# hhcho/sfgwas

Hardware: AMD Instinct MI355X
Metric: pca_power_iter_ring_macs_per_s (higher is better)
Workload: dtype u64 ring words, exact integers: int8 digits on the matrix core for the MAC of all five moduli, fp64-held integers in the encode and key-switch kernels

## Files before the change

### sfgwas_amd/csrc/ab/config.hip

```cpp
#include "../common.hpp"

void ab_read_config(SfgConfig &c) {
    auto env = [](const char *n) { return getenv(n); };
    if (const char *e = env("SFG_MAC_IMPL")) { c.mac_reg = !strcmp(e, "reg"); c.mac_bc = strcmp(e, "dma") != 0 && !c.mac_reg; c.mac_i8 = !strcmp(e, "i8"); }
    if (const char *e = env("SFG_MAC_I8_BIG")) c.mac_i8_big = atoi(e) != 0;
    if (const char *e = env("SFG_MAC_I8_ROT")) { c.mac_i8_nolds = strcmp(e, "lds") != 0; c.mac_i8_ring = !strcmp(e, "ring"); }
    if (env("SFG_MAC_I8_WG")) c.mac_i8_ring = false;
    if (const char *e = env("SFG_MAC_I8_WAVES")) c.mac_i8_waves = atoi(e) == 6 ? 6 : 12;
    if (const char *e = env("SFG_MAC_I8_WG")) c.mac_i8_wg1 = atoi(e) == 1;
    if (const char *e = env("SFG_MAC_WC")) c.mac_wc = atoi(e) == 2 ? 2 : 1;
    if (const char *e = env("SFG_MM_OVERLAP")) c.no_overlap = atoi(e) == 0;
    if (env("SFG_MM_NO_OVERLAP")) c.no_overlap = true;
    if (const char *e = env("SFG_NTT_HALF_IMPL")) c.ntt_half_full = !strcmp(e, "full");
    if (const char *e = env("SFG_NTT_FWD_IMPL")) c.ntt_fwd_full = !strcmp(e, "full");
    if (const char *e = env("SFG_MAC_PT")) c.mac_plain_pt = !strcmp(e, "plain");
    if (const char *e = env("SFG_PT_RIDE")) { c.pt_ride = atoi(e); if (c.pt_ride < 0) c.pt_ride = 0; c.pt_ride = c.pt_ride / 8 * 8; }
    if (const char *e = env("SFG_PT_COMPACT")) c.pt_compact = atoi(e) != 0;
    if (const char *e = env("SFG_PT_KMAJOR")) c.pt_kmajor = atoi(e) != 0;
    if (const char *e = env("SFG_PT_RIDE_DEPTH")) { c.i8_mover_depth_ride = atoi(e); if (c.i8_mover_depth_ride < 1 || c.i8_mover_depth_ride > 3) c.i8_mover_depth_ride = 1; }
    if (const char *e = env("SFG_PT_RIDE_NT")) c.i8_mover_nt_ride = atoi(e) != 0;
    if (env("SFG_ASSOC_TRACE")) c.assoc_trace = true;
}
int ab_set_attrs(sfg_ctx *ctx) { return ab_mac_dma_set_attrs(ctx) || ab_ntt_set_attrs(ctx); }
```

### sfgwas_amd/csrc/common.hpp

```cpp
#pragma once
#include <hip/hip_runtime.h>
#include <cstdint>
#include <cstdio>
#include <cstring>
#include <string>
#include <vector>
#include <map>
#include <set>
#include <initializer_list>
#include <type_traits>
#include <unistd.h>
#include "../../include/sfgwas_hip.h"
#include "fp64mod.hpp"
#include "consts.hpp"

typedef unsigned long long u64;
typedef unsigned __int128 u128;

constexpr unsigned long long SFG_I8_BIG_QMAX = 0x7F7F7F7F7F80ULL;

struct ModConst {
    double q, qinv;
    double ninv, ninv_q;
    u64 qi;
};

struct RotKey {
    u64 *key_dev = nullptr;
    uint16_t *index_dev = nullptr;
};

struct PhaseStat { double ms = 0; int launches = 0; double bytes = 0; };
struct PendingEvent { hipEvent_t e0, e1; std::string name; int launches; double bytes; };

struct sfg_geno {
    const int8_t *dev = nullptr;
    size_t nrow = 0, ncol = 0, ld = 0;
    bool owned = false;
    bool packed = false;
    struct PtcEntry { double *slot; bool transposed; };
    mutable std::map<uint64_t, PtcEntry> ptc;
    mutable size_t ptc_budget = 0, ptc_used = 0;
    mutable double *ptc_arena = nullptr;
    mutable uint32_t *ptc_perm = nullptr;
    mutable const void *ptc_owner = nullptr;
    mutable size_t ptc_hits = 0, ptc_fills = 0;
};

struct SfgConfig {
    int mm_group = 8;
    bool mm_group_auto = true;
    size_t acc_budget = 24ULL << 30;
    size_t assoc_cache_budget = 160ULL << 30;
    size_t ksw_budget = 4ULL << 30;
    int enc_batch = 2048;
    bool upload_blocking = false;
    bool test_hooks = false;
    std::string test_scratch_oom;
    double tie_band = 0x1p-50;
    bool mac_i8_big = true;
    bool mac_reg = false;
    bool mac_bc = true;
    bool mac_i8 = true;
    bool mac_i8_nolds = true;
    bool mac_i8_ring = true;
    int mac_i8_waves = 12;
    bool mac_i8_wg1 = false;
    int mac_wc = 1;
    bool no_overlap = true;
    bool ntt_fwd_full = false;
    bool ntt_half_full = false;
    bool pt_compact = true;
    bool pt_kmajor = true;
    int pt_ride = 192;
    int i8_mover_depth_ride = 1, i8_mover_nt_ride = 1;
    bool mac_plain_pt = false;
    bool assoc_trace = false;
};

struct SfgShared {
    int device = 0;
    int logN = SFG_LOGN, N = SFG_N, nq = 0, np = 0, nmod = 0, beta = 0;
    double scale = 0;
    u64 q[SFG_MAXMOD] = {0}, psi[SFG_MAXMOD] = {0};
    double *tw_fwd = nullptr;
    double *tw_inv = nullptr;
    double2 *pack_fwd = nullptr;
    double2 *pack_inv = nullptr;
    ModConst *modc = nullptr;
    ModConst modc_host[SFG_MAXMOD];
    void *enc_tables = nullptr;
    void *rvec_tables = nullptr;
    void *zeros_dev = nullptr;
    u64 *sk_dev = nullptr;
    u64 *pk_dev = nullptr;
    u64 *skqp_dev = nullptr;
    uint32_t enc_key[8] = {0, 0, 0, 0, 0, 0, 0, 0}; uint32_t *enc_key_dev = nullptr; bool enc_seeded = false;
    u64 enc_next = 0;
    std::map<u64, RotKey> rotkeys;
    SfgConfig cfg;
    int refs = 1;
};

struct sfg_ctx {
    SfgShared *sh = nullptr;
    bool is_fork = false;
    int device = 0;
    int logN = SFG_LOGN, N = SFG_N, nq = 0, np = 0, nmod = 0, beta = 0;
    double scale = 0;
    u64 q[SFG_MAXMOD] = {0}, psi[SFG_MAXMOD] = {0};
    double *tw_fwd = nullptr, *tw_inv = nullptr;
    double2 *pack_fwd = nullptr, *pack_inv = nullptr;
    ModConst *modc = nullptr;
    ModConst modc_host[SFG_MAXMOD];
    SfgConfig cfg;
    unsigned ntt_plain_seq = 0;
    struct I8Slot { const void *src = nullptr; u64 sig[8] = {0, 0, 0, 0, 0, 0, 0, 0}; u64 last_use = 0; };
    static constexpr int I8_SLOTS = 16;
    u64 i8_gen = 1, i8_clock = 0; I8Slot i8_slot[2][I8_SLOTS];
    hipStream_t own_stream = nullptr, stream = nullptr;
    hipStream_t user_stream = nullptr;
    hipStream_t aux_stream = nullptr;
    unsigned char *pin = nullptr; size_t pin_bytes = 0, pin_head = 0;
    hipStream_t coll_stream = nullptr;
    hipEvent_t ev_pipe[4] = {nullptr, nullptr, nullptr, nullptr};
    std::vector<hipEvent_t> ev_pool; size_t ev_next = 0;
    std::map<int, struct KswLevel *> ksw_cache;
    void *ws = nullptr; size_t ws_bytes = 0;
    std::map<std::string, std::pair<void *, size_t>> pool;
    std::map<std::string, std::pair<void *, size_t>> host_pool;
    std::map<std::string, unsigned long long> pool_epoch;
    unsigned long long api_epoch = 0; int api_depth = 0;
    int scratch_oom_seen = 0;
    std::vector<PendingEvent> pending;
    std::string err;
    std::map<std::string, PhaseStat> phases;
    std::set<const sfg_geno *> ptc_genos;
    bool test_hooks = false;
    void *tie_count_dev = nullptr;
    hipStream_t main_stream() const { return user_stream ? user_stream : own_stream; }
    std::map<u64, RotKey> &rotkeys() { return sh->rotkeys; }
    const std::map<u64, RotKey> &rotkeys() const { return sh->rotkeys; }
    void *enc_tables() const { return sh->enc_tables; }
    void *zeros_dev() const { return sh->zeros_dev; }
};

int sfg_sync_all(sfg_ctx *ctx);
int sfg_encoder_check(sfg_ctx *ctx);
void sfg_ptc_detach_all(sfg_ctx *ctx);
void sfg_ptc_invalidate_all(sfg_ctx *ctx);

int encrypt_set_attrs(sfg_ctx *ctx);
int sfg_rows_from_montgomery(sfg_ctx *ctx, unsigned long long *rows_dev, size_t nrows, int nmod);
void sfg_encrypt_destroy(SfgShared *sh);
int enc_take_indices(sfg_ctx *ctx, const char *what, int nct, unsigned long long *first);
int keygen_set_attrs(sfg_ctx *ctx);
void sfg_keygen_destroy(SfgShared *sh);
int sfg_rvec_init(sfg_ctx *ctx);
void sfg_rvec_destroy(SfgShared *sh);
// ... 119 lines not shown
```

### sfgwas_amd/csrc/kernels.hpp

```cpp
#pragma once
#include "common.hpp"
#include "mm_plan.hpp"
#include "assoc_plan.hpp"
#include "batch_plan.hpp"

constexpr int SFG_MAXPATTERN = 128;
struct ModPattern { int period; int8_t m[SFG_MAXPATTERN]; };
inline ModPattern mod_pattern_run(int first, int count) { ModPattern p; p.period = count; for (int j = 0; j < count; j++) p.m[j] = (int8_t)(first + j); return p; }
struct RowMap { int rpg; size_t gstride_in, gstride_out; };
struct PanelMap { int G, g, shift0; unsigned packed_mask = 0; int K = 0; };

int launch_ntt_fwd(sfg_ctx *ctx, const u64 *in, u64 *out, size_t nrows, const ModPattern &pat);
int launch_ntt_inv(sfg_ctx *ctx, const u64 *in, u64 *out, size_t nrows, const ModPattern &pat);
int launch_ntt_plain(sfg_ctx *ctx, const double *pc, u64 *out, size_t nplain, int L);
struct MoveJob;
struct PtRide;
int launch_ntt_plain_half(sfg_ctx *ctx, const double *pc, u64 *out_half, size_t nplain, int L, PanelMap pm, const uint32_t *perm = nullptr, const MoveJob *mv = nullptr);
int launch_expand_half(sfg_ctx *ctx, const u64 *half, u64 *full, size_t nrows);
int launch_ntt_fwd_map(sfg_ctx *ctx, const u64 *in, u64 *out, size_t nrows, const ModPattern &pat, const RowMap &rm);
int launch_ntt_inv_map(sfg_ctx *ctx, const u64 *in, u64 *out, size_t nrows, const ModPattern &pat, const RowMap &rm);
int launch_ntt_fwd_staged(sfg_ctx *ctx, const u64 *in, u64 *out, size_t nrows, const ModPattern &pat, bool staged);
int launch_ntt_inv_split(sfg_ctx *ctx, const u64 *in, u64 *out, size_t nrows, const ModPattern &pat, const RowMap &rm);
struct MacStrides { size_t rot_k, rot_r, pt_k, pt_n, out_n, out_r; bool pt_half = false; bool pt_packed = false; bool pt_digits = false; bool i8 = false; bool i8_big = false; bool pt_digits_big = false;
                    const int8_t *B_small = nullptr, *B_big = nullptr;
                    int pt_layout = 0, pt_L = 0;
                    int B_mode = 0;
                    const int8_t *A_small = nullptr, *A_big = nullptr; };
int launch_mac_i8_small(sfg_ctx *ctx, const double *rotf, size_t rotf_k_stride, size_t rotf_r_stride, int plane0, const u64 *pt, u64 *out, int K, int R, int r0, int Ncols,
                        int l0, int nl, int accumulate, const MacStrides &st);
int launch_mac_i8_big(sfg_ctx *ctx, const double *rotf, size_t rotf_k_stride, size_t rotf_r_stride, int plane0, const u64 *pt, u64 *out, int K, int R, int r0, int Ncols,
                      int l0, int accumulate, const MacStrides &st);
int launch_skew(sfg_ctx *ctx, const int8_t *blk, size_t ld, int r, int c, int transposed, int square, int8_t *D);
struct PcCache { double *slot = nullptr; int mode = 0; const uint32_t *perm = nullptr; };
int launch_encode_rows(sfg_ctx *ctx, const int8_t *D, int shift0, int nshift, int L, u64 *pt, bool half_rows = false, int G = 0, int g = 0, unsigned packed_mask = 0, const PcCache *pcache = nullptr,
                       PtRide *ride = nullptr);
int encode_rows_launches(const sfg_ctx *ctx, int nshift);
int i8_ride_prepare(sfg_ctx *ctx, const u64 *panel, int K, int Ncols, size_t pt_k, size_t pt_n, int layout, int L, int launches, PtRide &ride);
int i8_ride_finish(sfg_ctx *ctx, PtRide &ride);
int i8_ride_tiles(sfg_ctx *ctx, int K, int L, int8_t **Bs, int8_t **Bb);
struct I8Args;
void launch_i8_pack_pt_digits(hipStream_t q, const I8Args &a, unsigned items, bool big);
void launch_move_alone(hipStream_t q, const MoveJob &j);
int launch_share(sfg_ctx *ctx, const u64 *rows, size_t rows_ct_stride, const u64 *xr, size_t x_ct_stride, u64 *h, int nl, int nct, int neg = 0);
int launch_add_rows(sfg_ctx *ctx, const u64 *a, size_t a_ct_stride, const u64 *b, size_t b_ct_stride, u64 *out, size_t out_ct_stride, int nl, int nct);
struct DecSrc {
    enum Kind { ROWS, FINISH, DECRYPT } kind; const u64 *src; size_t stride; const u64 *h0agg;
    static DecSrc rows(const u64 *pt, size_t stride) { return DecSrc{ROWS, pt, stride, nullptr}; }
    static DecSrc finish(const u64 *ct, const u64 *h0agg) { return DecSrc{FINISH, ct, 0, h0agg}; }
    static DecSrc decrypt(const u64 *ct) { return DecSrc{DECRYPT, ct, 0, nullptr}; }
};
int launch_dec_front(sfg_ctx *ctx, const DecSrc &s, int first, int nb, int nl, u64 *x, int *launches = nullptr);
int check_level_count(sfg_ctx *ctx, const char *what, int nct, int level, int maxl, int min_count = 0);
int encrypt_errors_moddown(sfg_ctx *ctx, const int32_t *e0, const int32_t *e1, int nct, int level, u64 *out);
int launch_geno_unpack(sfg_ctx *ctx, const sfg_geno *g, size_t r0, size_t c0, size_t nr, size_t nc, int8_t *out, size_t ld_out);
int launch_rotate_right(sfg_ctx *ctx, const u64 *in, u64 *out, int nct, int level, const int *nrot_host);
int launch_rotate_right_indexed(sfg_ctx *ctx, const u64 *in, int nin, u64 *out, int nct, int level, const int *nrot_host, const int *in_index);
int launch_rotate_right_indexed_f64(sfg_ctx *ctx, const u64 *in, int nin, double *outf, int nct, int level, const int *nrot_host, const int *in_index, int L,
                                    const size_t *out_slot = nullptr);
int launch_rotate_right_sum(sfg_ctx *ctx, const u64 *in, int nin, int nct, int level, const int *nrot_host, const int *in_index, const int *group, int nout,
                            u64 *out, size_t out_stride, int accumulate);
int launch_relinearize(sfg_ctx *ctx, const u64 *tmp, int nct, int level, const u64 *mid, u64 *out);
int launch_ct_add(sfg_ctx *ctx, const u64 *a, const u64 *b, u64 *out, size_t nct, int level);
int mac_dma_planes(sfg_ctx *ctx, int L, std::vector<int> &plane_of, std::vector<int> &is_big);
double mac_big_maxterm(u64 q);
int launch_rot_to_f64(sfg_ctx *ctx, const u64 *rot, size_t nrows, int nl_rot, int L, double *rotf);
int launch_mac_dma(sfg_ctx *ctx, const double *rotf, size_t rows_per_k, const u64 *pt, u64 *out, int K, int R, int Ncols, int L, int accumulate, const MacStrides &st);
int launch_pack_pt(sfg_ctx *ctx, const u64 *in, u64 *out, size_t nrows, size_t words_per_row, int L, unsigned packed_mask);
unsigned mac_dma_packed_mask(sfg_ctx *ctx, int L);
bool mac_use_dma(const sfg_ctx *ctx);
int launch_mac_bc(sfg_ctx *ctx, const double *rotf, size_t rows_per_k, const u64 *pt, u64 *out, int K, int R, int Ncols, int L, int accumulate, const MacStrides &st);
int rotcache_build_rows_tab(sfg_ctx *ctx, const u64 *A, int s, int in_level, int max_level, int nbr, int b0, int b1, const std::vector<std::vector<uint8_t>> *tabs, double *cache);
int assoc_build_rotcache(sfg_ctx *ctx, const u64 *A_dev, int s, int in_level, int max_level, size_t nr, const std::vector<size_t> &widths, double **out);
struct I8RotPre { int G = 0, nbr = 0, s = 0, L = 0; std::vector<int8_t *> As, Ab; };
int i8_rotpre_build(sfg_ctx *ctx, const u64 *A_dev, int s, int in_level, int max_level, int nbr, const std::vector<std::vector<uint8_t>> *tabs, size_t budget_bytes, const char *prefix, I8RotPre &pre);
void i8_rotpre_free(I8RotPre &pre);
struct I8RotPreScope { I8RotPre pre; ~I8RotPreScope() { i8_rotpre_free(pre); } };
struct RotOperand {
    RotSrc src = RotSrc::own;
    const u64 *A = nullptr;
    int in_level = -1;
    const double *rows = nullptr;
    const I8RotPre *tiles = nullptr;
    static RotOperand own(const u64 *A, int in_level) { RotOperand r; r.A = A; r.in_level = in_level; return r; }
    static RotOperand f64_cache(const double *rows, int in_level = -1) { RotOperand r; r.src = RotSrc::f64_cache; r.rows = rows; r.in_level = in_level; return r; }
    static RotOperand i8_tiles(const I8RotPre *pre) { RotOperand r; r.src = RotSrc::i8_tiles; r.tiles = pre; return r; }
    int level_in(int max_level) const { return in_level < 0 ? max_level : in_level; }
    int validate(sfg_ctx *ctx, int s, int L, int nbr, int b0, int b1) const;
};
struct MmArgs { const sfg_geno *g; unsigned flags; int s, max_level, b0, b1, j0, j1, accumulate; uint64_t *acc; size_t acc_col_words; };
struct MmRangeArgs { const sfg_geno *g; unsigned flags; int s, max_level, blk0, blk1; uint64_t *out; };
int matmul_accumulate(sfg_ctx *ctx, const RotOperand &rot, const MmArgs &a);
int matmul_resident_range(sfg_ctx *ctx, const RotOperand &rot, const MmRangeArgs &a);
int launch_i8_pack_rot_to(sfg_ctx *ctx, const double *rotf, size_t rotf_k_stride, size_t rotf_r_stride, int plane0, int K, int R, int l0, int nl, bool big, int8_t *A_out);
struct AssocRot { RotOperand op; I8RotPre pre; };
int assoc_build_rot(sfg_ctx *ctx, const u64 *A_dev, int s, int in_level, int max_level, size_t nr, const std::vector<size_t> &widths, AssocRot &out);
void assoc_free_rot(AssocRot &r);
struct AssocRotScope { AssocRot r; ~AssocRotScope() { assoc_free_rot(r); } };
int assoc_product(sfg_ctx *ctx, const AssocRot &r, int s, int max_level, const sfg_geno *g, unsigned flags, int nct, uint64_t *out);
int assoc_batch_tail(sfg_ctx *ctx, const u64 *tmp, const sfg_geno *g, int s, size_t nct, size_t ctw, uint64_t *out_dev, size_t out_ct_capacity, size_t out_shift,
                     double *sum_host, double *sqsum_host);

int launch_bed_decode(sfg_ctx *ctx, hipStream_t st, const uint8_t *dbed, size_t bps, size_t num_sample, size_t num_snp, const int32_t *rmap, const int32_t *cmap,
                      int8_t *out, size_t ld);
int launch_bed_decode_lut(sfg_ctx *ctx, hipStream_t st, const uint8_t *dbed, size_t bps, size_t num_sample, size_t num_snp, const int32_t *rmap, const int32_t *cmap,
                          int8_t *out, size_t ld, unsigned lut);
int upload_filter_map(sfg_ctx *ctx, const uint8_t *filt, size_t n, DevMem &map, size_t *kept);

int assoc_stream_part(sfg_ctx *ctx, int fmt, const char *path, size_t num_sample, size_t num_snp, const uint8_t *row_filter, const uint8_t *col_filter,
                      size_t batch_snps, const uint64_t *A_dev, int s, int in_level, int max_level, unsigned flags,
                      uint64_t *out_dev, size_t out_ct_capacity, size_t *out_ct, double *sum_host, double *sqsum_host,
                      int part, int nparts, std::vector<std::pair<size_t, size_t>> *ranges);
```

### sfgwas_amd/csrc/mac_i8.hip

```cpp
#include "common.hpp"
#include "kernels.hpp"
#include "i8_move.hpp"
#include <algorithm>
#include <cstring>
#include <vector>

constexpr int I8_PC = 16;
template <int ND> constexpr int i8_rot_img_stride() { return ND * 512; }
template <int ND>
__global__ void __launch_bounds__(256) k_i8_pack_rot(I8Args a) {
    extern __shared__ __attribute__((aligned(16))) int8_t img[];
    constexpr int CS = i8_rot_img_stride<ND>();
    const int N = SFG_N, tid = threadIdx.x;
    int b = blockIdx.x;
    const int rt = b & 1; b >>= 1;
    const int khalf = b & 1; b >>= 1;
    const int xb = b % (N / I8_PC), ch = (b / (N / I8_PC)) % a.nch, m = b / (N / I8_PC) / a.nch;
    const int x0 = xb * I8_PC, cc = tid & (I8_PC - 1), kkq = (tid >> 4) & 3, kh2 = (tid >> 6) & 1, rh = tid >> 7;
    const double *src = ND == 6 ? a.rotf + (size_t)a.plane0 * N + 2 * (x0 + cc) : a.rotf + (size_t)(a.plane0 + m) * N + x0 + cc;
    size_t koff[4]; bool kv[4];
#pragma unroll
    for (int j = 0; j < 4; j++) {
        const int k = ch * 64 + 32 * khalf + 16 * kh2 + 4 * kkq + j;
        int ks = k; kv[j] = k < a.K;
        if (a.kb) { const int gg = k / a.kb, baby = k - gg * a.kb; kv[j] = kv[j] && baby < SFG_D; ks = gg * SFG_D + baby; }
        koff[j] = kv[j] ? (size_t)ks * a.rotf_k_stride : 0;
    }
    double lo[8][4], hi[ND == 6 ? 8 : 1][4];
#pragma unroll
    for (int ri = 0; ri < 8; ri++) {
        const int r = a.r0 + rt * 16 + rh * 8 + ri;
        const double *e = src + (size_t)(r < a.R ? r : a.r0) * a.rotf_r_stride;
#pragma unroll
        for (int j = 0; j < 4; j++) { lo[ri][j] = e[koff[j]]; if (ND == 6) hi[ri][j] = e[koff[j] + 1]; }
    }
#pragma unroll
    for (int ri = 0; ri < 8; ri++) {
        const int r16 = rh * 8 + ri;
        const bool rv = a.r0 + rt * 16 + r16 < a.R;
        unsigned dw[ND];
#pragma unroll
        for (int i = 0; i < ND; i++) dw[i] = 0;
#pragma unroll
        for (int j = 0; j < 4; j++) {
            long long v = ND == 6 ? (long long)hi[ND == 6 ? ri : 0][j] * 8388608LL + (long long)lo[ri][j] : (long long)lo[ri][j];
            if (!(rv && kv[j])) v = 0;
            int8_t d[ND]; i8_digits<ND>(v, d);
#pragma unroll
            for (int i = 0; i < ND; i++) dw[i] |= (unsigned)(uint8_t)d[i] << (8 * j);
        }
        unsigned *o = reinterpret_cast<unsigned *>(img + cc * CS + (((r16 + 16 * kh2) ^ cc) << 4) + 4 * kkq);
#pragma unroll
        for (int i = 0; i < ND; i++) o[i * 128] = dw[i];
    }
    __syncthreads();
    for (int idx = tid; idx < I8_PC * ND * 32; idx += 256) {
        const int c2 = idx / (ND * 32), rem = idx - c2 * (ND * 32), dg = rem >> 5, lr = rem & 31;
        const uint4 w = *reinterpret_cast<const uint4 *>(img + c2 * CS + dg * 512 + ((lr ^ c2) << 4));
        *reinterpret_cast<uint4 *>(a.A + ((((((size_t)m * N + x0 + c2) * a.nch + ch) * 2 + rt) * ND + dg) * 1024) + khalf * 512 + lr * 16) = w;
    }
}
constexpr int I8_PP = 32;
template <int ND>
__global__ void __launch_bounds__(256) k_i8_pack_pt(I8Args a) {
    constexpr int PSTR = ND * 256 + 4;
    __shared__ __attribute__((aligned(16))) unsigned char img[I8_PP * PSTR];
    const int H = SFG_N / 2, tid = threadIdx.x;
    int b = blockIdx.x;
    const int cb = b % (H / I8_PP); b /= H / I8_PP;
    const int kq = b % (a.nch * 4); b /= a.nch * 4;
    const int jt = b % a.njt, m = b / a.njt;
    const int c0 = cb * I8_PP, cc = tid & (I8_PP - 1), slot = tid >> 5;
    const u64 *src = a.pt + a.pt_l0_off + (size_t)m * a.pt_l_stride + c0 + cc;
#pragma unroll 2
    for (int it = 0; it < 8; it++) {
        const int item = it * 8 + slot, j = item >> 2, k4 = item & 3, n = jt * 16 + j;
        unsigned dw[ND];
#pragma unroll
        for (int i = 0; i < ND; i++) dw[i] = 0;
#pragma unroll
        for (int x = 0; x < 4; x++) {
            const int k = kq * 16 + k4 * 4 + x;
            long long v = 0;
            if (k < a.K && n < a.Ncols) {
                const u64 w = src[(size_t)n * a.pt_n_stride + (size_t)k * a.pt_k_stride];
                v = ND == 6 ? (long long)w : (long long)((w & 0xFFFULL) | (((w >> 16) & 0xFFFULL) << 12) | ((w >> 32) << 24));
            }
            int8_t d[ND]; i8_digits<ND>(v, d);
#pragma unroll
            for (int i = 0; i < ND; i++) dw[i] |= (unsigned)(uint8_t)d[i] << (8 * x);
        }
#pragma unroll
        for (int i = 0; i < ND; i++) *reinterpret_cast<unsigned *>(img + cc * PSTR + i * 256 + j * 16 + k4 * 4) = dw[i];
    }
    __syncthreads();
    const int ch = kq >> 2, g = kq & 3, l16 = tid & 15;
    for (int pc = tid >> 4; pc < I8_PP * ND; pc += 16) {
        const int c2 = pc / ND, d = pc % ND;
        const unsigned *sp = reinterpret_cast<const unsigned *>(img + c2 * PSTR + d * 256 + l16 * 16);
        const uint4 w = make_uint4(sp[0], sp[1], sp[2], sp[3]);
        *reinterpret_cast<uint4 *>(a.B + ((((((size_t)m * H + c0 + c2) * a.njt + jt) * a.nch + ch) * ND + d) * 1024) + g * 256 + l16 * 16) = w;
    }
}
template <int ND>
__global__ void __launch_bounds__(256) k_i8_pack_pt_digits(I8Args a) {
    __shared__ __attribute__((aligned(16))) unsigned img[I8_PD * 64];
    const int H = SFG_N / 2, tid = threadIdx.x;
    int b = blockIdx.x;
    const int cb = b % (H / I8_PD); b /= H / I8_PD;
    const int kq = b % (a.nch * 4); b /= a.nch * 4;
    const int jt = b % a.njt, m = b / a.njt;
    const int c0 = cb * I8_PD, cq = tid & 31, slot = tid >> 5;
    const int ch = kq >> 2, g = kq & 3, l16 = tid & 15;
    const unsigned char *src = reinterpret_cast<const unsigned char *>(a.pt + a.pt_l0_off + (size_t)m * a.pt_l_stride) + (size_t)cb * a.pt_cb_stride + cq * 4;
    constexpr int NI = 8;
    for (int d = 0; d < ND; d++) {
        for (int it0 = 0; it0 < 8; it0 += NI) {
            unsigned w[NI][4];
#pragma unroll
            for (int u = 0; u < NI; u++) {
                const int item = (it0 + u) * 8 + slot, j = item >> 2, k4 = item & 3, n = jt * 16 + j;
#pragma unroll
                for (int x = 0; x < 4; x++) {
                    const int k = kq * 16 + k4 * 4 + x;
                    const bool ok = k < a.K && n < a.Ncols;
                    const unsigned v = *reinterpret_cast<const unsigned *>(src + (ok ? ((size_t)n * a.pt_n_stride + (size_t)k * a.pt_k_stride) * 8 : (size_t)0) + (size_t)d * a.pt_d_stride);
                    w[u][x] = ok ? v : 0u;
                }
            }
#pragma unroll
            for (int u = 0; u < NI; u++) {
                const int item = (it0 + u) * 8 + slot, j = item >> 2, k4 = item & 3;
                unsigned o[4]; bytes_tr4(w[u][0], w[u][1], w[u][2], w[u][3], o);
#pragma unroll
                for (int e = 0; e < 4; e++) img[(cq * 4 + e) * 64 + ((j ^ (cq & 7)) << 2) + (k4 ^ (cq >> 3))] = o[e];
            }
        }
        __syncthreads();
        for (int pc = tid >> 4; pc < I8_PD; pc += 16) {
            const int q2 = pc >> 2;
            const unsigned *sp = img + pc * 64 + ((l16 ^ (q2 & 7)) << 2);
            const uint4 w = make_uint4(sp[0 ^ (q2 >> 3)], sp[1 ^ (q2 >> 3)], sp[2 ^ (q2 >> 3)], sp[3 ^ (q2 >> 3)]);
            *reinterpret_cast<uint4 *>(a.B + ((((((size_t)m * H + c0 + pc) * a.njt + jt) * a.nch + ch) * ND + d) * 1024) + g * 256 + l16 * 16) = w;
// ... 157 lines not shown
    SFG_HIP(ctx, hipFuncSetAttribute((const void *)k_mac_i8_ring<5, 3>, hipFuncAttributeMaxDynamicSharedMemorySize, 3 * 10 * 5 * 1024));
    SFG_HIP(ctx, hipFuncSetAttribute((const void *)k_mac_i8_ring<6, 2>, hipFuncAttributeMaxDynamicSharedMemorySize, 2 * 10 * 6 * 1024));
    SFG_HIP(ctx, hipFuncSetAttribute((const void *)k_mac_i8_ring<5, 3, 2>, hipFuncAttributeMaxDynamicSharedMemorySize, 3 * 10 * 5 * 1024));
    SFG_HIP(ctx, hipFuncSetAttribute((const void *)k_mac_i8_ring<6, 2, 2>, hipFuncAttributeMaxDynamicSharedMemorySize, 2 * 10 * 6 * 1024));
    return 0;
}
void launch_i8_pack_pt_digits(hipStream_t q, const I8Args &a, unsigned items, bool big) {
    if (big) hipLaunchKernelGGL(k_i8_pack_pt_digits<6>, dim3(items), dim3(256), 0, q, a);
    else hipLaunchKernelGGL(k_i8_pack_pt_digits<5>, dim3(items), dim3(256), 0, q, a);
}
void launch_move_alone(hipStream_t q, const MoveJob &j) {
#define SFG_MV(D, T) hipLaunchKernelGGL((k_i8_move_pt<D, T>), dim3(j.nblocks), dim3(256), 0, q, j)
#ifdef SFG_AB
    if (j.depth == 3) { if (j.nt) SFG_MV(3, true); else SFG_MV(3, false); return; }
    if (j.depth == 2) { if (j.nt) SFG_MV(2, true); else SFG_MV(2, false); return; }
    if (!j.nt) { SFG_MV(1, false); return; }
#endif
    SFG_MV(1, true);
#undef SFG_MV
}
static bool i8_ride_moduli(sfg_ctx *ctx, int L, int &l_small0, int &n_small, int &l_big) {
    std::vector<int> plane_of, is_big; if (mac_dma_planes(ctx, L, plane_of, is_big) < 0) return false;
    l_big = -1; l_small0 = -1; n_small = 0; int nbig = 0;
    for (int l = 0; l < L; l++) { if (is_big[l]) { l_big = l; nbig++; } else { if (l_small0 < 0) l_small0 = l; n_small++; } }
    if (nbig > 1 || !n_small) return false;
    for (int l = 0; l < L; l++) if (!is_big[l] && (l < l_small0 || l >= l_small0 + n_small)) return false;
    if (l_big >= 0 && (!ctx->cfg.mac_i8_big || ctx->q[l_big] > SFG_I8_BIG_QMAX)) return false;
    return true;
}
int i8_ride_tiles(sfg_ctx *ctx, int K, int L, int8_t **Bs, int8_t **Bb) {
    int l_small0, n_small, l_big;
    *Bs = *Bb = nullptr;
    if (!i8_ride_moduli(ctx, L, l_small0, n_small, l_big)) return 0;
    SFG_TRY(sfg_scratch(ctx, "mi8.Bs", mac_i8_tile_bytes(K, n_small, 5), (void **)Bs));
    if (l_big >= 0) SFG_TRY(sfg_scratch(ctx, "mi8.Bb", mac_i8_tile_bytes(K, 1, 6), (void **)Bb));
    return 0;
}
void i8_panel_rows(const sfg_ctx *ctx, int layout, int K, int L, int l, bool big, I8Args &a) {
    const size_t H = SFG_N / 2;
    a.pt_d_stride = H; a.pt_cb_stride = I8_PD;
    if (layout == 0) { a.pt_l0_off = (size_t)l * H; a.pt_l_stride = H; return; }
    size_t below = 0, all = 0; for (int t = 0; t < L; t++) { const size_t pl = ctx->q[t] < (1ULL << 36) ? 5 : 6; if (t < l) below += pl; all += pl; }
    const size_t nd = big ? 6 : 5;
    if (layout == 1) { a.pt_l0_off = below * H / 8; a.pt_l_stride = nd * H / 8; return; }
    const size_t blk = (size_t)K * 128;
    a.pt_d_stride = 64 * blk; a.pt_cb_stride = blk;
    a.pt_l0_off = below * 64 * blk / 8; a.pt_l_stride = nd * 64 * blk / 8;
    a.pt_k_stride = 16; a.pt_n_stride = all * 64 * blk / 8;
}
int i8_ride_prepare(sfg_ctx *ctx, const u64 *panel, int K, int Ncols, size_t pt_k, size_t pt_n, int layout, int L, int launches, PtRide &ride) {
    const int H = SFG_N / 2;
    ride = PtRide();
    int l_small0, n_small, l_big;
    if (ctx->cfg.pt_ride <= 0 || launches < 1 || Ncols > 96 || !i8_ride_moduli(ctx, L, l_small0, n_small, l_big)) return 0;
    if (layout != 2 && (pt_n * 8 >= (1ULL << 31) || pt_k * 8 * 16 >= (1ULL << 31))) return 0;
    if (layout == 2 && (size_t)K * 128 * 64 * 32 >= (1ULL << 31)) return 0;
    int8_t *Bs, *Bb; SFG_TRY(i8_ride_tiles(ctx, K, L, &Bs, &Bb));
    const int nch = (K + 63) / 64, njt = (Ncols + 15) / 16;
    auto fill = [&](I8Args &a, int l0, int nl, int8_t *B) {
        memset(&a, 0, sizeof a);
        a.pt = panel; a.pt_k_stride = pt_k; a.pt_n_stride = pt_n; a.K = K; a.Ncols = Ncols; a.l0 = l0; a.nl = nl; a.nch = nch; a.njt = njt; a.pt_digits = 1; a.B = B;
        i8_panel_rows(ctx, layout, K, L, l0, l0 == l_big, a);
    };
    MoveJob &j = ride.job;
    fill(j.a5, l_small0, n_small, Bs); j.n5 = (unsigned)((size_t)n_small * njt * nch * 4 * (H / I8_PD));
    if (l_big >= 0) { fill(j.a6, l_big, 1, Bb); j.n6 = (unsigned)((size_t)njt * nch * 4 * (H / I8_PD)); } else { memset(&j.a6, 0, sizeof j.a6); j.n6 = 0; }
    j.nblocks = (unsigned)ctx->cfg.pt_ride; j.depth = ctx->cfg.i8_mover_depth_ride; j.nt = ctx->cfg.i8_mover_nt_ride; j.first = 0; j.count = 0;
    ride.next = 0; ride.per = (ride.total() + (unsigned)launches - 1) / (unsigned)launches;
    ride.item_bytes5 = 5.0 * 2 * 32768; ride.item_bytes6 = 6.0 * 2 * 32768;
    ride.on = true;
    return 0;
}
int i8_ride_finish(sfg_ctx *ctx, PtRide &ride) {
    if (!ride.on || ride.next >= ride.total()) return 0;
    MoveJob j = ride.job; j.first = ride.next; j.count = ride.total() - ride.next; ride.next = ride.total();
    j.nblocks = std::min(2048u, (j.count + 7u) / 8u * 8u);
    PhaseTimer t(ctx, "mac_i8_pack_pt");
    launch_move_alone(ctx->stream, j);
    SFG_HIP(ctx, hipGetLastError());
    t.stop(1);
    return 0;
}
template <int ND>
static int launch_mac_i8_nd(sfg_ctx *ctx, const double *rotf, size_t rotf_k_stride, size_t rotf_r_stride, int plane0, const u64 *pt, u64 *out, int K, int R, int r0, int Ncols,
                            int l0, int nl, int accumulate, const MacStrides &st) {
    const int N = SFG_N, H = N / 2;
    constexpr bool BIG = ND == 6;
    if (!st.pt_half || (!BIG && !st.pt_packed)) SFG_FAIL(ctx, "sfg_mac (i8): needs half-row plaintext rows (packed-limb words or digit planes for the small moduli)");
    if (BIG && nl != 1) SFG_FAIL(ctx, "sfg_mac (i8): one 46-bit modulus per launch");
    if (Ncols > 96) SFG_FAIL(ctx, "sfg_mac (i8): more than 96 columns per launch");
    if ((long long)K * ND >= 131072) SFG_FAIL(ctx, "sfg_mac (i8): K too large for the int32 digit sums (ND K 2^14 must stay below 2^31)");
    for (int t = l0; t < l0 + nl; t++) {
        if (ctx->q[t] > (BIG ? SFG_I8_BIG_QMAX : (1ULL << 38))) SFG_FAIL(ctx, "sfg_mac (i8): modulus %d = %llu does not fit %d signed base-256 digits / the exact fp64 recombination", t, (unsigned long long)ctx->q[t], ND);
    }
    const int8_t *B_given = BIG ? st.B_big : st.B_small;
    const int8_t *B_pre = B_given && st.B_mode == 1 ? B_given : nullptr;
    if (B_given && (st.B_mode < 1 || st.B_mode > 2 || !st.pt_digits)) SFG_FAIL(ctx, "sfg_mac (i8): internal: given tile buffers take digit-plane panels");
    const int8_t *A_pre = BIG ? st.A_big : st.A_small;
    if (A_pre && (r0 != 0 || R > 32)) SFG_FAIL(ctx, "sfg_mac (i8): internal: given rot tiles cover one block of <= 32 rows");
    I8Args a; memset(&a, 0, sizeof a);
    a.rotf = rotf; a.pt = pt; a.out = out; a.rotf_k_stride = rotf_k_stride; a.rotf_r_stride = rotf_r_stride;
    a.pt_k_stride = st.pt_k; a.pt_n_stride = st.pt_n; a.out_n_stride = st.out_n; a.out_r_stride = st.out_r;
    if (st.pt_layout && !st.pt_digits) SFG_FAIL(ctx, "sfg_mac (i8): internal: compact panel rows hold digit planes");
    i8_panel_rows(ctx, st.pt_layout, K, st.pt_L, l0, BIG, a);
    a.K = K; a.R = R; a.Ncols = Ncols; a.accumulate = accumulate; a.r0 = r0; a.l0 = l0; a.nl = nl; a.plane0 = plane0;
    a.nch = (K + 63) / 64; a.njt = (Ncols + 15) / 16; a.pt_digits = st.pt_digits ? 1 : 0;
    const size_t nA = (size_t)nl * N * a.nch * 2 * ND * 1024, nB = (size_t)nl * H * a.njt * a.nch * ND * 1024, nT = (size_t)nl * H * 2 * a.njt * 2 * 256;
    const u64 sig[8] = {ctx->i8_gen, (u64)K, (u64)R, (u64)r0, (u64)l0 << 8 | (u64)nl, (u64)plane0, (u64)rotf_k_stride, (u64)rotf_r_stride};
    sfg_ctx::I8Slot *slots = ctx->i8_slot[BIG ? 1 : 0];
    int slot = -1;
    if (!A_pre) for (int i = 0; i < sfg_ctx::I8_SLOTS; i++) if (slots[i].src == (const void *)rotf && !memcmp(slots[i].sig, sig, sizeof sig)) slot = i;
    const bool repack = slot < 0 && !A_pre;
    char nm[24];
    if (repack) {
        int stale = -1, empty = -1, lru = 0;
        for (int i = 0; i < sfg_ctx::I8_SLOTS; i++) {
            if (!slots[i].src) { if (empty < 0) empty = i; continue; }
            if (slots[i].sig[0] != ctx->i8_gen && (stale < 0 || slots[i].last_use < slots[stale].last_use)) stale = i;
            if (slots[i].last_use < slots[lru].last_use || !slots[lru].src) lru = i;
        }
        slot = stale;
        if (slot < 0 && empty >= 0) {
            int live = 0; for (int i = 0; i < sfg_ctx::I8_SLOTS; i++) live += slots[i].src != nullptr;
            size_t fr = 0, tot = 0;
            if (live < 2 || (hipMemGetInfo(&fr, &tot) == hipSuccess && fr >= nA + (48ULL << 30))) slot = empty;
        }
        if (slot < 0) slot = lru;
    }
    if (A_pre) a.A = const_cast<int8_t *>(A_pre);
    else {
        snprintf(nm, sizeof nm, BIG ? "mi8.Ab%d" : "mi8.A%d", slot);
        SFG_TRY(sfg_scratch(ctx, nm, nA, (void **)&a.A));
        if (repack) { slots[slot].src = (const void *)rotf; memcpy(slots[slot].sig, sig, sizeof sig); }
        slots[slot].last_use = ++ctx->i8_clock;
    }
    if (B_given) a.B = const_cast<int8_t *>(B_given);
    else SFG_TRY(sfg_scratch(ctx, "mi8.B", nB, (void **)&a.B));
    SFG_TRY(sfg_scratch(ctx, "mi8.T", nT * 8, (void **)&a.T));
    if (!A_pre && !repack && ctx->pool[nm].second < nA) SFG_FAIL(ctx, "sfg_mac (i8): internal: kept rot copy smaller than its operand");
    const double tile = 1024.0;
    if (repack) { PhaseTimer t(ctx, "mac_i8_pack_rot");
      hipLaunchKernelGGL(k_i8_pack_rot<ND>, dim3((unsigned)((size_t)nl * a.nch * (N / I8_PC) * 4)), dim3(256), I8_PC * i8_rot_img_stride<ND>(), ctx->stream, a);
      SFG_HIP(ctx, hipGetLastError()); t.stop(1, (double)nl * N * ((double)K * std::min(32, R - r0) * (BIG ? 16.0 : 8.0) + (double)a.nch * 2 * ND * tile)); }
    if (!B_pre) { PhaseTimer t(ctx, "mac_i8_pack_pt");
      const unsigned items = (unsigned)((size_t)nl * a.njt * a.nch * 4 * (H / I8_PD));
      if (a.pt_digits) launch_i8_pack_pt_digits(ctx->stream, a, items, BIG);
      else hipLaunchKernelGGL(k_i8_pack_pt<ND>, dim3((unsigned)((size_t)nl * a.njt * a.nch * 4 * (H / I8_PP))), dim3(256), 0, ctx->stream, a);
      SFG_HIP(ctx, hipGetLastError()); t.stop(1, (double)nl * H * ((double)K * Ncols * (a.pt_digits ? (double)ND : 8.0) + (double)a.njt * a.nch * ND * tile)); }
    { PhaseTimer t(ctx, BIG ? "mac_big" : "mac_small");
      if (a.njt == 6 && ctx->cfg.mac_i8_ring) {
          if (BIG && ctx->cfg.mac_i8_waves == 12) hipLaunchKernelGGL((k_mac_i8_ring<6, 2, 2>), dim3((unsigned)(nl * H)), dim3(768), 2 * 10 * 6 * 1024, ctx->stream, a, ctx->modc);
          else if (BIG) hipLaunchKernelGGL((k_mac_i8_ring<6, 2>), dim3((unsigned)(nl * H)), dim3(384), 2 * 10 * 6 * 1024, ctx->stream, a, ctx->modc);
          else if (ctx->cfg.mac_i8_waves == 12) hipLaunchKernelGGL((k_mac_i8_ring<5, 3, 2>), dim3((unsigned)(nl * H)), dim3(768), 3 * 10 * 5 * 1024, ctx->stream, a, ctx->modc);
          else hipLaunchKernelGGL((k_mac_i8_ring<5, 3>), dim3((unsigned)(nl * H)), dim3(384), 3 * 10 * 5 * 1024, ctx->stream, a, ctx->modc);
      }
#ifdef SFG_AB
      else if (!BIG && a.njt == 6 && !ctx->cfg.mac_i8_nolds) ab_launch_mac_i8_lds(ctx->stream, a, ctx->modc, nl);
#endif
      else if (ctx->cfg.mac_i8_wg1) hipLaunchKernelGGL(k_mac_i8<ND>, dim3((unsigned)(nl * H * a.njt)), dim3(64), 0, ctx->stream, a, ctx->modc);
      else hipLaunchKernelGGL(k_mac_i8<ND>, dim3((unsigned)(nl * H)), dim3(64 * a.njt), 0, ctx->stream, a, ctx->modc);
      SFG_HIP(ctx, hipGetLastError());
      t.stop(1, (double)nl * ((double)N * a.nch * 2 * ND * tile + (double)H * a.njt * a.nch * ND * tile + (double)H * 2 * a.njt * 2 * 256 * 8.0)); }
    { PhaseTimer t(ctx, "mac_i8_untile");
      hipLaunchKernelGGL(k_i8_untile, dim3((unsigned)((size_t)nl * (H / 16) * 2 * a.njt * 2)), dim3(256), 0, ctx->stream, a, ctx->modc);
      SFG_HIP(ctx, hipGetLastError());
      t.stop(1, (double)nl * N * (double)Ncols * std::min(32, R - r0) * 8.0 * (accumulate ? 3.0 : 2.0)); }
    return 0;
}
int launch_i8_pack_rot_to(sfg_ctx *ctx, const double *rotf, size_t rotf_k_stride, size_t rotf_r_stride, int plane0, int K, int R, int l0, int nl, bool big, int8_t *A_out) {
    if (R > 32 || (big && nl != 1)) SFG_FAIL(ctx, "i8 rot tiles: internal: at most 32 rows, one 46-bit modulus per buffer");
    I8Args a; memset(&a, 0, sizeof a);
    a.rotf = rotf; a.rotf_k_stride = rotf_k_stride; a.rotf_r_stride = rotf_r_stride; a.K = K; a.R = R; a.r0 = 0; a.l0 = l0; a.nl = nl; a.plane0 = plane0;
    a.nch = (K + 63) / 64; a.kb = 0; a.A = A_out;
    const int N = SFG_N;
    PhaseTimer t(ctx, "mac_i8_pack_rot");
    if (big) hipLaunchKernelGGL(k_i8_pack_rot<6>, dim3((unsigned)((size_t)nl * a.nch * (N / I8_PC) * 4)), dim3(256), I8_PC * i8_rot_img_stride<6>(), ctx->stream, a);
    else hipLaunchKernelGGL(k_i8_pack_rot<5>, dim3((unsigned)((size_t)nl * a.nch * (N / I8_PC) * 4)), dim3(256), I8_PC * i8_rot_img_stride<5>(), ctx->stream, a);
    SFG_HIP(ctx, hipGetLastError());
    t.stop(1);
    return 0;
}
int launch_mac_i8_small(sfg_ctx *ctx, const double *rotf, size_t rotf_k_stride, size_t rotf_r_stride, int plane0, const u64 *pt, u64 *out, int K, int R, int r0, int Ncols,
                        int l0, int nl, int accumulate, const MacStrides &st) {
    return launch_mac_i8_nd<5>(ctx, rotf, rotf_k_stride, rotf_r_stride, plane0, pt, out, K, R, r0, Ncols, l0, nl, accumulate, st);
}
int launch_mac_i8_big(sfg_ctx *ctx, const double *rotf, size_t rotf_k_stride, size_t rotf_r_stride, int plane0, const u64 *pt, u64 *out, int K, int R, int r0, int Ncols,
                      int l0, int accumulate, const MacStrides &st) {
    return launch_mac_i8_nd<6>(ctx, rotf, rotf_k_stride, rotf_r_stride, plane0, pt, out, K, R, r0, Ncols, l0, 1, accumulate, st);
}

__global__ void __launch_bounds__(256) k_i8_words_to_planes(const u64 *in, u64 *out, int L, unsigned big_mask) {
    const int H = SFG_N / 2;
    const size_t row = blockIdx.x; const int l = (int)(row % (size_t)L);
    const u64 *src = in + row * H; int8_t *dst = reinterpret_cast<int8_t *>(out + row * H);
    const bool big = (big_mask >> l) & 1u;
    for (int c = threadIdx.x; c < H; c += 256) {
        const long long v = (long long)src[c];
        if (big) { int8_t d[6]; i8_digits<6>(v, d);
#pragma unroll
            for (int i = 0; i < 6; i++) dst[(size_t)i * H + c] = d[i]; }
        else { int8_t d[5]; i8_digits<5>(v, d);
#pragma unroll
            for (int i = 0; i < 5; i++) dst[(size_t)i * H + c] = d[i]; }
    }
}
extern "C" int sfg_mac_i8_dev(sfg_ctx *ctx, const uint64_t *rot, const uint64_t *pt_half, uint64_t *out, int K, int R, int Ncols, int L, int accumulate, int pt_form) {
    SFG_HIP(ctx, hipSetDevice(ctx->device));
    if (!ctx->test_hooks) SFG_FAIL(ctx, "sfg_mac_i8_dev is a test hook: the context was not created under the test switch");
    if (L < 1 || L > ctx->nq) SFG_FAIL(ctx, "sfg_mac_i8: L out of range");
    if (K < 1 || R < 1 || Ncols < 1) SFG_FAIL(ctx, "sfg_mac_i8: K, R and Ncols must be positive (got %d, %d, %d)", K, R, Ncols);
    if (Ncols > 96 || (long long)K * 6 >= 131072) SFG_FAIL(ctx, "sfg_mac_i8: at most 96 columns and K < 21846 per launch");
    if (pt_form != 0 && pt_form != 1) SFG_FAIL(ctx, "sfg_mac_i8: pt_form is 0 (digit planes) or 1 (panel words)");
    const int N = SFG_N, H = N / 2;
    std::vector<int> plane_of, is_big; const int nplanes = mac_dma_planes(ctx, L, plane_of, is_big);
    if (nplanes < 0) return 1;
    unsigned big_mask = 0, small_mask = 0; for (int l = 0; l < L; l++) (is_big[l] ? big_mask : small_mask) |= 1u << l;
    if (big_mask && !ctx->cfg.mac_i8_big) SFG_FAIL(ctx, "sfg_mac_i8: a modulus above 2^36 is on the fp64 kernel in this context (it exceeds six signed digits: q > 0x7F7F7F7F7F80; or the A/B build's switch)");
    const size_t rrows = (size_t)K * R, prows = (size_t)K * Ncols * L;
    double *rotf = nullptr; u64 *ptp = nullptr;
    int rc = 0;
    if (hipMalloc(&rotf, rrows * (size_t)nplanes * N * 8) != hipSuccess || hipMalloc(&ptp, prows * H * 8) != hipSuccess) { (void)hipGetLastError(); (void)hipFree(rotf); SFG_FAIL(ctx, "sfg_mac_i8: out of device memory"); }
    rc = launch_rot_to_f64(ctx, (const u64 *)rot, rrows, L, L, rotf);
    if (!rc) {
        if (pt_form == 0) { hipLaunchKernelGGL(k_i8_words_to_planes, dim3((unsigned)prows), dim3(256), 0, ctx->stream, (const u64 *)pt_half, ptp, L, big_mask); if (hipGetLastError() != hipSuccess) { rc = 1; ctx->err = "sfg_mac_i8: plane kernel launch failed"; } }
        else rc = launch_pack_pt(ctx, (const u64 *)pt_half, ptp, prows, (size_t)H, L, small_mask);
    }
    if (!rc) {
        MacStrides st;
        st.rot_k = (size_t)R * L * N; st.rot_r = (size_t)L * N;
        st.pt_k = (size_t)Ncols * L * H; st.pt_n = (size_t)L * H;
        st.out_n = (size_t)R * L * N; st.out_r = (size_t)L * N;
        st.pt_half = true; st.pt_packed = true; st.i8 = st.i8_big = true; st.pt_digits = st.pt_digits_big = pt_form == 0;
        PhaseTimer t(ctx, "mac");
        rc = launch_mac_bc(ctx, rotf, (size_t)R, ptp, (u64 *)out, K, R, Ncols, L, accumulate, st);
        t.stop(1);
    }
    (void)hipStreamSynchronize(ctx->stream); (void)hipFree(rotf); (void)hipFree(ptp);
    return rc;
}
```

### sfgwas_amd/csrc/matmul.hip

```cpp
#include "common.hpp"
#include "kernels.hpp"
#include "i8_move.hpp"
#include <algorithm>
#include <string>

static inline int ceil_div(size_t a, size_t b) { return (int)((a + b - 1) / b); }

struct Shape {
    size_t nrow, ncol;
    int nbr, m_ct;
    bool transposed;
    const int8_t *dev; size_t ld;
    const sfg_geno *g;
    int rows_of(int bi) const { return (int)(std::min((size_t)(bi + 1) * SFG_SLOTS, nrow) - (size_t)bi * SFG_SLOTS); }
    int cols_of(int bj) const { return (int)(std::min((size_t)(bj + 1) * SFG_SLOTS, ncol) - (size_t)bj * SFG_SLOTS); }
    const int8_t *block(int bi, int bj) const {
        return transposed ? dev + (size_t)bj * SFG_SLOTS * ld + (size_t)bi * SFG_SLOTS
                          : dev + (size_t)bi * SFG_SLOTS * ld + (size_t)bj * SFG_SLOTS;
    }
};
static Shape make_shape(const sfg_geno *g, unsigned flags) {
    Shape sh; sh.transposed = (flags & SFG_TRANSPOSE) != 0;
    sh.nrow = sh.transposed ? g->ncol : g->nrow; sh.ncol = sh.transposed ? g->nrow : g->ncol;
    sh.nbr = ceil_div(sh.nrow, SFG_SLOTS); sh.m_ct = ceil_div(sh.ncol, SFG_SLOTS);
// ... 214 lines not shown
extern "C" void sfg_geno_free(sfg_ctx *ctx, sfg_geno *g) {
    if (!g) return;
    ptc_drop(ctx, g);
    if (g->owned) { (void)hipSetDevice(ctx->device); (void)sfg_sync_all(ctx); (void)hipFree((void *)g->dev); }
    delete g;
}
extern "C" int sfg_geno_set_plaintext_cache(sfg_ctx *ctx, const sfg_geno *g, size_t max_bytes) {
    SFG_HIP(ctx, hipSetDevice(ctx->device));
    if (!g) SFG_FAIL(ctx, "sfg_geno_set_plaintext_cache: null matrix");
    if (!max_bytes) { ptc_drop(ctx, g); g->ptc_budget = 0; g->ptc_owner = nullptr; return 0; }
    if (g->ptc_owner && g->ptc_owner != (const void *)ctx) SFG_FAIL(ctx, "sfg_geno_set_plaintext_cache: the cache of this matrix belongs to another context (drop it there first)");
    if (!g->ptc_perm) {
        const int n = SFG_SLOTS, d = SFG_D; const unsigned M = 2u * SFG_N;
        std::vector<uint32_t> tab(n);
        std::vector<unsigned> pow5(n); pow5[0] = 1; for (int k = 1; k < n; k++) pow5[k] = (unsigned)(((u64)pow5[k - 1] * 5u) % M);
        for (int t = 0; t < n; t++) {
            const int u = (n - t) % n, k = ((t % d) + d * (u / d)) % n;
            tab[t] = (uint32_t)u | (uint32_t)pow5[k] << 16;
        }
        uint32_t *dv = nullptr;
        SFG_HIP(ctx, hipMalloc((void **)&dv, (size_t)n * 4));
        if (hipMemcpy(dv, tab.data(), (size_t)n * 4, hipMemcpyHostToDevice) != hipSuccess) { (void)hipFree(dv); SFG_FAIL(ctx, "sfg_geno_set_plaintext_cache: table upload failed"); }
        g->ptc_perm = dv;
    }
    const size_t slot_bytes = (size_t)SFG_SLOTS * SFG_SLOTS * 8, want = max_bytes / slot_bytes * slot_bytes;
    if (want != g->ptc_budget || !g->ptc_arena) {
        (void)hipStreamSynchronize(ctx->stream);
        g->ptc.clear(); g->ptc_used = 0;
        if (g->ptc_arena) { (void)hipFree(g->ptc_arena); g->ptc_arena = nullptr; }
        g->ptc_budget = 0;
        if (!want) SFG_FAIL(ctx, "sfg_geno_set_plaintext_cache: max_bytes is less than one block (%zu bytes)", slot_bytes);
        void *a = nullptr;
        if (hipMalloc(&a, want) != hipSuccess) { (void)hipGetLastError(); SFG_FAIL(ctx, "sfg_geno_set_plaintext_cache: cannot allocate %zu bytes", want); }
        g->ptc_arena = (double *)a; g->ptc_budget = want;
    }
    g->ptc_owner = ctx; ctx->ptc_genos.insert(g);
    return 0;
}
extern "C" int sfg_geno_plaintext_cache_stats(sfg_ctx *ctx, const sfg_geno *g, size_t *blocks, size_t *bytes, size_t *hits, size_t *fills) {
    if (!g) SFG_FAIL(ctx, "sfg_geno_plaintext_cache_stats: null matrix");
    if (blocks) *blocks = g->ptc.size();
    if (bytes) *bytes = g->ptc_used;
    if (hits) *hits = g->ptc_hits;
    if (fills) *fills = g->ptc_fills;
    return 0;
}
extern "C" int sfg_geno_colsums(sfg_ctx *ctx, const sfg_geno *g, double *sum_host, double *sqsum_host) {
    SFG_HIP(ctx, hipSetDevice(ctx->device));
    if (g->packed) {
        sfg_geno *u = nullptr; SFG_TRY(sfg_geno_unpack(ctx, g, &u));
        const int rc = sfg_geno_colsums(ctx, u, sum_host, sqsum_host); sfg_geno_free(ctx, u); return rc;
    }
    SFG_TRY(sfg_ws_reserve(ctx, g->ncol * 16));
    double *ds = (double *)ctx->ws, *dq = ds + g->ncol;
    SFG_HIP(ctx, hipMemsetAsync(ds, 0, g->ncol * 16, ctx->stream));
    hipLaunchKernelGGL(k_colsums, dim3((unsigned)((g->ncol + 255) / 256), (unsigned)((g->nrow + CS_ROWS - 1) / CS_ROWS)), dim3(256), 0, ctx->stream, g->dev, g->nrow, g->ncol, g->ld, ds, dq);
    SFG_HIP(ctx, hipGetLastError());
    if (sum_host) SFG_HIP(ctx, hipMemcpyAsync(sum_host, ds, g->ncol * 8, hipMemcpyDeviceToHost, ctx->stream));
    if (sqsum_host) SFG_HIP(ctx, hipMemcpyAsync(sqsum_host, dq, g->ncol * 8, hipMemcpyDeviceToHost, ctx->stream));
    SFG_HIP(ctx, hipStreamSynchronize(ctx->stream));
    return 0;
}
extern "C" int sfg_reduce_rows_dev(sfg_ctx *ctx, uint64_t *rows, size_t nrows_of_L, int L) {
    SFG_HIP(ctx, hipSetDevice(ctx->device));
    const size_t rows_total = nrows_of_L * L;
    if (!rows_total) return 0;
    hipLaunchKernelGGL(k_reduce_rows, dim3((unsigned)(rows_total * (SFG_N / 256))), dim3(256), 0, ctx->stream, (u64 *)rows, L, ctx->modc);
    SFG_HIP(ctx, hipGetLastError());
    return 0;
}

static std::vector<uint8_t> baby_table(const Shape &sh, int bi) {
    const int d = SFG_D, nr = sh.rows_of(bi);
    std::vector<uint8_t> baby_t(d, 0);
    for (int shift = 0; shift < SFG_SLOTS; shift++) {
        if (baby_t[shift % d]) continue;
        bool any = false;
        for (int bj = 0; bj < sh.m_ct && !any; bj++) any = diag_bool(nr, sh.cols_of(bj), SFG_SLOTS, -shift);
        if (any) baby_t[shift % d] = 1;
    }
    return baby_t;
}
static int build_rot_row_tab(sfg_ctx *ctx, const u64 *A, int s, int nl_in, int nl, int lev, int L, int nbr, int bi, const std::vector<uint8_t> &baby_t,
                             u64 *a_row, u64 *rotc, bool dma, double *rotf_dst) {
    const int d = SFG_D;
    SFG_TRY(launch_gather_operands(ctx, A, a_row, nbr, s, bi * s, s, nl_in, nl));
    {
        PhaseTimer t(ctx, "rotate");
        std::vector<int> nrv((size_t)d * s, 0), inv((size_t)d * s, 0);
        for (int baby = 0; baby < d; baby++) for (int i = 0; i < s; i++) { nrv[(size_t)baby * s + i] = baby_t[baby] ? -baby : 0; inv[(size_t)baby * s + i] = i; }
        if (dma) SFG_TRY(launch_rotate_right_indexed_f64(ctx, a_row, s, rotf_dst, d * s, lev, nrv.data(), inv.data(), L));
        else SFG_TRY(launch_rotate_right_indexed(ctx, a_row, s, rotc, d * s, lev, nrv.data(), inv.data()));
        t.stop(1);
    }
    return 0;
}


struct PoolMemory { size_t search = 0, keep = 0; bool failed = false; };
static PoolMemory pool_memory(sfg_ctx *ctx, const char *extra_prefix) {
    PoolMemory m; size_t fr = 0, tot = 0;
    m.failed = hipMemGetInfo(&fr, &tot) != hipSuccess;
    m.search = m.keep = fr;
    for (const auto &kv : ctx->pool) {
        if ((extra_prefix && kv.first.rfind(extra_prefix, 0) == 0) || kv.first == "mm.pt" || kv.first == "mm.rotf" || kv.first.rfind("mi8.", 0) == 0) m.search += kv.second.second;
        if (kv.first.rfind("mi8.A", 0) == 0) m.keep += kv.second.second;
    }
    return m;
}
static MmPlanIn plan_input(sfg_ctx *ctx, int s, int L, int nblockrows, int ncolb, const RotOperand &rot) {
    const SfgConfig &c = ctx->cfg;
    MmPlanIn in;
    in.mm_group = c.mm_group; in.mm_group_auto = c.mm_group_auto; in.mac_i8 = c.mac_i8; in.mac_i8_big = c.mac_i8_big;
    in.pt_compact = c.pt_compact; in.pt_kmajor = c.pt_kmajor; in.pt_ride = c.pt_ride; in.no_overlap = c.no_overlap;
    in.dma = mac_use_dma(ctx); in.packed_mask = in.dma ? mac_dma_packed_mask(ctx, L) : 0u; in.mods = ModSplit(ctx->q, L);
    in.s = s; in.L = L; in.nblockrows = nblockrows; in.ncolb = ncolb; in.rot = rot.src; in.pre_G = rot.tiles ? rot.tiles->G : 0;
    if (mm_plan_reads_memory(in)) { const PoolMemory m = pool_memory(ctx, nullptr); in.mem_failed = m.failed; in.mem_search = m.search; in.mem_keep = m.keep; }
    return in;
}
struct MmCall {
    sfg_ctx *ctx; const Shape &sh; unsigned flags; const RotOperand &rot;
    int s, L, lev, nl, nl_in; bool dma; unsigned packed_mask; size_t ctw, accw, rowf = 0;
    MmPlan plan;
    u64 *a_row = nullptr, *rotc = nullptr; int8_t *skew = nullptr, *unpacked = nullptr; double *rotf = nullptr;
    int8_t *rideBs = nullptr, *rideBb = nullptr;
};
struct MacJob { bool on = false; u64 *ptp = nullptr; int gsn = 0, gi = 0, acc_flag = 0; u64 *accj = nullptr; const double *rotf_grp = nullptr; };

static int build_group(const MmCall &c, int bg, int b1, int buf) {
    sfg_ctx *ctx = c.ctx; const int d = SFG_D, s = c.s, ng = std::min(c.plan.G, b1 - bg);
    ctx->i8_gen++;
    double *dst = c.rotf + (size_t)buf * c.plan.grp_slices * s * 2 * c.rowf;
    for (int g = 0; g < ng; g++) SFG_TRY(build_rot_row_tab(ctx, c.rot.A, s, c.nl_in, c.nl, c.lev, c.L, c.sh.nbr, bg + g, baby_table(c.sh, bg + g), c.a_row, c.rotc, c.dma, c.dma ? dst + (size_t)g * d * s * 2 * c.rowf : nullptr));
    if (c.dma && (ng * d) % 4)
        SFG_HIP(ctx, hipMemsetAsync(dst + (size_t)ng * d * s * 2 * c.rowf, 0, (size_t)3 * s * 2 * c.rowf * 8, ctx->stream));
    return 0;
}
static int run_mac(const MmCall &c, const MacJob &m, int B_mode) {
    sfg_ctx *ctx = c.ctx; const MmPlan &p = c.plan; const int N = SFG_N, d = SFG_D;
    PhaseTimer t(ctx, "mac");
    MacStrides st;
    if (c.rideBs) { st.B_small = c.rideBs; st.B_big = c.rideBb; st.B_mode = B_mode; }
    if (c.rot.tiles) { st.A_small = c.rot.tiles->As[m.gi]; st.A_big = c.rot.tiles->Ab[m.gi]; }
    st.rot_k = (size_t)c.s * c.ctw; st.rot_r = (size_t)c.nl * N;
    st.pt_k = p.plw; st.pt_n = (size_t)m.gsn * d * p.plw; st.pt_half = c.dma; st.pt_packed = c.packed_mask != 0; st.pt_digits = st.i8 = p.use_i8; st.i8_big = st.pt_digits_big = p.use_i8_big;
    st.pt_layout = p.pt_layout; st.pt_L = c.L;
    st.out_n = c.accw; st.out_r = (size_t)c.L * N;
    int rc;
    if (c.dma) rc = launch_mac_dma(ctx, m.rotf_grp, (size_t)c.s * 2, m.ptp, m.accj, m.gsn * d, 2 * c.s, d, c.L, m.acc_flag, st);
#ifdef SFG_AB
    else rc = launch_mac_strided(ctx, c.rotc, m.ptp, m.accj, d, 2 * c.s, d, c.L, m.acc_flag, st);
#else
    else { rc = 1; ctx->err = "matmul: the register-staged MAC exists in the A/B build only (make ab)"; }
#endif
    t.stop(1);
    return rc;
}
struct PtcSlot {
    static constexpr size_t slot_bytes = (size_t)SFG_SLOTS * SFG_SLOTS * 8;
    PcCache pcc; const sfg_geno *g; uint64_t key = 0; bool fresh = false;
    PtcSlot(const MmCall &c, int bi, int bj) : g(c.sh.g) {
        if (!c.dma || !g->ptc_budget || g->ptc_owner != (const void *)c.ctx) return;
        const uint64_t sr = c.sh.transposed ? bj : bi, sc = c.sh.transposed ? bi : bj;
        key = sr << 33 | sc << 1 | ((c.flags & SFG_SQUARE) ? 1u : 0u);
        auto it = g->ptc.find(key);
        if (it != g->ptc.end()) { pcc.slot = it->second.slot; pcc.mode = it->second.transposed == c.sh.transposed ? 2 : 3; pcc.perm = g->ptc_perm; g->ptc_hits++; }
        else if (g->ptc_used + slot_bytes <= g->ptc_budget) {
            double *slot = g->ptc_arena + g->ptc_used / 8;
            g->ptc[key] = sfg_geno::PtcEntry{slot, c.sh.transposed}; g->ptc_used += slot_bytes; g->ptc_fills++;
            pcc.slot = slot; pcc.mode = 1; fresh = true;
        }
    }
    void undo() {
        if (!fresh) return;
        auto it = g->ptc.find(key);
        if (it != g->ptc.end()) { g->ptc.erase(it); g->ptc_used -= slot_bytes; }
        fresh = false;
    }
};
static int encode_block(const MmCall &c, int bi, int bj, int g, int ng, u64 *pt, PtRide *ride) {
    sfg_ctx *ctx = c.ctx; const Shape &sh = c.sh; const MmPlan &p = c.plan;
    const int d = SFG_D, L = c.L, nr = sh.rows_of(bi), nc = sh.cols_of(bj), tr = sh.transposed ? 1 : 0, sq = (c.flags & SFG_SQUARE) ? 1 : 0;
    const size_t plw = p.plw, nplain = (size_t)d * d;
    PtcSlot ptc(c, bi, bj);
    int rc = 0;
    if (ptc.pcc.mode < 2) {
        PhaseTimer t(ctx, "skew");
        if (sh.g->packed) {
            const size_t sr0 = (size_t)(tr ? bj : bi) * SFG_SLOTS, sc0 = (size_t)(tr ? bi : bj) * SFG_SLOTS;
            rc = launch_geno_unpack(ctx, sh.g, sr0, sc0, tr ? nc : nr, tr ? nr : nc, c.unpacked, SFG_SLOTS);
            if (!rc) rc = launch_skew(ctx, c.unpacked, SFG_SLOTS, nr, nc, tr, sq, c.skew);
        } else rc = launch_skew(ctx, sh.block(bi, bj), sh.ld, nr, nc, tr, sq, c.skew);
        t.stop(1);
    }
    if (rc) { ptc.undo(); return rc; }
    int runs[2][2]; int nruns = 0;
    if (nr + nc > SFG_SLOTS) { runs[0][0] = 0; runs[0][1] = SFG_SLOTS; nruns = 1; }
    else { runs[0][0] = 0; runs[0][1] = nr; runs[1][0] = SFG_SLOTS - nc + 1; runs[1][1] = SFG_SLOTS; nruns = runs[1][0] < runs[1][1] ? 2 : 1; }
    const bool full = nruns == 1 && runs[0][1] - runs[0][0] == SFG_SLOTS;
    if (p.kmajor) {
        const int kb0 = g * d;
        if (full) rc = launch_pt_zero_kmajor(ctx, pt, ng * d, p.pt_planes, d - 1, d, kb0 + (SFG_SLOTS - (d - 1) * d), kb0 + d);
        else rc = launch_pt_zero_kmajor(ctx, pt, ng * d, p.pt_planes, 0, d, kb0, kb0 + d);
    } else if (full) {
        rc = launch_pt_zero(ctx, pt + (((size_t)(d - 1) * ng + g) * d + (SFG_SLOTS - (d - 1) * d)) * plw, 0, (nplain - SFG_SLOTS) * plw, 1, L, p.prow, c.packed_mask);
    } else {
        rc = launch_pt_zero(ctx, pt + (size_t)g * d * plw, (size_t)ng * d * plw, (size_t)d * plw, d, L, p.prow, c.packed_mask);
    }
    if (rc) { ptc.undo(); return rc; }
    PhaseTimer t(ctx, "encode");
    for (int r = 0; r < nruns && !rc; r++) {
        if (c.dma) rc = launch_encode_rows(ctx, c.skew, runs[r][0], runs[r][1] - runs[r][0], L, pt, true, ng, g, p.enc_flags, ptc.pcc.mode ? &ptc.pcc : nullptr, ride);
        else rc = launch_encode_rows(ctx, c.skew, runs[r][0], runs[r][1] - runs[r][0], L, pt + (size_t)runs[r][0] * plw, false);
    }
    t.stop(nruns);
    if (rc) ptc.undo();
    return rc;
}
static int ride_launch_count(const MmCall &c, int bg, int ng, int nc) {
    int launches = 0;
    for (int g = 0; g < ng; g++) {
        const int nr = c.sh.rows_of(bg + g);
        if (nr + nc > SFG_SLOTS) launches += encode_rows_launches(c.ctx, SFG_SLOTS);
        else launches += encode_rows_launches(c.ctx, nr) + (nc > 1 ? encode_rows_launches(c.ctx, nc - 1) : 0);
    }
    return launches;
}

int RotOperand::validate(sfg_ctx *ctx, int s, int L, int nbr, int b0, int b1) const {
    if (src == RotSrc::f64_cache && !mac_use_dma(ctx)) SFG_FAIL(ctx, "matmul: a prebuilt rotation cache needs the LDS-DMA MAC (the A/B build selected the register-staged kernel)");
    if (src == RotSrc::i8_tiles) {
        if (!tiles || !tiles->G) SFG_FAIL(ctx, "matmul: no int8 rot tiles");
        if (!mac_use_dma(ctx) || b0 != 0 || b1 != tiles->nbr || nbr != tiles->nbr || s != tiles->s || L != tiles->L)
            SFG_FAIL(ctx, "matmul: internal: the int8 rot tiles were built for another product (block rows %d, s = %d, level %d)", tiles->nbr, tiles->s, tiles->L);
    }
    return 0;
}
static int accumulate_blocks(sfg_ctx *ctx, const RotOperand &rot, const Shape &sh, const MmArgs &a) {
    const int N = SFG_N, d = SFG_D, s = a.s, max_level = a.max_level, L = max_level, in_level = rot.level_in(max_level);
    const int b0 = a.b0, b1 = a.b1, j0 = a.j0, j1 = a.j1, accumulate = a.accumulate; u64 *const acc = (u64 *)a.acc;
    SFG_TRY(rot.validate(ctx, s, L, sh.nbr, b0, b1));
    const int lev = in_level > max_level ? max_level : in_level, nl = lev + 1, nl_in = in_level + 1;
    if (L < 1 || L > ctx->nq) SFG_FAIL(ctx, "matmul: max_level out of range");
    if (nl < L) SFG_FAIL(ctx, "matmul: input level %d has fewer than max_level = %d moduli", in_level, max_level);
    if (b0 < 0 || b1 > sh.nbr || b0 > b1 || j0 < 0 || j1 > sh.m_ct || j0 > j1) SFG_FAIL(ctx, "matmul: block range out of bounds");
    const size_t ctw = (size_t)2 * nl * N, accw = (size_t)s * 2 * L * N;
    const int ncolb = j1 - j0;
    const size_t acc_col = a.acc_col_words ? a.acc_col_words : (size_t)d * accw;
    if (acc_col < (size_t)d * accw) SFG_FAIL(ctx, "matmul: internal: accumulator column stride below 91 giant steps");
    if (b0 == b1 || j0 == j1) {
        if (!accumulate) for (int c = 0; c < ncolb; c++) SFG_HIP(ctx, hipMemsetAsync(acc + (size_t)c * acc_col, 0, (size_t)d * accw * 8, ctx->stream));
        return 0;
    }
    const MmPlanIn in = plan_input(ctx, s, L, b1 - b0, ncolb, rot);
    if (in.dma && in.mods.too_big) SFG_FAIL(ctx, "sfg_mac: modulus >= 2^47 unsupported by the fp64 limb schedule");
    MmCall c{ctx, sh, a.flags, rot, s, L, lev, nl, nl_in, in.dma, in.packed_mask, ctw, accw};
    c.plan = mm_plan(in);
    MmPlan &plan = c.plan;
    const int G = plan.G; const bool dma = in.dma, rot_ext = in.rot != RotSrc::own;
    u64 *pt = nullptr;
    SFG_TRY(sfg_scratch(ctx, "mm.a_row", (size_t)s * ctw * 8, (void **)&c.a_row));
    SFG_TRY(sfg_scratch(ctx, "mm.rotc", dma ? 8 : (size_t)d * s * ctw * 8, (void **)&c.rotc));
    if (plan.ride_want && sfg_scratch(ctx, "mm.pt", plan.panel_words * 8 * 2 + 65536, (void **)&pt)) { ctx->err.clear(); plan.ride_want = false; }
    if (!plan.ride_want) SFG_TRY(sfg_scratch(ctx, "mm.pt", plan.panel_words * 8 + 65536, (void **)&pt));
    u64 *const pt_base = pt;
    SFG_TRY(sfg_scratch(ctx, "mm.skew", (size_t)SFG_SLOTS * SFG_SLOTS, (void **)&c.skew));
    if (sh.g->packed) SFG_TRY(sfg_scratch(ctx, "mm.unpack", (size_t)SFG_SLOTS * SFG_SLOTS, (void **)&c.unpacked));
    if (dma) {
        c.rowf = (size_t)in.mods.fp64_planes * N;
        if (!rot_ext) SFG_TRY(sfg_scratch(ctx, "mm.rotf", plan.grp_slices * s * 2 * c.rowf * 8 * (plan.pipelined ? 2 : 1), (void **)&c.rotf));
    }
    const size_t rot_half = plan.grp_slices * s * 2 * c.rowf;
    hipStream_t main_stream = ctx->stream;
    if (plan.pipelined) {
        SFG_TRY(sfg_stream_after(ctx, ctx->aux_stream, main_stream));
        { AuxScope aux(ctx); SFG_TRY(build_group(c, b0, b1, 0)); }
        SFG_HIP(ctx, hipEventRecord(ctx->ev_pipe[0], ctx->aux_stream));
    }
    int rc = 0, gi = 0, it = 0;
    MacJob held;
    for (int bg = b0; bg < b1; bg += G, gi++) {
        const int ng = std::min(G, b1 - bg);
        if (held.on && in.rot != RotSrc::i8_tiles) { SFG_TRY(run_mac(c, held, 2)); held.on = false; }
        const double *rotf_grp = c.rotf;
        if (in.rot == RotSrc::f64_cache) rotf_grp = rot.rows + (size_t)(bg - b0) * d * s * 2 * c.rowf;
        else if (in.rot == RotSrc::i8_tiles) rotf_grp = nullptr;
        else if (plan.pipelined) {
            if (bg + G < b1) {
                SFG_TRY(sfg_stream_after(ctx, ctx->aux_stream, main_stream));
                { AuxScope aux(ctx); SFG_TRY(build_group(c, bg + G, b1, (gi + 1) & 1)); }
                SFG_HIP(ctx, hipEventRecord(ctx->ev_pipe[(gi + 1) & 1], ctx->aux_stream));
            }
            SFG_HIP(ctx, hipStreamWaitEvent(main_stream, ctx->ev_pipe[gi & 1], 0));
            rotf_grp = c.rotf + (size_t)(gi & 1) * rot_half;
        } else SFG_TRY(build_group(c, bg, b1, 0));
        for (int bj = j0; bj < j1; bj++, it++) {
            pt = pt_base + (size_t)(plan.ride_want ? (it & 1) : 0) * plan.panel_words;
            PtRide ride;
            if (plan.ride_want && !c.rideBs) SFG_TRY(i8_ride_tiles(ctx, G * d, L, &c.rideBs, &c.rideBb));
            if (held.on && plan.ride_want && c.rideBs) {
                SFG_TRY(i8_ride_prepare(ctx, held.ptp, held.gsn * d, d, plan.plw, (size_t)held.gsn * d * plan.plw, plan.pt_layout, L, ride_launch_count(c, bg, ng, sh.cols_of(bj)), ride));
                if (ride.on && (ride.job.a5.B != c.rideBs || (ride.job.n6 && ride.job.a6.B != c.rideBb))) SFG_FAIL(ctx, "matmul: internal: the riding transposition's tile buffers moved");
            }
            if (held.on && !ride.on) { SFG_TRY(run_mac(c, held, c.rideBs ? 2 : 0)); held.on = false; }
            for (int g = 0; g < ng; g++) SFG_TRY(encode_block(c, bg + g, bj, g, ng, pt, ride.on ? &ride : nullptr));
            if (held.on) { SFG_TRY(i8_ride_finish(ctx, ride)); SFG_TRY(run_mac(c, held, 1)); held.on = false; }
            MacJob m; m.on = true; m.ptp = pt; m.gsn = ng; m.gi = gi;
            m.acc_flag = (accumulate || bg != b0) ? 1 : 0;
            m.accj = acc + (size_t)(bj - j0) * acc_col; m.rotf_grp = rotf_grp;
            if (plan.ride_want && c.rideBs) held = m;
            else SFG_TRY(run_mac(c, m, c.rideBs ? 2 : 0));
        }
    }
    if (held.on) rc = run_mac(c, held, 2);
    return rc;
}

static int matmul_finalize(sfg_ctx *ctx, const u64 *acc, int s, int max_level, int ncolb, int m_ct_out, int jout0, int g0, int g1,
                           const std::vector<uint8_t> *giant_active, int accumulate, u64 *out, int acc_giants = SFG_D, int giant_base = 0) {
    const int N = SFG_N, d = SFG_D, L = max_level;
    const size_t accw = (size_t)s * 2 * L * N, ctw = (size_t)2 * L * N;
    if (g0 < 0 || g1 > acc_giants || g0 > g1 || giant_base < 0) SFG_FAIL(ctx, "finalize: giant range out of bounds");
    std::vector<int> glist;
    for (int g = g0; g < g1; g++) if (giant_base + g < d && (!giant_active || (*giant_active)[giant_base + g])) glist.push_back(g);
    const int ng = (int)glist.size();
    std::vector<int> nrv((size_t)ng * s), inv((size_t)ng * s), grp((size_t)ng * s);
    for (int k = 0; k < ng; k++) for (int i = 0; i < s; i++) { nrv[(size_t)k * s + i] = -(giant_base + glist[k]) * d; inv[(size_t)k * s + i] = glist[k] * s + i; grp[(size_t)k * s + i] = i; }
    int rc = 0;
    for (int jb = 0; jb < ncolb && !rc; jb++) {
        const u64 *accj = acc + (size_t)jb * acc_giants * accw;
        u64 *o = out + (size_t)(jout0 + jb) * ctw;
        PhaseTimer t(ctx, "rotate");
        rc = launch_rotate_right_sum(ctx, accj, acc_giants * s, ng * s, L - 1, nrv.data(), inv.data(), grp.data(), s, o, (size_t)m_ct_out * ctw, accumulate);
        t.stop(1);
    }
    return rc;
}

static void giant_table(const Shape &sh, std::vector<uint8_t> &giant_t) {
    giant_t.assign(SFG_D, 0);
    for (int bi = 0; bi < sh.nbr; bi++) {
        const int nr = sh.rows_of(bi);
        for (int shift = 0; shift < SFG_SLOTS; shift++) {
            if (giant_t[shift / SFG_D]) { shift = (shift / SFG_D + 1) * SFG_D - 1; continue; }
            bool any = false;
            for (int bj = 0; bj < sh.m_ct && !any; bj++) any = diag_bool(nr, sh.cols_of(bj), SFG_SLOTS, -shift);
            if (any) giant_t[shift / SFG_D] = 1;
        }
    }
}

int matmul_accumulate(sfg_ctx *ctx, const RotOperand &rot, const MmArgs &a) {
    ApiScope api_scope(ctx);
    SFG_HIP(ctx, hipSetDevice(ctx->device));
    return accumulate_blocks(ctx, rot, make_shape(a.g, a.flags), a);
}
extern "C" int sfg_matmul_accumulate_dev(sfg_ctx *ctx, const uint64_t *A, int s, int in_level, int max_level, const sfg_geno *g, unsigned flags,
                                         int b0, int b1, int j0, int j1, int accumulate, uint64_t *acc) {
    return matmul_accumulate(ctx, RotOperand::own((const u64 *)A, in_level), {g, flags, s, max_level, b0, b1, j0, j1, accumulate, acc, 0});
}
extern "C" int sfg_matmul_finalize_dev(sfg_ctx *ctx, const uint64_t *acc, int s, int max_level, int ncolb, int g0, int g1, int accumulate, uint64_t *out) {
    ApiScope api_scope(ctx);
    SFG_HIP(ctx, hipSetDevice(ctx->device));
    return matmul_finalize(ctx, (const u64 *)acc, s, max_level, ncolb, ncolb, 0, g0, g1, nullptr, accumulate, (u64 *)out);
}

extern "C" int sfg_matmul_finalize_slots_dev(sfg_ctx *ctx, const uint64_t *acc, int s, int max_level, int ncolb, int acc_giants, int giant_base,
                                             int g0, int g1, int accumulate, uint64_t *out) {
    ApiScope api_scope(ctx);
    SFG_HIP(ctx, hipSetDevice(ctx->device));
    if (acc_giants < 1) SFG_FAIL(ctx, "finalize: acc_giants must be positive");
    return matmul_finalize(ctx, (const u64 *)acc, s, max_level, ncolb, ncolb, 0, g0, g1, nullptr, accumulate, (u64 *)out, acc_giants, giant_base);
}

int matmul_resident_range(sfg_ctx *ctx, const RotOperand &rot_in, const MmRangeArgs &a) {
    ApiScope api_scope(ctx);
    SFG_HIP(ctx, hipSetDevice(ctx->device));
    ctx->phases.clear();
    if (rot_in.src == RotSrc::own) ctx->i8_gen++;
    const Shape sh = make_shape(a.g, a.flags);
    const int d = SFG_D, s = a.s, L = a.max_level;
    std::vector<uint8_t> giant_t; giant_table(sh, giant_t);
    int b0 = 0, b1 = sh.nbr, j0 = 0, j1 = sh.m_ct;
    if (sh.transposed) { b0 = a.blk0; b1 = a.blk1; } else { j0 = a.blk0; j1 = a.blk1; }
    if (b0 < 0 || b1 > sh.nbr || j0 < 0 || j1 > sh.m_ct || b0 > b1 || j0 > j1) SFG_FAIL(ctx, "matmul: SNP-block range out of bounds");
    if (L < 1 || L > ctx->nq) SFG_FAIL(ctx, "matmul: max_level out of range");
    SFG_TRY(rot_in.validate(ctx, s, L, sh.nbr, b0, b1));
    const int m_out = j1 - j0;
    MmRangeIn in;
    in.s = s; in.L = L; in.nl = std::min(rot_in.level_in(L), L) + 1; in.rows = b1 - b0; in.cols = j1 - j0; in.fp64_planes = ModSplit(ctx->q, L).fp64_planes;
    in.acc_budget = ctx->cfg.acc_budget; in.no_overlap = ctx->cfg.no_overlap; in.dma = mac_use_dma(ctx); in.rot = rot_in.src;
    const MmRangePlan plan = mm_range_plan(in);
    RotOperand rot = rot_in;
    if (plan.whole_cache) {
        double *buf = nullptr;
        SFG_TRY(sfg_scratch(ctx, "mm.rotf", plan.cache_bytes, (void **)&buf));
        std::vector<std::vector<uint8_t>> tabs;
        for (int bi = b0; bi < b1; bi++) tabs.push_back(baby_table(sh, bi));
        SFG_TRY(rotcache_build_rows_tab(ctx, rot_in.A, s, rot_in.in_level, L, sh.nbr, b0, b1, &tabs, buf));
        rot = RotOperand::f64_cache(buf, rot_in.in_level);
    }
    const int jg = plan.jg; const size_t accw = (size_t)s * 2 * L * SFG_N;
    hipStream_t main_stream = ctx->stream;
    int k = 0;
    for (int ja = j0; ja < j1; ja += jg, k++) {
        const int jb = std::min(j1, ja + jg);
        u64 *acc = nullptr;
        SFG_TRY(sfg_scratch(ctx, "mm.acc", plan.acc_bytes, (void **)&acc));
        if (plan.overlap) {
            acc += (size_t)(k & 1) * jg * d * accw;
            if (k >= 2) SFG_HIP(ctx, hipStreamWaitEvent(main_stream, ctx->ev_pipe[2 + (k & 1)], 0));
        }
        SFG_TRY(accumulate_blocks(ctx, rot, sh, {a.g, a.flags, s, L, b0, b1, ja, jb, 0, (uint64_t *)acc, 0}));
        if (plan.overlap) SFG_TRY(sfg_stream_after(ctx, ctx->aux_stream, main_stream));
        { AuxScope aux(ctx, plan.overlap); SFG_TRY(matmul_finalize(ctx, acc, s, L, jb - ja, m_out, ja - j0, 0, d, &giant_t, 0, (u64 *)a.out)); }
        if (plan.overlap) SFG_HIP(ctx, hipEventRecord(ctx->ev_pipe[2 + (k & 1)], ctx->aux_stream));
    }
    if (plan.overlap) SFG_TRY(sfg_stream_after(ctx, main_stream, ctx->aux_stream));
    return 0;
}
extern "C" int sfg_matmul_resident_range_dev(sfg_ctx *ctx, const uint64_t *A, int s, int in_level, int max_level, const sfg_geno *g, unsigned flags,
                                             int blk0, int blk1, uint64_t *out) {
    return matmul_resident_range(ctx, RotOperand::own((const u64 *)A, in_level), {g, flags, s, max_level, blk0, blk1, out});
}

static int rotcache_rowf(sfg_ctx *ctx, int L, size_t &rowf) {
    if (!mac_use_dma(ctx)) SFG_FAIL(ctx, "rotation cache objects need the LDS-DMA MAC (the A/B build selected the register-staged kernel)");
    if (L < 1 || L > ctx->nq) SFG_FAIL(ctx, "rotcache: max_level out of range");
    std::vector<int> plane_of, is_big; const int nplanes = mac_dma_planes(ctx, L, plane_of, is_big);
    if (nplanes < 0) return 1;
    rowf = (size_t)nplanes * SFG_N; return 0;
}
extern "C" int sfg_rotcache_layout(sfg_ctx *ctx, int s, int max_level, size_t *job_doubles, size_t *tail_doubles) {
    size_t rowf = 0; SFG_TRY(rotcache_rowf(ctx, max_level, rowf));
    if (job_doubles) *job_doubles = (size_t)SFG_D * 2 * rowf;
    if (tail_doubles) *tail_doubles = (size_t)3 * s * 2 * rowf;
    return 0;
}
extern "C" int sfg_rotcache_build_jobs_dev(sfg_ctx *ctx, const uint64_t *A, int s, int in_level, int max_level, int nbr, int job0, int job1, double *staged) {
    ApiScope api_scope(ctx);
    SFG_HIP(ctx, hipSetDevice(ctx->device));
    const int N = SFG_N, d = SFG_D, L = max_level;
    size_t rowf = 0; SFG_TRY(rotcache_rowf(ctx, L, rowf));
    const int lev = in_level > max_level ? max_level : in_level, nl = lev + 1, nl_in = in_level + 1;
    if (nl < L || in_level >= ctx->nq) SFG_FAIL(ctx, "rotcache: input level %d unusable with max_level = %d", in_level, max_level);
    if (s < 1 || nbr < 1 || job0 < 0 || job1 > nbr * s || job0 > job1) SFG_FAIL(ctx, "rotcache: job range out of bounds");
    const size_t ctw = (size_t)2 * nl * N;
    constexpr int CH = 64;
    u64 *a_in = nullptr;
    SFG_TRY(sfg_scratch(ctx, "rc.in", (size_t)CH * ctw * 8, (void **)&a_in));
    PhaseTimer t(ctx, "rotate");
    for (int c0 = job0; c0 < job1; c0 += CH) {
        const int nj = std::min(CH, job1 - c0);
        SFG_TRY(launch_gather_operands(ctx, (const u64 *)A, a_in, nbr, s, c0, nj, nl_in, nl));
        std::vector<int> nrv((size_t)d * nj), inv((size_t)d * nj); std::vector<size_t> slot((size_t)d * nj);
        for (int baby = 0; baby < d; baby++) for (int k = 0; k < nj; k++) {
            nrv[(size_t)baby * nj + k] = -baby; inv[(size_t)baby * nj + k] = k; slot[(size_t)baby * nj + k] = (size_t)(c0 - job0 + k) * d + baby;
        }
        SFG_TRY(launch_rotate_right_indexed_f64(ctx, a_in, nj, staged, d * nj, lev, nrv.data(), inv.data(), L, slot.data()));
    }
    t.stop(1);
    return 0;
}
extern "C" int sfg_rotcache_scatter_dev(sfg_ctx *ctx, const double *staged, int s, int max_level, int job0, int job1, int row0, int nrows, double *cache) {
    ApiScope api_scope(ctx);
    SFG_HIP(ctx, hipSetDevice(ctx->device));
    ctx->i8_gen++;
    const int d = SFG_D;
    size_t rowf = 0; SFG_TRY(rotcache_rowf(ctx, max_level, rowf));
    if (s < 1 || nrows < 1 || job0 < row0 * s || job1 > (row0 + nrows) * s || job0 > job1) SFG_FAIL(ctx, "rotcache: job range outside the cache rows");
    const size_t jw = (size_t)2 * rowf;
    for (int job = job0; job < job1; job++) {
        const int bi = job / s, i = job % s;
        SFG_HIP(ctx, hipMemcpy2DAsync(cache + (((size_t)(bi - row0) * d) * s + i) * jw, (size_t)s * jw * 8, staged + (size_t)(job - job0) * d * jw, jw * 8, jw * 8, d,
                                      hipMemcpyDeviceToDevice, ctx->stream));
    }
    SFG_HIP(ctx, hipMemsetAsync(cache + (size_t)nrows * d * s * jw, 0, (size_t)3 * s * jw * 8, ctx->stream));
    return 0;
}
int rotcache_build_rows_tab(sfg_ctx *ctx, const u64 *A, int s, int in_level, int max_level, int nbr, int b0, int b1, const std::vector<std::vector<uint8_t>> *tabs, double *cache) {
    ctx->i8_gen++;
    SFG_HIP(ctx, hipSetDevice(ctx->device));
    const int N = SFG_N, d = SFG_D, L = max_level;
    size_t rowf = 0; SFG_TRY(rotcache_rowf(ctx, L, rowf));
    const int lev = in_level > max_level ? max_level : in_level, nl = lev + 1;
    if (nl < L || in_level >= ctx->nq) SFG_FAIL(ctx, "rotcache: input level %d unusable with max_level = %d", in_level, max_level);
    if (s < 1 || b0 < 0 || b1 > nbr || b0 > b1) SFG_FAIL(ctx, "rotcache: block-row range out of bounds");
    const size_t ctw = (size_t)2 * nl * N, per_row = (size_t)d * s * 2 * rowf;
    u64 *a_row = nullptr, *rotc = nullptr;
    SFG_TRY(sfg_scratch(ctx, "mm.a_row", (size_t)s * ctw * 8, (void **)&a_row));
    SFG_TRY(sfg_scratch(ctx, "mm.rotc", 8, (void **)&rotc));
    const std::vector<uint8_t> all(d, 1);
    for (int bi = b0; bi < b1; bi++)
        SFG_TRY(build_rot_row_tab(ctx, A, s, in_level + 1, nl, lev, L, nbr, bi, tabs ? (*tabs)[bi - b0] : all, a_row, rotc, true, cache + (size_t)(bi - b0) * per_row));
    SFG_HIP(ctx, hipMemsetAsync(cache + (size_t)(b1 - b0) * per_row, 0, (size_t)3 * s * 2 * rowf * 8, ctx->stream));
    return 0;
}
extern "C" int sfg_rotcache_build_rows_dev(sfg_ctx *ctx, const uint64_t *A, int s, int in_level, int max_level, int nbr, int b0, int b1, double *cache) {
    ApiScope api_scope(ctx);
    return rotcache_build_rows_tab(ctx, (const u64 *)A, s, in_level, max_level, nbr, b0, b1, nullptr, cache);
}
void i8_rotpre_free(I8RotPre &pre) { pre = I8RotPre(); }
int i8_rotpre_build(sfg_ctx *ctx, const u64 *A, int s, int in_level, int max_level, int nbr, const std::vector<std::vector<uint8_t>> *tabs, size_t budget_bytes, const char *prefix, I8RotPre &pre) {
    pre = I8RotPre();
    const int d = SFG_D, L = max_level;
    const auto &c = ctx->cfg;
    if (!mac_use_dma(ctx) || !c.mac_bc || c.mac_plain_pt || !c.mac_i8 || !c.mac_i8_big || 2 * s > 30 || L < 1 || L > ctx->nq || nbr < 1) return 0;
    if (!mac_dma_packed_mask(ctx, L)) return 0;
    const ModSplit m(ctx->q, L);
    const int l_big = m.l_big, l_s0 = m.l_small0, n_s = m.nsmall; const int *plane_of = m.plane_of;
    const size_t rowf = (size_t)m.fp64_planes * SFG_N;
    PoolMemory mem;
    if (c.mm_group_auto && nbr > c.mm_group) mem = pool_memory(ctx, prefix);
    int G = i8pre_group_size(m, c.mm_group, c.mm_group_auto, s, nbr, mem.failed, mem.search, budget_bytes);
    if (!G) return 0;
    double *tmp = nullptr;
    auto alloc_all = [&](int Gc) -> bool {
        const int ngc = (nbr + Gc - 1) / Gc;
        pre.As.assign(ngc, nullptr); pre.Ab.assign(ngc, nullptr);
        int arc = sfg_scratch(ctx, "mm.rotf", ((size_t)Gc * d + 3) * s * 2 * rowf * 8, (void **)&tmp);
        for (int gi = 0; gi < ngc && !arc; gi++) {
            const int ng = std::min(Gc, nbr - gi * Gc);
            char nm[48];
            snprintf(nm, sizeof nm, "%s.s%d", prefix, gi);
            arc = sfg_scratch(ctx, nm, mac_i8_rot_tile_bytes(ng * d, n_s, 5), (void **)&pre.As[gi]);
            if (!arc && l_big >= 0) { snprintf(nm, sizeof nm, "%s.b%d", prefix, gi); arc = sfg_scratch(ctx, nm, mac_i8_rot_tile_bytes(ng * d, 1, 6), (void **)&pre.Ab[gi]); }
        }
        if (arc) { ctx->err.clear(); i8_rotpre_free(pre); }
        return !arc;
    };
    if (!alloc_all(G)) {
        const int G0 = std::min(c.mm_group, nbr);
        if (G0 == G) return 0;
        G = G0;
        if (!alloc_all(G)) return 0;
    }
    const int ngrp = (nbr + G - 1) / G;
    for (int gi = 0; gi < ngrp; gi++) {
        const int bg = gi * G, ng = std::min(G, nbr - bg);
        std::vector<std::vector<uint8_t>> sub;
        if (tabs) sub.assign(tabs->begin() + bg, tabs->begin() + bg + ng);
        int rc = rotcache_build_rows_tab(ctx, A, s, in_level, max_level, nbr, bg, bg + ng, tabs ? &sub : nullptr, tmp);
        if (!rc) rc = launch_i8_pack_rot_to(ctx, tmp, (size_t)s * 2 * rowf, rowf, plane_of[l_s0], ng * d, 2 * s, l_s0, n_s, false, pre.As[gi]);
        if (!rc && l_big >= 0) rc = launch_i8_pack_rot_to(ctx, tmp, (size_t)s * 2 * rowf, rowf, plane_of[l_big], ng * d, 2 * s, l_big, 1, true, pre.Ab[gi]);
        if (rc) { i8_rotpre_free(pre); return rc; }
    }
    pre.G = G; pre.nbr = nbr; pre.s = s; pre.L = L;
    return 0;
}
extern "C" int sfg_matmul_resident_range_rc_dev(sfg_ctx *ctx, const double *cache, int s, int max_level, const sfg_geno *g, unsigned flags,
                                                int blk0, int blk1, uint64_t *out) {
    if (!cache) SFG_FAIL(ctx, "matmul: null rotation cache");
    return matmul_resident_range(ctx, RotOperand::f64_cache(cache), {g, flags, s, max_level, blk0, blk1, out});
}
extern "C" int sfg_matmul_accumulate_rc_dev(sfg_ctx *ctx, const double *cache, int s, int max_level, const sfg_geno *g, unsigned flags,
                                            int b0, int b1, int j0, int j1, int accumulate, uint64_t *acc) {
    if (!cache) SFG_FAIL(ctx, "matmul: null rotation cache");
    return matmul_accumulate(ctx, RotOperand::f64_cache(cache), {g, flags, s, max_level, b0, b1, j0, j1, accumulate, acc, 0});
}

extern "C" int sfg_matmul_resident_dev(sfg_ctx *ctx, const uint64_t *A, int s, int in_level, int max_level, const sfg_geno *g, unsigned flags, uint64_t *out) {
    ApiScope api_scope(ctx);
    const size_t nb = (g->ncol + SFG_SLOTS - 1) / SFG_SLOTS;
    return sfg_matmul_resident_range_dev(ctx, A, s, in_level, max_level, g, flags, 0, (int)nb, out);
}

extern "C" int sfg_matmul_stream(sfg_ctx *ctx, const uint64_t *A_host, int s, int in_level, int max_level,
                                 const int8_t *geno_host, size_t nrow, size_t ncol, size_t ld, unsigned flags,
                                 uint64_t *out_host, double *sum_host, double *sqsum_host) {
    ApiScope api_scope(ctx);
    SFG_HIP(ctx, hipSetDevice(ctx->device));
    sfg_geno *g = nullptr;
    SFG_TRY(sfg_geno_upload(ctx, geno_host, nrow, ncol, ld, &g));
    Shape sh = make_shape(g, flags);
    const size_t a_words = (size_t)s * sh.nbr * 2 * (in_level + 1) * SFG_N, o_words = (size_t)s * sh.m_ct * 2 * max_level * SFG_N;
    u64 *dA = nullptr, *dO = nullptr; int rc = 0;
    if (hipMalloc(&dA, a_words * 8) != hipSuccess || hipMalloc(&dO, o_words * 8) != hipSuccess) { rc = 1; ctx->err = "matmul_stream: out of device memory"; }
    if (!rc && hipMemcpy(dA, A_host, a_words * 8, hipMemcpyHostToDevice) != hipSuccess) { rc = 1; ctx->err = "matmul_stream: upload failed"; }
    if (!rc && (sum_host || sqsum_host)) rc = sfg_geno_colsums(ctx, g, sum_host, sqsum_host);
// ... 255 lines not shown
```

### sfgwas_amd/csrc/mm_plan.hpp

```cpp
#pragma once
#include "consts.hpp"
#include <algorithm>
#include <cstdint>

struct ModSplit {
    int L = 0, nsmall = 0, nbig = 0;
    int l_big = -1, l_small0 = -1;
    int small_runs = 0;
    int fp64_planes = 0, digit_planes = 0;
    int plane_of[SFG_MAXMOD] = {0}, is_big[SFG_MAXMOD] = {0};
    unsigned packed_mask_all = 0;
    bool too_big = false;
    ModSplit() {}
    ModSplit(const unsigned long long *q, int L_) : L(L_) {
        for (int l = 0; l < L; l++) {
            if (q[l] >= (1ULL << 47)) too_big = true;
            is_big[l] = q[l] >= (1ULL << 36); plane_of[l] = fp64_planes;
            fp64_planes += is_big[l] ? 2 : 1; digit_planes += is_big[l] ? 6 : 5;
            if (is_big[l]) { if (l_big < 0) l_big = l; nbig++; }
            else { if (l_small0 < 0) l_small0 = l; nsmall++; packed_mask_all |= 1u << l; if (l == 0 || is_big[l - 1]) small_runs++; }
        }
    }
    bool all_small() const { return nbig == 0; }
};

inline size_t mac_i8_stream_bytes(int K, int nl, int ND, int copies_of_rot) {
    const size_t N = SFG_N, H = N / 2, nch = ((size_t)K + 63) / 64;
    return (size_t)nl * (N * nch * 2 * ND * 1024 * copies_of_rot + H * 6 * nch * ND * 1024 + H * 2 * 6 * 2 * 256 * 8);
}
inline size_t mac_i8_tile_bytes(int Kp, int nl, int ND) { return (size_t)nl * (SFG_N / 2) * 6 * (((size_t)Kp + 63) / 64) * ND * 1024; }
inline size_t mac_i8_rot_tile_bytes(int K, int nl, int ND) { return (size_t)nl * SFG_N * (((size_t)K + 63) / 64) * 2 * ND * 1024; }

enum class RotSrc { own, f64_cache, i8_tiles };
struct MmPlanIn {
    int mm_group = 8; bool mm_group_auto = true, mac_i8 = true, mac_i8_big = true, pt_compact = true, pt_kmajor = true; int pt_ride = 192; bool no_overlap = true;
    bool dma = true;
    unsigned packed_mask = 0;
    ModSplit mods;
    int s = 0, L = 0, nblockrows = 0, ncolb = 0;
    RotSrc rot = RotSrc::own; int pre_G = 0;
    size_t mem_search = 0;
    size_t mem_keep = 0;
    bool mem_failed = false;
};
struct MmPlan {
    int G = 0, ngroups = 0;
    bool keep_all = false;
    bool use_i8 = false, use_i8_big = false;
    bool compact = false, kmajor = false; int pt_layout = 0, pt_planes = 0;
    size_t prow = 0, plw = 0, panel_words = 0;
    size_t grp_slices = 0;
    bool pipelined = false;
    bool ride_want = false;
    unsigned enc_flags = 0;
};

inline MmPlan plan_at(const MmPlanIn &in, int G) {
    const int N = SFG_N, d = SFG_D, nb = in.nblockrows;
    const bool pre8 = in.rot == RotSrc::i8_tiles, own = in.rot == RotSrc::own;
    MmPlan p;
    p.G = G; p.ngroups = (nb + G - 1) / G;
    p.prow = in.dma ? (size_t)N / 2 : (size_t)N;
    if (in.dma && in.mac_i8 && in.packed_mask && in.rot == RotSrc::f64_cache && p.ngroups <= 16 && !in.mem_failed) {
        const size_t all = mac_i8_stream_bytes(G * d, in.mods.nsmall, 5, 0), per = mac_i8_stream_bytes(G * d, in.mods.nsmall, 5, 1) - all;
        p.keep_all = in.mem_keep >= (size_t)p.ngroups * per + all + SFG_I8_KEEP_RESERVE;
    }
    p.use_i8 = pre8 || (in.dma && in.mac_i8 && in.packed_mask && (p.ngroups <= 2 || in.ncolb >= 4 || p.keep_all));
    p.use_i8_big = pre8 || (p.use_i8 && in.mac_i8_big);
    const bool all_i8 = p.use_i8 && (p.use_i8_big || in.mods.all_small());
    p.grp_slices = (size_t)G * d + 3;
    p.pipelined = in.dma && own && nb > G && !in.no_overlap;
    p.compact = in.pt_compact && in.dma && all_i8;
    p.plw = (size_t)in.L * p.prow;
    if (p.compact) { p.pt_planes = in.mods.digit_planes; p.plw = (size_t)p.pt_planes * ((size_t)N / 2) / 8; }
    p.kmajor = p.compact && in.pt_kmajor && (size_t)G * d * 128 * 64 * 32 < (1ULL << 31);
    p.pt_layout = p.kmajor ? 2 : p.compact ? 1 : 0;
    p.panel_words = (size_t)G * d * d * p.plw;
    p.ride_want = all_i8 && in.pt_ride > 0 && (in.ncolb >= 2 || (pre8 && nb > G));
    if (in.dma) p.enc_flags = in.packed_mask | (p.use_i8 ? PT_DIGITS : 0u) | (p.use_i8_big ? PT_DIGITS_BIG : 0u) | (p.compact ? PT_COMPACT : 0u) | (p.kmajor ? PT_KMAJOR : 0u);
    return p;
}
inline size_t mm_search_estimate(const MmPlanIn &in, int G2) {
    const MmPlan p = plan_at(in, G2);
    const bool ride2 = in.mac_i8 && in.pt_ride > 0 && in.ncolb >= 2;
    size_t need = p.panel_words * 8 * (ride2 ? 2 : 1);
    if (in.rot == RotSrc::own) need += p.grp_slices * in.s * 2 * (size_t)in.mods.fp64_planes * SFG_N * 8 * (p.pipelined ? 2 : 1);
    if (in.mac_i8) {
        need += mac_i8_stream_bytes(G2 * SFG_D, in.mods.nsmall, 5, 1);
        if (in.mac_i8_big && in.mods.nbig) need += mac_i8_stream_bytes(G2 * SFG_D, 1, 6, 1);
    }
    return need;
}
inline int mm_group_size(const MmPlanIn &in) {
    const int nb = in.nblockrows;
    if (!in.dma) return 1;
    int G = in.rot == RotSrc::i8_tiles ? in.pre_G : in.mm_group;
    if (in.rot != RotSrc::i8_tiles && in.mm_group_auto && nb > G && (in.ncolb >= 4 || in.rot == RotSrc::own) && in.mods.fp64_planes > 0 && !in.mods.too_big && !in.mem_failed)
        for (int cand : {24, 20, 16, 14, 12, 10}) {
            const int G2 = std::min(cand, nb);
            if (G2 <= G) break;
            if (mm_search_estimate(in, G2) + (12ULL << 30) <= in.mem_search) { G = G2; break; }
        }
    return std::min(G, nb);
}
inline MmPlan mm_plan(const MmPlanIn &in) {
    if (in.nblockrows <= 0 || in.ncolb <= 0) return MmPlan();
    return plan_at(in, mm_group_size(in));
}
inline bool mm_plan_reads_memory(const MmPlanIn &in) {
    return in.dma && ((in.rot != RotSrc::i8_tiles && in.mm_group_auto && in.nblockrows > in.mm_group) || (in.rot == RotSrc::f64_cache && in.mac_i8 && in.packed_mask));
}

struct MmRangeIn {
    int s = 0, L = 0, nl = 0, rows = 0, cols = 0, fp64_planes = 0;
    size_t acc_budget = 0; bool no_overlap = true, dma = true; RotSrc rot = RotSrc::own;
};
struct MmRangePlan {
    int jg = 1, npasses = 0;
    bool whole_cache = false, overlap = false;
    size_t cache_bytes = 0, acc_bytes = 0;
};
inline MmRangePlan mm_range_plan(const MmRangeIn &in) {
    const size_t N = SFG_N, d = SFG_D, per_col = d * in.s * 2 * in.L * N * 8, rowf = (size_t)in.fp64_planes * N;
    MmRangePlan p;
    int jg0 = (int)(in.acc_budget / per_col); if (jg0 < 1) jg0 = 1;
    p.cache_bytes = ((size_t)in.rows * d * in.s * 2 * rowf + 3 * (size_t)in.s * 2 * rowf) * 8;
    p.whole_cache = in.rot == RotSrc::own && in.dma && in.cols > jg0 && in.rows > 0 && in.nl >= in.L && p.cache_bytes <= SFG_MM_WHOLE_CACHE_CAP;
    p.overlap = (p.whole_cache || in.rot != RotSrc::own) && !in.no_overlap;
    p.jg = p.overlap ? (jg0 + 1) / 2 : jg0;
    p.npasses = in.cols > 0 ? (in.cols + p.jg - 1) / p.jg : 0;
    p.acc_bytes = (size_t)p.jg * per_col * (p.overlap ? 2 : 1);
    return p;
}

inline size_t i8pre_tile_bytes(const ModSplit &m, int nbr, int G) {
    size_t t = 0;
    for (int b = 0; b < nbr; b += G) { const int ng = std::min(G, nbr - b); t += mac_i8_rot_tile_bytes(ng * SFG_D, m.nsmall, 5) + (m.nbig ? mac_i8_rot_tile_bytes(ng * SFG_D, 1, 6) : 0); }
    return t;
}
inline int i8pre_group_size(const ModSplit &m, int mm_group, bool mm_group_auto, int s, int nbr, bool mem_failed, size_t mem_search, size_t budget_bytes) {
    const int d = SFG_D;
    if (m.too_big || m.nbig > 1 || m.small_runs != 1) return 0;
    int G = std::min(mm_group, nbr);
    if (mm_group_auto && nbr > G && !mem_failed)
        for (int cand : {16, 12}) {
            const int G2 = std::min(cand, nbr);
            if (G2 <= G) break;
            const size_t panel = (size_t)G2 * d * d * m.L * (SFG_N / 2) * 8 * 2, rotf = ((size_t)G2 * d + 3) * s * 2 * m.fp64_planes * SFG_N * 8;
            const size_t need = i8pre_tile_bytes(m, nbr, G2) + panel + rotf + mac_i8_stream_bytes(G2 * d, m.nsmall, 5, 0) + (m.nbig ? mac_i8_stream_bytes(G2 * d, 1, 6, 0) : 0) + (24ULL << 30);
            if (need <= mem_search && i8pre_tile_bytes(m, nbr, G2) <= budget_bytes) { G = G2; break; }
        }
    if ((long long)G * d * 6 >= 131072 || i8pre_tile_bytes(m, nbr, G) > budget_bytes) return 0;
    return G;
}
```

### sfgwas_amd/csrc/rotate.hip

```cpp
#include "common.hpp"
#include "kernels.hpp"
#include "ksw.hpp"
#include "ksw_plan.hpp"
#include <memory>

constexpr int KSW_T = 3;


static void fill_ext(const sfg_ctx *ctx, ExtConst &e, const std::vector<int> &src) {
    memset(&e, 0, sizeof e);
    e.a = (int)src.size();
    for (int m = 0; m < e.a; m++) e.src[m] = src[m];
    for (int m = 0; m < e.a; m++) {
        u64 qm = ctx->q[src[m]], h = 1;
        for (int k = 0; k < e.a; k++) if (k != m) h = h_mulmod(h, ctx->q[src[k]] % qm, qm);
        u64 hi = h_invmod(h, qm);
        e.qhat_inv[m] = (double)hi; e.qhat_inv_q[m] = (double)hi / (double)qm;
    }
    for (int t = 0; t < ctx->nmod; t++) {
        u64 qt = ctx->q[t], D = 1 % qt;
        for (int m = 0; m < e.a; m++) {
            u64 ht = 1 % qt;
            for (int k = 0; k < e.a; k++) if (k != m) ht = h_mulmod(ht, ctx->q[src[k]] % qt, qt);
            e.qhat_t[t][m] = (double)ht; e.qhat_t_q[t][m] = (double)ht / (double)qt;
            D = h_mulmod(D, ctx->q[src[m]] % qt, qt);
        }
        e.D_t[t] = (double)D; e.D_t_q[t] = (double)D / (double)qt;
    }
}


int get_ksw(sfg_ctx *ctx, int level, const KswConst **dev, const KswConst **host) {
    const int nl = level + 1, alpha = ctx->np, nt = nl + ctx->np, beta = (nl + alpha - 1) / alpha;
    if (alpha > KSW_MAXA || beta > KSW_MAXDIG) SFG_FAIL(ctx, "key-switch shape unsupported (alpha > 4 or beta > 8)");
    if (beta * nt > SFG_MAXPATTERN) SFG_FAIL(ctx, "key-switch shape unsupported (beta * (level + 1 + np) = %d rows exceed the modulus pattern table)", beta * nt);
    auto it = ctx->ksw_cache.find(level);
    if (it != ctx->ksw_cache.end()) { *dev = it->second->dev; *host = &it->second->host; return 0; }
    std::unique_ptr<KswLevel> rec(new KswLevel);
    KswConst &kc = rec->host; memset(&kc, 0, sizeof kc);
    kc.level = level; kc.nl = nl; kc.np = ctx->np; kc.alpha = alpha; kc.nt = nt; kc.beta = beta;
    for (int t = 0; t < kc.nt; t++) { kc.tmod[t] = t < kc.nl ? t : ctx->nq + (t - kc.nl); kc.digit_of[t] = t < kc.nl ? t / kc.alpha : -1; }
    for (int i = 0; i < kc.beta; i++) {
        std::vector<int> src;
        for (int m = i * kc.alpha; m < (i + 1) * kc.alpha && m < kc.nl; m++) src.push_back(m);
        fill_ext(ctx, kc.dig[i], src);
    }
    std::vector<int> ps; for (int p = 0; p < kc.np; p++) ps.push_back(ctx->nq + p);
    fill_ext(ctx, kc.pq, ps);
    for (int t = 0; t < kc.nl; t++) {
        u64 qt = ctx->q[t], P = 1;
        for (int p = 0; p < kc.np; p++) P = h_mulmod(P, ctx->q[ctx->nq + p] % qt, qt);
        u64 pi = h_invmod(P, qt);
        kc.pinv[t] = (double)pi; kc.pinv_q[t] = (double)pi / (double)qt;
    }
    SFG_HIP(ctx, hipMalloc(&rec->dev, sizeof(KswConst)));
    if (hipError_t e = hipMemcpy(rec->dev, &kc, sizeof(KswConst), hipMemcpyHostToDevice)) { (void)hipFree(rec->dev); SFG_HIP(ctx, e); }
    *dev = rec->dev; *host = &rec->host;
    ctx->ksw_cache[level] = rec.release();
    return 0;
}


__device__ __forceinline__ void inv_last_of(const ModConst &mc, double w, double &u, double &v) {
    const double wn = canon(mulmod_lazy(w, mc.ninv, mc.ninv_q, mc.q), mc.q, mc.qinv);
    inv_last_pair(u, v, mc.ninv, mc.ninv_q, wn, wn * mc.qinv, mc.q, mc.qinv, u, v);
}
template <bool PRE1>
__global__ void __launch_bounds__(256) k_ksw_extend(const u64 *c2, u64 *ext, const KswConst *kcp, const ModConst *modc, const double *tw_fwd, const double *tw_inv) {
    const KswConst &kc = *kcp;
    const int N = SFG_N, n = N / 2, x = blockIdx.x * 256 + threadIdx.x, i = blockIdx.y; const size_t b = blockIdx.z;
    const ExtConst &e = kc.dig[i];
    const u64 *c2b = c2 + b * (size_t)kc.nl * N;
    u64 *eb = ext + (b * kc.beta + i) * (size_t)kc.nt * N;
    double xs[2][KSW_MAXA], y[2][KSW_MAXA], v[2] = {0.0, 0.0};
#pragma unroll
    for (int h = 0; h < 2; h++)
#pragma unroll
        for (int m = 0; m < KSW_MAXA; m++) xs[h][m] = m < e.a ? u64_to_f64(c2b[(size_t)e.src[m] * N + h * n + x]) : 0.0;
#pragma unroll
    for (int m = 0; m < KSW_MAXA; m++) if (m < e.a) inv_last_of(modc[e.src[m]], tw_inv[(size_t)e.src[m] * N + 1], xs[0][m], xs[1][m]);
    if (e.a > 1) { ext_prepare(e, modc, xs[0], y[0], v[0]); ext_prepare(e, modc, xs[1], y[1], v[1]); }
    for (int t = 0; t < kc.nt; t++) {
        const int tg = kc.tmod[t];
        if (kc.digit_of[t] == i) continue;
        const double q = modc[tg].q, qinv = modc[tg].qinv;
        double o0, o1;
        if (e.a == 1) { o0 = canon(xs[0][0], q, qinv); o1 = canon(xs[1][0], q, qinv); }
        else { o0 = ext_target(e, tg, q, qinv, y[0], v[0]); o1 = ext_target(e, tg, q, qinv, y[1], v[1]); }
        if (PRE1) { const double W = tw_fwd[(size_t)tg * N + 1]; fwd_stage1_pair(o0, o1, W, W * qinv, q, qinv, o0, o1); }
        eb[(size_t)t * N + x] = f64_to_u64(o0); eb[(size_t)t * N + n + x] = f64_to_u64(o1);
    }
}

template <int T>
__global__ void __launch_bounds__(256) k_ksw_inner_p(const u64 *ext, const u64 *const *keys, const int *inidx, const KswTile *tiles, u64 *acc, const KswConst *kcp,
                                                    const ModConst *modc, int nmod) {
    const KswConst &kc = *kcp;
    const int N = SFG_N, x = 2 * (blockIdx.x * 256 + threadIdx.x), m = blockIdx.y, t = kc.nl + m;
    const KswTile tl = tiles[blockIdx.z];
    const int tg = kc.tmod[t];
    const double q = modc[tg].q, qinv = modc[tg].qinv;
    const u64 *key = keys[tl.start];
    const u64 *eb[T];
#pragma unroll
    for (int j = 0; j < T; j++) eb[j] = ext + ((size_t)inidx[tl.start + (j < tl.count ? j : 0)] * kc.beta * (size_t)kc.nt + t) * N + x;
    double a[T][4];
#pragma unroll
    for (int j = 0; j < T; j++) a[j][0] = a[j][1] = a[j][2] = a[j][3] = 0.0;
    for (int i = 0; i < kc.beta; i++) {
        const ulonglong2 k0 = *reinterpret_cast<const ulonglong2 *>(key + (((size_t)i * 2 + 0) * nmod + tg) * N + x);
        const ulonglong2 k1 = *reinterpret_cast<const ulonglong2 *>(key + (((size_t)i * 2 + 1) * nmod + tg) * N + x);
        const double k0x = u64_to_f64(k0.x), k0y = u64_to_f64(k0.y), k1x = u64_to_f64(k1.x), k1y = u64_to_f64(k1.y);
#pragma unroll
        for (int j = 0; j < T; j++) {
            const ulonglong2 ev = *reinterpret_cast<const ulonglong2 *>(eb[j] + (size_t)i * kc.nt * N);
            const double ex = u64_to_f64(ev.x), ey = u64_to_f64(ev.y);
            a[j][0] += mulmod2(ex, k0x, q, qinv); a[j][1] += mulmod2(ey, k0y, q, qinv);
            a[j][2] += mulmod2(ex, k1x, q, qinv); a[j][3] += mulmod2(ey, k1y, q, qinv);
        }
    }
#pragma unroll
    for (int j = 0; j < T; j++) {
        if (j < tl.count) {
            u64 *o = acc + ((size_t)(tl.start + j) * 2 * kc.np + m) * N + x;
            *reinterpret_cast<ulonglong2 *>(o) = make_ulonglong2(f64_to_u64(canon(a[j][0], q, qinv)), f64_to_u64(canon(a[j][1], q, qinv)));
            *reinterpret_cast<ulonglong2 *>(o + (size_t)kc.np * N) = make_ulonglong2(f64_to_u64(canon(a[j][2], q, qinv)), f64_to_u64(canon(a[j][3], q, qinv)));
        }
    }
}

template <bool PRE1>
__global__ void __launch_bounds__(256) k_moddown_extend(const u64 *acc, u64 *ext2, const KswConst *kcp, const ModConst *modc, const double *tw_fwd, const double *tw_inv, int nq_out) {
    const KswConst &kc = *kcp;
    const int N = SFG_N, n = N / 2, x = blockIdx.x * 256 + threadIdx.x, p = blockIdx.y; const size_t b = blockIdx.z;
    const ExtConst &e = kc.pq;
    const u64 *ap = acc + (b * 2 + p) * (size_t)kc.np * N;
    double xs[2][KSW_MAXA], y[2][KSW_MAXA], v[2] = {0.0, 0.0};
#pragma unroll
    for (int h = 0; h < 2; h++)
#pragma unroll
        for (int m = 0; m < KSW_MAXA; m++) xs[h][m] = m < e.a ? u64_to_f64(ap[(size_t)m * N + h * n + x]) : 0.0;
#pragma unroll
    for (int m = 0; m < KSW_MAXA; m++) if (m < e.a) inv_last_of(modc[e.src[m]], tw_inv[(size_t)e.src[m] * N + 1], xs[0][m], xs[1][m]);
    if (e.a > 1) { ext_prepare(e, modc, xs[0], y[0], v[0]); ext_prepare(e, modc, xs[1], y[1], v[1]); }
    for (int t = 0; t < nq_out; t++) {
        const double q = modc[t].q, qinv = modc[t].qinv;
        double o0, o1;
        if (e.a == 1) { o0 = canon(xs[0][0], q, qinv); o1 = canon(xs[1][0], q, qinv); }
        else { o0 = ext_target(e, t, q, qinv, y[0], v[0]); o1 = ext_target(e, t, q, qinv, y[1], v[1]); }
        if (PRE1) { const double W = tw_fwd[(size_t)t * N + 1]; fwd_stage1_pair(o0, o1, W, W * qinv, q, qinv, o0, o1); }
        u64 *row = ext2 + ((b * 2 + p) * (size_t)kc.nl + t) * N;
        row[x] = f64_to_u64(o0); row[n + x] = f64_to_u64(o1);
    }
}

struct F64Form { int on, L, centre; size_t rowf; int plane_of[SFG_MAXMOD], big[SFG_MAXMOD]; };
__device__ __forceinline__ void store_rot_f64(double *row, const F64Form &ff, int t, int x, double v, double q) {
    const int N = SFG_N;
    double *o = row + (size_t)ff.plane_of[t] * N;
    if (ff.big[t]) {
        const double wc = v > __builtin_floor(q * 0.5) ? v - q : v;
        const double hi = __builtin_floor((wc + 4194304.0) * 0x1p-23), lo = wc - hi * 8388608.0;
        o[2 * x] = lo; o[2 * x + 1] = hi;
    } else o[x] = (ff.centre && v > __builtin_floor(q * 0.5)) ? v - q : v;
}
template <int T>
__device__ __forceinline__ void ksw_inner_q(const u64 *ext, const u64 *ct_in, const u64 *key, const KswConst &kc, int nmod, int t, int src, const size_t (&bi)[T],
                                           double q, double qinv, double (&a)[T][2]) {
    const int N = SFG_N;
#pragma unroll
    for (int j = 0; j < T; j++) a[j][0] = a[j][1] = 0.0;
    for (int i = 0; i < kc.beta; i++) {
        const double k0 = u64_to_f64(key[(((size_t)i * 2 + 0) * nmod + t) * N + src]), k1 = u64_to_f64(key[(((size_t)i * 2 + 1) * nmod + t) * N + src]);
        const bool own = kc.digit_of[t] == i;
#pragma unroll
        for (int j = 0; j < T; j++) {
            const double e = u64_to_f64(own ? ct_in[(bi[j] * 2 * (size_t)kc.nl + kc.nl + t) * N + src] : ext[((bi[j] * kc.beta + i) * (size_t)kc.nt + t) * N + src]);
            a[j][0] += mulmod2(e, k0, q, qinv); a[j][1] += mulmod2(e, k1, q, qinv);
        }
    }
}
template <int T>
__global__ void __launch_bounds__(256) k_ksw_finish(const u64 *ext, const u64 *ct_in, const u64 *const *keys, const int *inidx, const u64 *ext2, const uint16_t *const *index,
                                                   u64 *const *ct_out, const KswTile *tiles, const KswConst *kcp, const ModConst *modc, int nmod, const u64 *add1, F64Form ff) {
    const KswConst &kc = *kcp;
    const int N = SFG_N, x = blockIdx.x * 256 + threadIdx.x, t = blockIdx.y;
    if (ff.on && t >= ff.L) return;
    const KswTile tl = tiles[blockIdx.z];
    const double q = modc[t].q, qinv = modc[t].qinv, pinv = kc.pinv[t], pinv_q = kc.pinv_q[t];
    const int src = index[tl.start][x];
    size_t bi[T];
#pragma unroll
    for (int j = 0; j < T; j++) bi[j] = (size_t)inidx[tl.start + (j < tl.count ? j : 0)];
    double a[T][2];
    ksw_inner_q<T>(ext, ct_in, keys[tl.start], kc, nmod, t, src, bi, q, qinv, a);
#pragma unroll
    for (int j = 0; j < T; j++) {
        if (j < tl.count) {
            const size_t b = (size_t)(tl.start + j);
#pragma unroll
            for (int p = 0; p < 2; p++) {
                const double e = u64_to_f64(ext2[((b * 2 + p) * (size_t)kc.nl + t) * N + src]);
                double r = mulmod_lazy(pred(a[j][p], q, qinv) - e, pinv, pinv_q, q);
                if (p == 0) r += u64_to_f64(ct_in[(bi[j] * 2 * (size_t)kc.nl + t) * N + src]);
                else if (add1) r += u64_to_f64(add1[(bi[j] * (size_t)kc.nl + t) * N + src]);
                const double v = canon(r, q, qinv);
                if (ff.on) store_rot_f64(reinterpret_cast<double *>(ct_out[b]) + (size_t)p * ff.rowf, ff, t, x, v, q);
                else ct_out[b][((size_t)p * kc.nl + t) * N + x] = f64_to_u64(v);
            }
        }
    }
}

struct KswSeg { const u64 *plain; u64 *out; int start, count, accumulate, pad; };
__global__ void __launch_bounds__(256) k_ksw_finish_sum(const u64 *ext, const u64 *ct_in, const u64 *const *keys, const int *inidx, const u64 *ext2, const uint16_t *const *index,
                                                       const KswSeg *segs, const int *jobs, const KswConst *kcp, const ModConst *modc, int nmod) {
    const KswConst &kc = *kcp;
    const int N = SFG_N, x = blockIdx.x * 256 + threadIdx.x, t = blockIdx.y;
    const KswSeg sg = segs[blockIdx.z];
    const double q = modc[t].q, qinv = modc[t].qinv, pinv = kc.pinv[t], pinv_q = kc.pinv_q[t];
    const size_t w0 = (size_t)t * N + x, w1 = ((size_t)kc.nl + t) * N + x;
    double s0 = 0.0, s1 = 0.0;
    if (sg.accumulate) { s0 = u64_to_f64(sg.out[w0]); s1 = u64_to_f64(sg.out[w1]); }
    if (sg.plain) { s0 += u64_to_f64(sg.plain[w0]); s1 += u64_to_f64(sg.plain[w1]); }
    for (int k = 0; k < sg.count; k++) {
        const size_t b = (size_t)jobs[sg.start + k];
        const size_t bi[1] = {(size_t)inidx[b]};
        const int src = index[b][x];
        double a[1][2];
        ksw_inner_q<1>(ext, ct_in, keys[b], kc, nmod, t, src, bi, q, qinv, a);
        const double e0 = u64_to_f64(ext2[((b * 2 + 0) * (size_t)kc.nl + t) * N + src]), e1 = u64_to_f64(ext2[((b * 2 + 1) * (size_t)kc.nl + t) * N + src]);
        const double c0 = u64_to_f64(ct_in[(bi[0] * 2 * (size_t)kc.nl + t) * N + src]);
        s0 += canon(mulmod_lazy(pred(a[0][0], q, qinv) - e0, pinv, pinv_q, q) + c0, q, qinv);
        s1 += canon(mulmod_lazy(pred(a[0][1], q, qinv) - e1, pinv, pinv_q, q), q, qinv);
        if ((k & 7) == 7) { s0 = pred(s0, q, qinv); s1 = pred(s1, q, qinv); }
    }
    sg.out[w0] = f64_to_u64(canon(s0, q, qinv)); sg.out[w1] = f64_to_u64(canon(s1, q, qinv));
}

__global__ void __launch_bounds__(256) k_ct_add(const u64 *a, const u64 *b, u64 *out, int nl, const ModConst *modc, size_t total_rows) {
    const int N = SFG_N; const size_t row = blockIdx.x / (N / 256); const int m = (int)(row % nl);
    const u64 q = modc[m].qi;
    const size_t off = row * N + (blockIdx.x % (N / 256)) * 256 + threadIdx.x;
    u64 v = a[off] + b[off]; out[off] = v >= q ? v - q : v;
}

struct KswSum { int nout; std::vector<const u64 *> plain; u64 *out; size_t out_stride; int accumulate; };
struct KswJobs {
    std::vector<int> job_in; std::vector<const u64 *> keyp; std::vector<const uint16_t *> idxp; std::vector<u64 *> outp; std::vector<int> group;
    void add(int in, const RotKey &key, u64 *out, int grp = 0) { job_in.push_back(in); keyp.push_back(key.key_dev); idxp.push_back(key.index_dev); outp.push_back(out); group.push_back(grp); }
    KswJobs(int nct, const RotKey &key, u64 *out, size_t stride) { for (int j = 0; j < nct; j++) add(j, key, out + (size_t)j * stride); }
    KswJobs() {}
};
struct KswBatch { const u64 *in; int nin, level; const u64 *add1 = nullptr; const F64Form *ff = nullptr; const KswSum *sum = nullptr; };
static_assert(sizeof(KswSeg) == KSW_SEG_BYTES && sizeof(void *) == KSW_PTR_BYTES, "ksw_plan.hpp lays the tables out for these sizes");

static int launch_keyswitch_jobs(sfg_ctx *ctx, const KswBatch &bt, const KswJobs &jb) {
    const int N = SFG_N, level = bt.level, nl = level + 1, nin = bt.nin;
    const u64 *in = bt.in, *add1 = bt.add1; const KswSum *sum = bt.sum;
    F64Form ff; memset(&ff, 0, sizeof ff); if (bt.ff) ff = *bt.ff;
    const KswConst *kcd, *kcp;
    SFG_TRY(get_ksw(ctx, level, &kcd, &kcp));
    const KswConst &kc = *kcp;
    const size_t ctw = (size_t)2 * nl * N;
    const int nr = (int)jb.job_in.size(), nout = sum ? sum->nout : 0;
    if (sum && (ff.on || add1 || (int)sum->plain.size() != nout)) SFG_FAIL(ctx, "key switch: internal: malformed sum groups");
    if (!nr && !nout) return 0;
    const int nq_out = ff.on ? ff.L : nl;
    const bool pre1 = !ctx->cfg.ntt_fwd_full;
    const KswSizes sz = ksw_plan_sizes(nl, kc.np, kc.nt, kc.beta, nin, nr, nout, ctx->cfg.ksw_budget, (size_t)N);
    std::vector<KswGroup> groups;
    ksw_plan_groups(jb.job_in.data(), jb.keyp.data(), jb.idxp.data(), nr, nin, sz.in_grp, sz.chunk, KSW_T, groups);
    SFG_TRY(sfg_ws_reserve(ctx, sz.at.bytes));
    u64 *const w = (u64 *)ctx->ws; char *const wb = (char *)ctx->ws;
    u64 *c2 = w + sz.at.c2, *ext = w + sz.at.ext, *acc = w + sz.at.acc, *ext2 = w + sz.at.ext2, *extT = w + sz.at.extT, *ext2T = w + sz.at.ext2T;
    const u64 **keys_all = (const u64 **)(wb + sz.at.keys); const uint16_t **idx_all = (const uint16_t **)(wb + sz.at.idx); u64 **out_all = (u64 **)(wb + sz.at.out);
    KswSeg *segs_d = (KswSeg *)(wb + sz.at.segs); int *inidx_all = (int *)(wb + sz.at.inidx), *segjobs_d = (int *)(wb + sz.at.segjobs);
    KswTile *tiles_all = (KswTile *)(wb + sz.at.tiles);
    std::vector<char> seen(nout, 0);
    std::vector<KswSegPlan> plan; std::vector<KswSeg> segs; std::vector<int> segjobs, grp;
    auto finish_sum = [&](const std::vector<int> &jobs, size_t c0, int nb, const u64 *bin, const u64 **keys_d, const int *inidx_d, const uint16_t **idx_d) -> int {
        grp.resize(nb);
        for (int k = 0; k < nb; k++) grp[k] = jb.group[jobs[c0 + k]];
        ksw_plan_segments(grp.data(), nb, nout, seen, plan, segjobs);
        if (plan.empty()) return 0;
        segs.clear();
        for (const KswSegPlan &sp : plan) {
            KswSeg sg; sg.plain = sp.first ? sum->plain[sp.out] : nullptr; sg.out = sum->out + (size_t)sp.out * sum->out_stride;
            sg.start = sp.start; sg.count = sp.count; sg.accumulate = (sum->accumulate || !sp.first) ? 1 : 0; sg.pad = 0;
            segs.push_back(sg);
        }
        SFG_TRY(sfg_upload_small(ctx, segs_d, segs.data(), segs.size() * sizeof(KswSeg)));
        SFG_TRY(sfg_upload_small(ctx, segjobs_d, segjobs.data(), (size_t)nb * sizeof(int)));
        hipLaunchKernelGGL(k_ksw_finish_sum, dim3(N / 256, nl, (unsigned)segs.size()), dim3(256), 0, ctx->stream, extT, bin, keys_d, inidx_d, ext2T, idx_d,
                           segs_d, segjobs_d, kcd, ctx->modc, ctx->nmod);
        SFG_HIP(ctx, hipGetLastError());
        return 0;
    };
    ModPattern pq; pq.period = nl; for (int m = 0; m < nl; m++) pq.m[m] = m < nq_out ? (int8_t)m : (int8_t)-2;
    const ModPattern pin = mod_pattern_run(0, nl);
    ModPattern pext; pext.period = kc.beta * kc.nt;
    for (int i = 0; i < kc.beta; i++) for (int t = 0; t < kc.nt; t++)
        pext.m[i * kc.nt + t] = (kc.digit_of[t] == i || (t >= nq_out && t < nl)) ? (int8_t)-2 : (int8_t)kc.tmod[t];
    const ModPattern pp = mod_pattern_run(ctx->nq, kc.np);
    RowMap rm_dense; rm_dense.rpg = 1; rm_dense.gstride_in = N; rm_dense.gstride_out = N;
    for (const KswGroup &g : groups) {
        const int i0 = g.i0, ni = g.ni;
        const std::vector<int> &jobs = g.jobs;
        const u64 *bin = in + (size_t)i0 * ctw;
        RowMap rm1; rm1.rpg = nl; rm1.gstride_in = ctw; rm1.gstride_out = (size_t)nl * N;
        SFG_TRY(launch_ntt_inv_split(ctx, bin + (size_t)nl * N, c2, (size_t)ni * nl, pin, rm1));
        if (pre1) hipLaunchKernelGGL(k_ksw_extend<true>, dim3(N / 512, kc.beta, ni), dim3(256), 0, ctx->stream, c2, ext, kcd, ctx->modc, ctx->tw_fwd, ctx->tw_inv);
        else hipLaunchKernelGGL(k_ksw_extend<false>, dim3(N / 512, kc.beta, ni), dim3(256), 0, ctx->stream, c2, ext, kcd, ctx->modc, ctx->tw_fwd, ctx->tw_inv);
        SFG_HIP(ctx, hipGetLastError());
        SFG_TRY(launch_ntt_fwd_staged(ctx, ext, extT, (size_t)ni * kc.beta * kc.nt, pext, pre1));
        {
            const size_t nj = jobs.size();
            std::vector<const u64 *> kp(nj); std::vector<const uint16_t *> ip(nj); std::vector<u64 *> op(nj); std::vector<int> ii(nj);
            for (size_t k = 0; k < nj; k++) { int j = jobs[k]; kp[k] = jb.keyp[j]; ip[k] = jb.idxp[j]; op[k] = sum ? nullptr : jb.outp[j]; ii[k] = jb.job_in[j] - i0; }
            SFG_TRY(sfg_upload_small(ctx, keys_all, kp.data(), nj * sizeof(void *)));
            SFG_TRY(sfg_upload_small(ctx, idx_all, ip.data(), nj * sizeof(void *)));
            if (!sum) SFG_TRY(sfg_upload_small(ctx, out_all, op.data(), nj * sizeof(void *)));
            SFG_TRY(sfg_upload_small(ctx, inidx_all, ii.data(), nj * sizeof(int)));
            SFG_TRY(sfg_upload_small(ctx, tiles_all, g.tiles.data(), g.tiles.size() * sizeof(KswTile)));
        }
        for (const KswChunk &c : g.chunks) {
            const int nb = c.nb;
            const u64 **keys_d = keys_all + c.c0; const uint16_t **idx_d = idx_all + c.c0; u64 **out_d = out_all + c.c0; int *inidx_d = inidx_all + c.c0;
            const KswTile *tiles_d = tiles_all + c.tile0; const unsigned ntiles = (unsigned)c.ntiles;
            hipLaunchKernelGGL(k_ksw_inner_p<KSW_T>, dim3(N / 512, kc.np, ntiles), dim3(256), 0, ctx->stream, extT, keys_d, inidx_d, tiles_d, acc, kcd, ctx->modc, ctx->nmod);
            SFG_HIP(ctx, hipGetLastError());
            SFG_TRY(launch_ntt_inv_split(ctx, acc, acc, (size_t)nb * 2 * kc.np, pp, rm_dense));
            if (pre1) hipLaunchKernelGGL(k_moddown_extend<true>, dim3(N / 512, 2, nb), dim3(256), 0, ctx->stream, acc, ext2, kcd, ctx->modc, ctx->tw_fwd, ctx->tw_inv, nq_out);
            else hipLaunchKernelGGL(k_moddown_extend<false>, dim3(N / 512, 2, nb), dim3(256), 0, ctx->stream, acc, ext2, kcd, ctx->modc, ctx->tw_fwd, ctx->tw_inv, nq_out);
            SFG_HIP(ctx, hipGetLastError());
            SFG_TRY(launch_ntt_fwd_staged(ctx, ext2, ext2T, (size_t)nb * 2 * nl, pq, pre1));
            if (sum) { SFG_TRY(finish_sum(jobs, (size_t)c.c0, nb, bin, keys_d, inidx_d, idx_d)); continue; }
            hipLaunchKernelGGL(k_ksw_finish<KSW_T>, dim3(N / 256, nq_out, ntiles), dim3(256), 0, ctx->stream, extT, bin, keys_d, inidx_d, ext2T, idx_d, out_d, tiles_d, kcd,
                               ctx->modc, ctx->nmod, add1 ? add1 + (size_t)i0 * nl * N : nullptr, ff);
            SFG_HIP(ctx, hipGetLastError());
        }
    }
    if (sum) SFG_TRY(finish_sum(std::vector<int>(), 0, 0, in, keys_all, inidx_all, idx_all));
    return 0;
}
struct RotJob { int nrot, src; const RotKey *key; };
static int resolve_rotation(sfg_ctx *ctx, const int *nrot_host, const int *in_index, int j, int nin, RotJob &r) {
    r.nrot = nrot_host[j] % SFG_SLOTS; if (r.nrot < 0) r.nrot += SFG_SLOTS;
    r.src = in_index ? in_index[j] : j; r.key = nullptr;
    if (r.src < 0 || r.src >= nin) SFG_FAIL(ctx, "rotate: input index out of range");
    if (r.nrot == 0) return 0;
    u64 g = sfg_galois_for_rotation(ctx, SFG_SLOTS - r.nrot);
    auto it = ctx->rotkeys().find(g);
    if (it == ctx->rotkeys().end()) SFG_FAIL(ctx, "rotate: no rotation key loaded for right-rotation by %d (galois element %llu)", r.nrot, g);
    r.key = &it->second;
    return 0;
}
static int unrotated_run(const int *nrot_host, const int *in_index, int j, int nct, int src, int nin) {
    int run = 1;
    while (j + run < nct && (nrot_host[j + run] % SFG_SLOTS) == 0 && (in_index ? in_index[j + run] : j + run) == src + run && src + run < nin) run++;
    return run;
}
int launch_rotate_right_indexed(sfg_ctx *ctx, const u64 *in, int nin, u64 *out, int nct, int level, const int *nrot_host, const int *in_index) {
    if (level < 0 || level >= ctx->nq) SFG_FAIL(ctx, "rotate: level out of range");
    const size_t ctw = (size_t)2 * (level + 1) * SFG_N;
    KswBatch bt{in, nin, level}; KswJobs jb; RotJob r;
    for (int j = 0; j < nct; j++) {
        SFG_TRY(resolve_rotation(ctx, nrot_host, in_index, j, nin, r));
        if (r.key) { jb.add(r.src, *r.key, out + j * ctw); continue; }
        const int run = unrotated_run(nrot_host, in_index, j, nct, r.src, nin);
        SFG_HIP(ctx, hipMemcpyAsync(out + j * ctw, in + (size_t)r.src * ctw, (size_t)run * ctw * 8, hipMemcpyDeviceToDevice, ctx->stream));
        j += run - 1;
    }
    return launch_keyswitch_jobs(ctx, bt, jb);
}
int launch_rotate_right_sum(sfg_ctx *ctx, const u64 *in, int nin, int nct, int level, const int *nrot_host, const int *in_index, const int *group, int nout,
                            u64 *out, size_t out_stride, int accumulate) {
    if (level < 0 || level >= ctx->nq) SFG_FAIL(ctx, "rotate: level out of range");
    const size_t ctw = (size_t)2 * (level + 1) * SFG_N;
    KswSum sum; sum.nout = nout; sum.plain.assign(nout, nullptr); sum.out = out; sum.out_stride = out_stride; sum.accumulate = accumulate;
    KswBatch bt{in, nin, level}; bt.sum = &sum; KswJobs jb; RotJob r;
    for (int j = 0; j < nct; j++) {
        if (group[j] < 0 || group[j] >= nout) SFG_FAIL(ctx, "rotate: sum group out of range");
        SFG_TRY(resolve_rotation(ctx, nrot_host, in_index, j, nin, r));
        if (r.key) { jb.add(r.src, *r.key, nullptr, group[j]); continue; }
        if (sum.plain[group[j]]) SFG_FAIL(ctx, "rotate: more than one unrotated member in a sum group");
        sum.plain[group[j]] = in + (size_t)r.src * ctw;
    }
    return launch_keyswitch_jobs(ctx, bt, jb);
}
int launch_rotate_right_indexed_f64(sfg_ctx *ctx, const u64 *in, int nin, double *outf, int nct, int level, const int *nrot_host, const int *in_index, int L,
                                    const size_t *out_slot) {
    const int N = SFG_N, nl = level + 1;
    ctx->i8_gen++;
    if (level < 0 || level >= ctx->nq || L > nl) SFG_FAIL(ctx, "rotate: level out of range");
    const size_t ctw = (size_t)2 * nl * N;
    std::vector<int> plane_of, is_big; const int nplanes = mac_dma_planes(ctx, L, plane_of, is_big);
    if (nplanes < 0) return 1;
    F64Form ff; memset(&ff, 0, sizeof ff);
    ff.on = 1; ff.L = L; ff.centre = mac_dma_packed_mask(ctx, L) != 0; ff.rowf = (size_t)nplanes * N;
    for (int l = 0; l < L; l++) { ff.plane_of[l] = plane_of[l]; ff.big[l] = is_big[l]; }
    KswBatch bt{in, nin, level}; bt.ff = &ff; KswJobs jb; RotJob r;
    for (int j = 0; j < nct; j++) {
        SFG_TRY(resolve_rotation(ctx, nrot_host, in_index, j, nin, r));
        double *dst = outf + (out_slot ? out_slot[j] : (size_t)j) * 2 * ff.rowf;
        if (r.key) { jb.add(r.src, *r.key, reinterpret_cast<u64 *>(dst)); continue; }
        const int run = out_slot ? 1 : unrotated_run(nrot_host, in_index, j, nct, r.src, nin);
        SFG_TRY(launch_rot_to_f64(ctx, in + (size_t)r.src * ctw, (size_t)2 * run, nl, L, dst));
        j += run - 1;
    }
    return launch_keyswitch_jobs(ctx, bt, jb);
}
int launch_relinearize(sfg_ctx *ctx, const u64 *tmp, int nct, int level, const u64 *mid, u64 *out) {
    auto it = ctx->rotkeys().find(1);
    if (it == ctx->rotkeys().end()) SFG_FAIL(ctx, "relinearize: no relinearisation key loaded");
    KswBatch bt{tmp, nct, level}; bt.add1 = mid;
    return launch_keyswitch_jobs(ctx, bt, KswJobs(nct, it->second, out, (size_t)2 * (level + 1) * SFG_N));
}
int launch_rotate_right(sfg_ctx *ctx, const u64 *in, u64 *out, int nct, int level, const int *nrot_host) {
    return launch_rotate_right_indexed(ctx, in, nct, out, nct, level, nrot_host, nullptr);
}

extern "C" int sfg_rotate_right_dev(sfg_ctx *ctx, const uint64_t *in, uint64_t *out, int nct, int level, const int *nrot_host) {
    SFG_HIP(ctx, hipSetDevice(ctx->device));
    if (in == out) SFG_FAIL(ctx, "rotate: in and out must not alias");
    PhaseTimer t(ctx, "rotate");
    int rc = launch_rotate_right(ctx, (const u64 *)in, (u64 *)out, nct, level, nrot_host);
    t.stop(1);
    return rc;
}

extern "C" int sfg_ct_galois_dev(sfg_ctx *ctx, const uint64_t *in, uint64_t *out, int nct, int level, uint64_t galois_el) {
    SFG_HIP(ctx, hipSetDevice(ctx->device));
    if (in == out) SFG_FAIL(ctx, "galois: in and out must not alias");
    if (level < 0 || level >= ctx->nq) SFG_FAIL(ctx, "galois: level out of range");
    auto it = ctx->rotkeys().find(galois_el);
    if (it == ctx->rotkeys().end() || galois_el == 1) SFG_FAIL(ctx, "galois: no switching key loaded for galois element %llu", (unsigned long long)galois_el);
    PhaseTimer t(ctx, "rotate");
    int rc = launch_keyswitch_jobs(ctx, KswBatch{(const u64 *)in, nct, level}, KswJobs(nct, it->second, (u64 *)out, (size_t)2 * (level + 1) * SFG_N));
    t.stop(1);
    return rc;
}

int launch_ct_add(sfg_ctx *ctx, const u64 *a, const u64 *b, u64 *out, size_t nct, int level) {
    const int nl = level + 1; const size_t rows = nct * 2 * nl;
    if (!rows) return 0;
    hipLaunchKernelGGL(k_ct_add, dim3((unsigned)(rows * (SFG_N / 256))), dim3(256), 0, ctx->stream, a, b, out, nl, ctx->modc, rows);
    SFG_HIP(ctx, hipGetLastError());
    return 0;
}
extern "C" int sfg_ct_add_dev(sfg_ctx *ctx, const uint64_t *a, const uint64_t *b, uint64_t *out, int nct, int level) {
    SFG_HIP(ctx, hipSetDevice(ctx->device));
    if (level < 0 || level >= ctx->nq) SFG_FAIL(ctx, "evaluator op: level %d out of range", level);
    if (nct < 0) SFG_FAIL(ctx, "evaluator op: negative ciphertext count");
    return launch_ct_add(ctx, (const u64 *)a, (const u64 *)b, (u64 *)out, (size_t)nct, level);
}
```

Baseline: 6425 billion.

## Emit rotated ciphertext rows as int8 digit planes instead of fp64 planes

Adds a digit-plane output form for rotations: the key-switch finish kernel and a new unrotated-copy kernel write byte digit planes directly, and a new pack kernel builds the i8 MAC rot tiles from these bytes instead of converting fp64 rows. This is meant to cut the memory traffic of the rotated operand, which goes from 8 bytes per fp64 plane to one byte per digit plane, and to remove the conversion work in the pack step. It is on by default through a new config flag, and a test hook compares the tiles from both paths. The cost is extra DPP/permute work in the finish kernel and a second code path that must stay bit-exact.

```diff
diff --git a/sfgwas_amd/csrc/ab/config.hip b/sfgwas_amd/csrc/ab/config.hip
--- a/sfgwas_amd/csrc/ab/config.hip
+++ b/sfgwas_amd/csrc/ab/config.hip
@@ -19,6 +19,7 @@
     if (const char *e = env("SFG_PT_KMAJOR")) c.pt_kmajor = atoi(e) != 0;
     if (const char *e = env("SFG_PT_RIDE_DEPTH")) { c.i8_mover_depth_ride = atoi(e); if (c.i8_mover_depth_ride < 1 || c.i8_mover_depth_ride > 3) c.i8_mover_depth_ride = 1; }
     if (const char *e = env("SFG_PT_RIDE_NT")) c.i8_mover_nt_ride = atoi(e) != 0;
+    if (const char *e = env("SFG_ROT_OPERAND")) c.rot_digits = strcmp(e, "f64") != 0;
     if (env("SFG_ASSOC_TRACE")) c.assoc_trace = true;
 }
 int ab_set_attrs(sfg_ctx *ctx) { return ab_mac_dma_set_attrs(ctx) || ab_ntt_set_attrs(ctx); }
diff --git a/sfgwas_amd/csrc/ab/rot_tiles.hip b/sfgwas_amd/csrc/ab/rot_tiles.hip
--- /dev/null
+++ b/sfgwas_amd/csrc/ab/rot_tiles.hip
@@ -0,0 +1,51 @@
+#include "../common.hpp"
+#include "../kernels.hpp"
+#include <vector>
+
+__global__ void __launch_bounds__(256) k_rt_diff(const unsigned *a, const unsigned *b, size_t n, unsigned long long *cnt) {
+    unsigned long long c = 0, nz = 0;
+    for (size_t i = (size_t)blockIdx.x * 256 + threadIdx.x; i < n; i += (size_t)gridDim.x * 256) {
+        const unsigned x = a[i], y = b[i];
+        if (x == y && x == 0u) continue;
+#pragma unroll
+        for (int k = 0; k < 4; k++) { c += ((x ^ y) >> (8 * k) & 255u) != 0u; nz += (x >> (8 * k) & 255u) != 0u; }
+    }
+    if (c) atomicAdd(cnt, c);
+    if (nz) atomicAdd(cnt + 1, nz);
+}
+extern "C" int sfg_ab_rot_tiles_diff(sfg_ctx *ctx, const uint64_t *cts, int s, int level, int L, const int *nrot, int K, unsigned long long *counts) {
+    SFG_HIP(ctx, hipSetDevice(ctx->device));
+    if (!ctx->test_hooks) SFG_FAIL(ctx, "sfg_ab_rot_tiles_diff is a test hook");
+    if (s < 1 || 2 * s > 30 || K < 1 || K > 64 || L < 1 || L > level + 1 || level >= ctx->nq) SFG_FAIL(ctx, "sfg_ab_rot_tiles_diff: bad arguments");
+    const int N = SFG_N;
+    const ModSplit m(ctx->q, L);
+    if (m.too_big || m.nbig > 1 || m.small_runs > 1) SFG_FAIL(ctx, "sfg_ab_rot_tiles_diff: expects one run of 35-bit moduli and at most one 46-bit one");
+    const size_t rowf = (size_t)m.fp64_planes * N, rowb = (size_t)m.digit_planes * N, rows = (size_t)K * s * 2;
+    const size_t nAs = m.nsmall ? mac_i8_rot_tile_bytes(K, m.nsmall, 5) : 0, nAb = m.nbig ? mac_i8_rot_tile_bytes(K, 1, 6) : 0;
+    DevMem f64rows, digrows, A0, A1, cnt;
+    SFG_HIP(ctx, hipMalloc(&f64rows.h, rows * rowf * 8)); SFG_HIP(ctx, hipMalloc(&digrows.h, rows * rowb)); SFG_HIP(ctx, hipMalloc(&A0.h, nAs + nAb)); SFG_HIP(ctx, hipMalloc(&A1.h, nAs + nAb));
+    SFG_HIP(ctx, hipMalloc(&cnt.h, 4 * sizeof(unsigned long long)));
+    SFG_HIP(ctx, hipMemsetAsync(A0.h, 0x5A, nAs + nAb, ctx->stream)); SFG_HIP(ctx, hipMemsetAsync(A1.h, 0xA5, nAs + nAb, ctx->stream));
+    SFG_HIP(ctx, hipMemsetAsync(cnt.h, 0, 4 * sizeof(unsigned long long), ctx->stream));
+    std::vector<int> nrv((size_t)K * s), inv((size_t)K * s);
+    for (int k = 0; k < K; k++) for (int i = 0; i < s; i++) { nrv[(size_t)k * s + i] = nrot[k]; inv[(size_t)k * s + i] = i; }
+    SFG_TRY(launch_rotate_right_indexed_f64(ctx, (const u64 *)cts, s, (double *)f64rows.h, K * s, level, nrv.data(), inv.data(), L));
+    SFG_TRY(launch_rotate_right_indexed_digits(ctx, (const u64 *)cts, s, (uint8_t *)digrows.h, K * s, level, nrv.data(), inv.data(), L));
+    int8_t *a0 = (int8_t *)A0.h, *a1 = (int8_t *)A1.h;
+    if (m.nsmall) {
+        SFG_TRY(launch_i8_pack_rot_to(ctx, f64rows.h, (size_t)s * 2 * rowf, rowf, m.plane_of[m.l_small0], K, 2 * s, m.l_small0, m.nsmall, false, a0));
+        int dp = 0; for (int l = 0; l < m.l_small0; l++) dp += m.is_big[l] ? 6 : 5;
+        SFG_TRY(launch_i8_pack_rot_to(ctx, digrows.h, (size_t)s * 2 * rowb, rowb, dp, K, 2 * s, m.l_small0, m.nsmall, false, a1, true));
+        hipLaunchKernelGGL(k_rt_diff, dim3(4096), dim3(256), 0, ctx->stream, (const unsigned *)a0, (const unsigned *)a1, nAs / 4, (unsigned long long *)cnt.h);
+    }
+    if (m.nbig) {
+        SFG_TRY(launch_i8_pack_rot_to(ctx, f64rows.h, (size_t)s * 2 * rowf, rowf, m.plane_of[m.l_big], K, 2 * s, m.l_big, 1, true, a0 + nAs));
+        int dp = 0; for (int l = 0; l < m.l_big; l++) dp += m.is_big[l] ? 6 : 5;
+        SFG_TRY(launch_i8_pack_rot_to(ctx, digrows.h, (size_t)s * 2 * rowb, rowb, dp, K, 2 * s, m.l_big, 1, true, a1 + nAs, true));
+        hipLaunchKernelGGL(k_rt_diff, dim3(4096), dim3(256), 0, ctx->stream, (const unsigned *)(a0 + nAs), (const unsigned *)(a1 + nAs), nAb / 4, (unsigned long long *)cnt.h + 2);
+    }
+    SFG_HIP(ctx, hipGetLastError());
+    SFG_HIP(ctx, hipMemcpyAsync(counts, cnt.h, 4 * sizeof(unsigned long long), hipMemcpyDeviceToHost, ctx->stream));
+    SFG_HIP(ctx, hipStreamSynchronize(ctx->stream));
+    return 0;
+}
diff --git a/sfgwas_amd/csrc/common.hpp b/sfgwas_amd/csrc/common.hpp
--- a/sfgwas_amd/csrc/common.hpp
+++ b/sfgwas_amd/csrc/common.hpp
@@ -75,6 +75,7 @@
     int pt_ride = 192;
     int i8_mover_depth_ride = 1, i8_mover_nt_ride = 1;
     bool mac_plain_pt = false;
+    bool rot_digits = true;
     bool assoc_trace = false;
 };
 
diff --git a/sfgwas_amd/csrc/kernels.hpp b/sfgwas_amd/csrc/kernels.hpp
--- a/sfgwas_amd/csrc/kernels.hpp
+++ b/sfgwas_amd/csrc/kernels.hpp
@@ -25,10 +25,11 @@
                     const int8_t *B_small = nullptr, *B_big = nullptr;
                     int pt_layout = 0, pt_L = 0;
                     int B_mode = 0;
-                    const int8_t *A_small = nullptr, *A_big = nullptr; };
-int launch_mac_i8_small(sfg_ctx *ctx, const double *rotf, size_t rotf_k_stride, size_t rotf_r_stride, int plane0, const u64 *pt, u64 *out, int K, int R, int r0, int Ncols,
+                    const int8_t *A_small = nullptr, *A_big = nullptr;
+                    bool rot_digits = false; };
+int launch_mac_i8_small(sfg_ctx *ctx, const void *rot, size_t rotf_k_stride, size_t rotf_r_stride, int plane0, const u64 *pt, u64 *out, int K, int R, int r0, int Ncols,
                         int l0, int nl, int accumulate, const MacStrides &st);
-int launch_mac_i8_big(sfg_ctx *ctx, const double *rotf, size_t rotf_k_stride, size_t rotf_r_stride, int plane0, const u64 *pt, u64 *out, int K, int R, int r0, int Ncols,
+int launch_mac_i8_big(sfg_ctx *ctx, const void *rot, size_t rotf_k_stride, size_t rotf_r_stride, int plane0, const u64 *pt, u64 *out, int K, int R, int r0, int Ncols,
                       int l0, int accumulate, const MacStrides &st);
 int launch_skew(sfg_ctx *ctx, const int8_t *blk, size_t ld, int r, int c, int transposed, int square, int8_t *D);
 struct PcCache { double *slot = nullptr; int mode = 0; const uint32_t *perm = nullptr; };
@@ -57,6 +58,7 @@
 int launch_rotate_right_indexed(sfg_ctx *ctx, const u64 *in, int nin, u64 *out, int nct, int level, const int *nrot_host, const int *in_index);
 int launch_rotate_right_indexed_f64(sfg_ctx *ctx, const u64 *in, int nin, double *outf, int nct, int level, const int *nrot_host, const int *in_index, int L,
                                     const size_t *out_slot = nullptr);
+int launch_rotate_right_indexed_digits(sfg_ctx *ctx, const u64 *in, int nin, uint8_t *out8, int nct, int level, const int *nrot_host, const int *in_index, int L);
 int launch_rotate_right_sum(sfg_ctx *ctx, const u64 *in, int nin, int nct, int level, const int *nrot_host, const int *in_index, const int *group, int nout,
                             u64 *out, size_t out_stride, int accumulate);
 int launch_relinearize(sfg_ctx *ctx, const u64 *tmp, int nct, int level, const u64 *mid, u64 *out);
@@ -81,8 +83,10 @@
     int in_level = -1;
     const double *rows = nullptr;
     const I8RotPre *tiles = nullptr;
+    const uint8_t *digits = nullptr;
     static RotOperand own(const u64 *A, int in_level) { RotOperand r; r.A = A; r.in_level = in_level; return r; }
     static RotOperand f64_cache(const double *rows, int in_level = -1) { RotOperand r; r.src = RotSrc::f64_cache; r.rows = rows; r.in_level = in_level; return r; }
+    static RotOperand digit_cache(const uint8_t *rows8, int in_level) { RotOperand r; r.src = RotSrc::digit_cache; r.digits = rows8; r.in_level = in_level; return r; }
     static RotOperand i8_tiles(const I8RotPre *pre) { RotOperand r; r.src = RotSrc::i8_tiles; r.tiles = pre; return r; }
     int level_in(int max_level) const { return in_level < 0 ? max_level : in_level; }
     int validate(sfg_ctx *ctx, int s, int L, int nbr, int b0, int b1) const;
@@ -91,7 +95,7 @@
 struct MmRangeArgs { const sfg_geno *g; unsigned flags; int s, max_level, blk0, blk1; uint64_t *out; };
 int matmul_accumulate(sfg_ctx *ctx, const RotOperand &rot, const MmArgs &a);
 int matmul_resident_range(sfg_ctx *ctx, const RotOperand &rot, const MmRangeArgs &a);
-int launch_i8_pack_rot_to(sfg_ctx *ctx, const double *rotf, size_t rotf_k_stride, size_t rotf_r_stride, int plane0, int K, int R, int l0, int nl, bool big, int8_t *A_out);
+int launch_i8_pack_rot_to(sfg_ctx *ctx, const void *rot, size_t rotf_k_stride, size_t rotf_r_stride, int plane0, int K, int R, int l0, int nl, bool big, int8_t *A_out, bool digits = false);
 struct AssocRot { RotOperand op; I8RotPre pre; };
 int assoc_build_rot(sfg_ctx *ctx, const u64 *A_dev, int s, int in_level, int max_level, size_t nr, const std::vector<size_t> &widths, AssocRot &out);
 void assoc_free_rot(AssocRot &r);
diff --git a/sfgwas_amd/csrc/mac_i8.hip b/sfgwas_amd/csrc/mac_i8.hip
--- a/sfgwas_amd/csrc/mac_i8.hip
+++ b/sfgwas_amd/csrc/mac_i8.hip
@@ -59,6 +59,56 @@
         const uint4 w = *reinterpret_cast<const uint4 *>(img + c2 * CS + dg * 512 + ((lr ^ c2) << 4));
         *reinterpret_cast<uint4 *>(a.A + ((((((size_t)m * N + x0 + c2) * a.nch + ch) * 2 + rt) * ND + dg) * 1024) + khalf * 512 + lr * 16) = w;
     }
+}
+template <int ND>
+__global__ void __launch_bounds__(256) k_i8_pack_rot_digits(I8Args a) {
+    __shared__ __attribute__((aligned(16))) unsigned img[I8_PD * 64];
+    const int N = SFG_N, tid = threadIdx.x;
+    int b = blockIdx.x;
+    const int cb = b % (N / I8_PD); b /= N / I8_PD;
+    const int kq = b % (a.nch * 4); b /= a.nch * 4;
+    const int rt = b & 1, m = b >> 1;
+    const int c0 = cb * I8_PD, cq = tid & 31, slot = tid >> 5;
+    const int ch = kq >> 2, g = kq & 3, l16 = tid & 15;
+    const unsigned char *src = reinterpret_cast<const unsigned char *>(a.rotf) + (size_t)(a.plane0 + m * ND) * N + c0 + cq * 4;
+    constexpr int NI = 8;
+    for (int d = 0; d < ND; d++) {
+        for (int it0 = 0; it0 < 8; it0 += NI) {
+            unsigned w[NI][4];
+#pragma unroll
+            for (int u = 0; u < NI; u++) {
+                const int item = (it0 + u) * 8 + slot, j = item >> 2, k4 = item & 3, r = a.r0 + rt * 16 + j;
+#pragma unroll
+                for (int x = 0; x < 4; x++) {
+                    const int k = kq * 16 + k4 * 4 + x;
+                    const bool ok = k < a.K && r < a.R;
+                    const unsigned v = *reinterpret_cast<const unsigned *>(src + (ok ? (size_t)k * a.rotf_k_stride + (size_t)r * a.rotf_r_stride : (size_t)0) + (size_t)d * N);
+                    w[u][x] = ok ? v : 0u;
+                }
+            }
+#pragma unroll
+            for (int u = 0; u < NI; u++) {
+                const int item = (it0 + u) * 8 + slot, j = item >> 2, k4 = item & 3;
+                unsigned o[4]; bytes_tr4(w[u][0], w[u][1], w[u][2], w[u][3], o);
+#pragma unroll
+                for (int e = 0; e < 4; e++) img[(cq * 4 + e) * 64 + ((j ^ (cq & 7)) << 2) + (k4 ^ (cq >> 3))] = o[e];
+            }
+        }
+        __syncthreads();
+        for (int pc = tid >> 4; pc < I8_PD; pc += 16) {
+            const int q2 = pc >> 2;
+            const unsigned *sp = img + pc * 64 + ((l16 ^ (q2 & 7)) << 2);
+            const uint4 w = make_uint4(sp[0 ^ (q2 >> 3)], sp[1 ^ (q2 >> 3)], sp[2 ^ (q2 >> 3)], sp[3 ^ (q2 >> 3)]);
+            *reinterpret_cast<uint4 *>(a.A + ((((((size_t)m * N + c0 + pc) * a.nch + ch) * 2 + rt) * ND + d) * 1024) + g * 256 + l16 * 16) = w;
+        }
+        __syncthreads();
+    }
+}
+template <int ND>
+static void launch_i8_pack_rot_any(hipStream_t q, const I8Args &a, int nl, bool digits) {
+    const int N = SFG_N;
+    if (digits) hipLaunchKernelGGL(k_i8_pack_rot_digits<ND>, dim3((unsigned)((size_t)nl * 2 * a.nch * 4 * (N / I8_PD))), dim3(256), 0, q, a);
+    else hipLaunchKernelGGL(k_i8_pack_rot<ND>, dim3((unsigned)((size_t)nl * a.nch * (N / I8_PC) * 4)), dim3(256), I8_PC * i8_rot_img_stride<ND>(), q, a);
 }
 constexpr int I8_PP = 32;
 template <int ND>
@@ -382,10 +432,11 @@
     return 0;
 }
 template <int ND>
-static int launch_mac_i8_nd(sfg_ctx *ctx, const double *rotf, size_t rotf_k_stride, size_t rotf_r_stride, int plane0, const u64 *pt, u64 *out, int K, int R, int r0, int Ncols,
+static int launch_mac_i8_nd(sfg_ctx *ctx, const void *rot, size_t rotf_k_stride, size_t rotf_r_stride, int plane0, const u64 *pt, u64 *out, int K, int R, int r0, int Ncols,
                             int l0, int nl, int accumulate, const MacStrides &st) {
     const int N = SFG_N, H = N / 2;
     constexpr bool BIG = ND == 6;
+    const double *rotf = (const double *)rot;
     if (!st.pt_half || (!BIG && !st.pt_packed)) SFG_FAIL(ctx, "sfg_mac (i8): needs half-row plaintext rows (packed-limb words or digit planes for the small moduli)");
     if (BIG && nl != 1) SFG_FAIL(ctx, "sfg_mac (i8): one 46-bit modulus per launch");
     if (Ncols > 96) SFG_FAIL(ctx, "sfg_mac (i8): more than 96 columns per launch");
@@ -406,7 +457,7 @@
     a.K = K; a.R = R; a.Ncols = Ncols; a.accumulate = accumulate; a.r0 = r0; a.l0 = l0; a.nl = nl; a.plane0 = plane0;
     a.nch = (K + 63) / 64; a.njt = (Ncols + 15) / 16; a.pt_digits = st.pt_digits ? 1 : 0;
     const size_t nA = (size_t)nl * N * a.nch * 2 * ND * 1024, nB = (size_t)nl * H * a.njt * a.nch * ND * 1024, nT = (size_t)nl * H * 2 * a.njt * 2 * 256;
-    const u64 sig[8] = {ctx->i8_gen, (u64)K, (u64)R, (u64)r0, (u64)l0 << 8 | (u64)nl, (u64)plane0, (u64)rotf_k_stride, (u64)rotf_r_stride};
+    const u64 sig[8] = {ctx->i8_gen, (u64)K, (u64)R, (u64)r0, (u64)l0 << 8 | (u64)nl, (u64)plane0 | (u64)st.rot_digits << 32, (u64)rotf_k_stride, (u64)rotf_r_stride};
     sfg_ctx::I8Slot *slots = ctx->i8_slot[BIG ? 1 : 0];
     int slot = -1;
     if (!A_pre) for (int i = 0; i < sfg_ctx::I8_SLOTS; i++) if (slots[i].src == (const void *)rotf && !memcmp(slots[i].sig, sig, sizeof sig)) slot = i;
@@ -440,8 +491,8 @@
     if (!A_pre && !repack && ctx->pool[nm].second < nA) SFG_FAIL(ctx, "sfg_mac (i8): internal: kept rot copy smaller than its operand");
     const double tile = 1024.0;
     if (repack) { PhaseTimer t(ctx, "mac_i8_pack_rot");
-      hipLaunchKernelGGL(k_i8_pack_rot<ND>, dim3((unsigned)((size_t)nl * a.nch * (N / I8_PC) * 4)), dim3(256), I8_PC * i8_rot_img_stride<ND>(), ctx->stream, a);
-      SFG_HIP(ctx, hipGetLastError()); t.stop(1, (double)nl * N * ((double)K * std::min(32, R - r0) * (BIG ? 16.0 : 8.0) + (double)a.nch * 2 * ND * tile)); }
+      launch_i8_pack_rot_any<ND>(ctx->stream, a, nl, st.rot_digits);
+      SFG_HIP(ctx, hipGetLastError()); t.stop(1, (double)nl * N * ((double)K * std::min(32, R - r0) * (st.rot_digits ? (double)ND : BIG ? 16.0 : 8.0) + (double)a.nch * 2 * ND * tile)); }
     if (!B_pre) { PhaseTimer t(ctx, "mac_i8_pack_pt");
       const unsigned items = (unsigned)((size_t)nl * a.njt * a.nch * 4 * (H / I8_PD));
       if (a.pt_digits) launch_i8_pack_pt_digits(ctx->stream, a, items, BIG);
@@ -467,24 +518,23 @@
       t.stop(1, (double)nl * N * (double)Ncols * std::min(32, R - r0) * 8.0 * (accumulate ? 3.0 : 2.0)); }
     return 0;
 }
-int launch_i8_pack_rot_to(sfg_ctx *ctx, const double *rotf, size_t rotf_k_stride, size_t rotf_r_stride, int plane0, int K, int R, int l0, int nl, bool big, int8_t *A_out) {
+int launch_i8_pack_rot_to(sfg_ctx *ctx, const void *rot, size_t rotf_k_stride, size_t rotf_r_stride, int plane0, int K, int R, int l0, int nl, bool big, int8_t *A_out, bool digits) {
     if (R > 32 || (big && nl != 1)) SFG_FAIL(ctx, "i8 rot tiles: internal: at most 32 rows, one 46-bit modulus per buffer");
     I8Args a; memset(&a, 0, sizeof a);
-    a.rotf = rotf; a.rotf_k_stride = rotf_k_stride; a.rotf_r_stride = rotf_r_stride; a.K = K; a.R = R; a.r0 = 0; a.l0 = l0; a.nl = nl; a.plane0 = plane0;
+    a.rotf = (const double *)rot; a.rotf_k_stride = rotf_k_stride; a.rotf_r_stride = rotf_r_stride; a.K = K; a.R = R; a.r0 = 0; a.l0 = l0; a.nl = nl; a.plane0 = plane0;
     a.nch = (K + 63) / 64; a.kb = 0; a.A = A_out;
-    const int N = SFG_N;
     PhaseTimer t(ctx, "mac_i8_pack_rot");
-    if (big) hipLaunchKernelGGL(k_i8_pack_rot<6>, dim3((unsigned)((size_t)nl * a.nch * (N / I8_PC) * 4)), dim3(256), I8_PC * i8_rot_img_stride<6>(), ctx->stream, a);
-    else hipLaunchKernelGGL(k_i8_pack_rot<5>, dim3((unsigned)((size_t)nl * a.nch * (N / I8_PC) * 4)), dim3(256), I8_PC * i8_rot_img_stride<5>(), ctx->stream, a);
+    if (big) launch_i8_pack_rot_any<6>(ctx->stream, a, nl, digits);
+    else launch_i8_pack_rot_any<5>(ctx->stream, a, nl, digits);
     SFG_HIP(ctx, hipGetLastError());
     t.stop(1);
     return 0;
 }
-int launch_mac_i8_small(sfg_ctx *ctx, const double *rotf, size_t rotf_k_stride, size_t rotf_r_stride, int plane0, const u64 *pt, u64 *out, int K, int R, int r0, int Ncols,
+int launch_mac_i8_small(sfg_ctx *ctx, const void *rotf, size_t rotf_k_stride, size_t rotf_r_stride, int plane0, const u64 *pt, u64 *out, int K, int R, int r0, int Ncols,
                         int l0, int nl, int accumulate, const MacStrides &st) {
     return launch_mac_i8_nd<5>(ctx, rotf, rotf_k_stride, rotf_r_stride, plane0, pt, out, K, R, r0, Ncols, l0, nl, accumulate, st);
 }
-int launch_mac_i8_big(sfg_ctx *ctx, const double *rotf, size_t rotf_k_stride, size_t rotf_r_stride, int plane0, const u64 *pt, u64 *out, int K, int R, int r0, int Ncols,
+int launch_mac_i8_big(sfg_ctx *ctx, const void *rotf, size_t rotf_k_stride, size_t rotf_r_stride, int plane0, const u64 *pt, u64 *out, int K, int R, int r0, int Ncols,
                       int l0, int accumulate, const MacStrides &st) {
     return launch_mac_i8_nd<6>(ctx, rotf, rotf_k_stride, rotf_r_stride, plane0, pt, out, K, R, r0, Ncols, l0, 1, accumulate, st);
 }
diff --git a/sfgwas_amd/csrc/matmul.hip b/sfgwas_amd/csrc/matmul.hip
--- a/sfgwas_amd/csrc/matmul.hip
+++ b/sfgwas_amd/csrc/matmul.hip
@@ -320,14 +320,15 @@
     return baby_t;
 }
 static int build_rot_row_tab(sfg_ctx *ctx, const u64 *A, int s, int nl_in, int nl, int lev, int L, int nbr, int bi, const std::vector<uint8_t> &baby_t,
-                             u64 *a_row, u64 *rotc, bool dma, double *rotf_dst) {
+                             u64 *a_row, u64 *rotc, bool dma, void *rot_dst, bool digits = false) {
     const int d = SFG_D;
     SFG_TRY(launch_gather_operands(ctx, A, a_row, nbr, s, bi * s, s, nl_in, nl));
     {
         PhaseTimer t(ctx, "rotate");
         std::vector<int> nrv((size_t)d * s, 0), inv((size_t)d * s, 0);
         for (int baby = 0; baby < d; baby++) for (int i = 0; i < s; i++) { nrv[(size_t)baby * s + i] = baby_t[baby] ? -baby : 0; inv[(size_t)baby * s + i] = i; }
-        if (dma) SFG_TRY(launch_rotate_right_indexed_f64(ctx, a_row, s, rotf_dst, d * s, lev, nrv.data(), inv.data(), L));
+        if (dma && digits) SFG_TRY(launch_rotate_right_indexed_digits(ctx, a_row, s, (uint8_t *)rot_dst, d * s, lev, nrv.data(), inv.data(), L));
+        else if (dma) SFG_TRY(launch_rotate_right_indexed_f64(ctx, a_row, s, (double *)rot_dst, d * s, lev, nrv.data(), inv.data(), L));
         else SFG_TRY(launch_rotate_right_indexed(ctx, a_row, s, rotc, d * s, lev, nrv.data(), inv.data()));
         t.stop(1);
     }
@@ -350,7 +351,7 @@
     const SfgConfig &c = ctx->cfg;
     MmPlanIn in;
     in.mm_group = c.mm_group; in.mm_group_auto = c.mm_group_auto; in.mac_i8 = c.mac_i8; in.mac_i8_big = c.mac_i8_big;
-    in.pt_compact = c.pt_compact; in.pt_kmajor = c.pt_kmajor; in.pt_ride = c.pt_ride; in.no_overlap = c.no_overlap;
+    in.pt_compact = c.pt_compact; in.pt_kmajor = c.pt_kmajor; in.pt_ride = c.pt_ride; in.no_overlap = c.no_overlap; in.rot_digits = c.rot_digits;
     in.dma = mac_use_dma(ctx); in.packed_mask = in.dma ? mac_dma_packed_mask(ctx, L) : 0u; in.mods = ModSplit(ctx->q, L);
     in.s = s; in.L = L; in.nblockrows = nblockrows; in.ncolb = ncolb; in.rot = rot.src; in.pre_G = rot.tiles ? rot.tiles->G : 0;
     if (mm_plan_reads_memory(in)) { const PoolMemory m = pool_memory(ctx, nullptr); in.mem_failed = m.failed; in.mem_search = m.search; in.mem_keep = m.keep; }
@@ -358,20 +359,20 @@
 }
 struct MmCall {
     sfg_ctx *ctx; const Shape &sh; unsigned flags; const RotOperand &rot;
-    int s, L, lev, nl, nl_in; bool dma; unsigned packed_mask; size_t ctw, accw, rowf = 0;
+    int s, L, lev, nl, nl_in; bool dma; unsigned packed_mask; size_t ctw, accw, rowf = 0, rowb = 0;
     MmPlan plan;
-    u64 *a_row = nullptr, *rotc = nullptr; int8_t *skew = nullptr, *unpacked = nullptr; double *rotf = nullptr;
+    u64 *a_row = nullptr, *rotc = nullptr; int8_t *skew = nullptr, *unpacked = nullptr; char *rotf = nullptr;
     int8_t *rideBs = nullptr, *rideBb = nullptr;
 };
-struct MacJob { bool on = false; u64 *ptp = nullptr; int gsn = 0, gi = 0, acc_flag = 0; u64 *accj = nullptr; const double *rotf_grp = nullptr; };
+struct MacJob { bool on = false; u64 *ptp = nullptr; int gsn = 0, gi = 0, acc_flag = 0; u64 *accj = nullptr; const void *rotf_grp = nullptr; };
 
 static int build_group(const MmCall &c, int bg, int b1, int buf) {
     sfg_ctx *ctx = c.ctx; const int d = SFG_D, s = c.s, ng = std::min(c.plan.G, b1 - bg);
     ctx->i8_gen++;
-    double *dst = c.rotf + (size_t)buf * c.plan.grp_slices * s * 2 * c.rowf;
-    for (int g = 0; g < ng; g++) SFG_TRY(build_rot_row_tab(ctx, c.rot.A, s, c.nl_in, c.nl, c.lev, c.L, c.sh.nbr, bg + g, baby_table(c.sh, bg + g), c.a_row, c.rotc, c.dma, c.dma ? dst + (size_t)g * d * s * 2 * c.rowf : nullptr));
+    char *dst = c.rotf + (size_t)buf * c.plan.grp_slices * s * 2 * c.rowb;
+    for (int g = 0; g < ng; g++) SFG_TRY(build_rot_row_tab(ctx, c.rot.A, s, c.nl_in, c.nl, c.lev, c.L, c.sh.nbr, bg + g, baby_table(c.sh, bg + g), c.a_row, c.rotc, c.dma, c.dma ? dst + (size_t)g * d * s * 2 * c.rowb : nullptr, c.plan.rot_digits));
     if (c.dma && (ng * d) % 4)
-        SFG_HIP(ctx, hipMemsetAsync(dst + (size_t)ng * d * s * 2 * c.rowf, 0, (size_t)3 * s * 2 * c.rowf * 8, ctx->stream));
+        SFG_HIP(ctx, hipMemsetAsync(dst + (size_t)ng * d * s * 2 * c.rowb, 0, (size_t)3 * s * 2 * c.rowb, ctx->stream));
     return 0;
 }
 static int run_mac(const MmCall &c, const MacJob &m, int B_mode) {
@@ -384,8 +385,19 @@
     st.pt_k = p.plw; st.pt_n = (size_t)m.gsn * d * p.plw; st.pt_half = c.dma; st.pt_packed = c.packed_mask != 0; st.pt_digits = st.i8 = p.use_i8; st.i8_big = st.pt_digits_big = p.use_i8_big;
     st.pt_layout = p.pt_layout; st.pt_L = c.L;
     st.out_n = c.accw; st.out_r = (size_t)c.L * N;
-    int rc;
-    if (c.dma) rc = launch_mac_dma(ctx, m.rotf_grp, (size_t)c.s * 2, m.ptp, m.accj, m.gsn * d, 2 * c.s, d, c.L, m.acc_flag, st);
+    int rc = 0;
+    if (c.dma && p.rot_digits) {
+        const ModSplit ms(ctx->q, c.L);
+        st.rot_digits = true;
+        for (int l = 0, pl = 0; l < c.L && !rc;) {
+            const int big = ms.is_big[l]; int e = l, pe = pl; while (e < c.L && ms.is_big[e] == big) { pe += big ? 6 : 5; e++; }
+            if (!big) rc = launch_mac_i8_small(ctx, m.rotf_grp, (size_t)c.s * 2 * c.rowb, c.rowb, pl, m.ptp, m.accj, m.gsn * d, 2 * c.s, 0, d, l, e - l, m.acc_flag, st);
+            else { MacStrides sb = st; sb.pt_digits = st.pt_digits_big;
+                   for (int t = l; t < e && !rc; t++) rc = launch_mac_i8_big(ctx, m.rotf_grp, (size_t)c.s * 2 * c.rowb, c.rowb, pl + (t - l) * 6, m.ptp, m.accj, m.gsn * d, 2 * c.s, 0, d, t, m.acc_flag, sb); }
+            l = e; pl = pe;
+        }
+    }
+    else if (c.dma) rc = launch_mac_dma(ctx, (const double *)m.rotf_grp, (size_t)c.s * 2, m.ptp, m.accj, m.gsn * d, 2 * c.s, d, c.L, m.acc_flag, st);
 #ifdef SFG_AB
     else rc = launch_mac_strided(ctx, c.rotc, m.ptp, m.accj, d, 2 * c.s, d, c.L, m.acc_flag, st);
 #else
@@ -467,6 +479,8 @@
 
 int RotOperand::validate(sfg_ctx *ctx, int s, int L, int nbr, int b0, int b1) const {
     if (src == RotSrc::f64_cache && !mac_use_dma(ctx)) SFG_FAIL(ctx, "matmul: a prebuilt rotation cache needs the LDS-DMA MAC (the A/B build selected the register-staged kernel)");
+    if (src == RotSrc::digit_cache && (!digits || !rot_digits_possible(mac_use_dma(ctx), ctx->cfg.mac_i8, ctx->cfg.mac_i8_big, mac_dma_packed_mask(ctx, L), ctx->cfg.rot_digits, ModSplit(ctx->q, L), s)))
+        SFG_FAIL(ctx, "matmul: internal: a digit-plane rotation cache on a context that does not multiply every modulus on the int8 MAC");
     if (src == RotSrc::i8_tiles) {
         if (!tiles || !tiles->G) SFG_FAIL(ctx, "matmul: no int8 rot tiles");
         if (!mac_use_dma(ctx) || b0 != 0 || b1 != tiles->nbr || nbr != tiles->nbr || s != tiles->s || L != tiles->L)
@@ -505,10 +519,10 @@
     SFG_TRY(sfg_scratch(ctx, "mm.skew", (size_t)SFG_SLOTS * SFG_SLOTS, (void **)&c.skew));
     if (sh.g->packed) SFG_TRY(sfg_scratch(ctx, "mm.unpack", (size_t)SFG_SLOTS * SFG_SLOTS, (void **)&c.unpacked));
     if (dma) {
-        c.rowf = (size_t)in.mods.fp64_planes * N;
-        if (!rot_ext) SFG_TRY(sfg_scratch(ctx, "mm.rotf", plan.grp_slices * s * 2 * c.rowf * 8 * (plan.pipelined ? 2 : 1), (void **)&c.rotf));
-    }
-    const size_t rot_half = plan.grp_slices * s * 2 * c.rowf;
+        c.rowf = (size_t)in.mods.fp64_planes * N; c.rowb = plan.rot_row_bytes;
+        if (!rot_ext) SFG_TRY(sfg_scratch(ctx, "mm.rotf", plan.grp_slices * s * 2 * c.rowb * (plan.pipelined ? 2 : 1), (void **)&c.rotf));
+    }
+    const size_t rot_half = plan.grp_slices * s * 2 * c.rowb;
     hipStream_t main_stream = ctx->stream;
     if (plan.pipelined) {
         SFG_TRY(sfg_stream_after(ctx, ctx->aux_stream, main_stream));
@@ -520,8 +534,9 @@
     for (int bg = b0; bg < b1; bg += G, gi++) {
         const int ng = std::min(G, b1 - bg);
         if (held.on && in.rot != RotSrc::i8_tiles) { SFG_TRY(run_mac(c, held, 2)); held.on = false; }
-        const double *rotf_grp = c.rotf;
+        const void *rotf_grp = c.rotf;
         if (in.rot == RotSrc::f64_cache) rotf_grp = rot.rows + (size_t)(bg - b0) * d * s * 2 * c.rowf;
+        else if (in.rot == RotSrc::digit_cache) rotf_grp = rot.digits + (size_t)(bg - b0) * d * s * 2 * c.rowb;
         else if (in.rot == RotSrc::i8_tiles) rotf_grp = nullptr;
         else if (plan.pipelined) {
             if (bg + G < b1) {
@@ -611,6 +626,7 @@
     return matmul_finalize(ctx, (const u64 *)acc, s, max_level, ncolb, ncolb, 0, g0, g1, nullptr, accumulate, (u64 *)out, acc_giants, giant_base);
 }
 
+static int rotcache_build_rows_form(sfg_ctx *ctx, const u64 *A, int s, int in_level, int max_level, int nbr, int b0, int b1, const std::vector<std::vector<uint8_t>> *tabs, void *cache_, bool digits);
 int matmul_resident_range(sfg_ctx *ctx, const RotOperand &rot_in, const MmRangeArgs &a) {
     ApiScope api_scope(ctx);
     SFG_HIP(ctx, hipSetDevice(ctx->device));
@@ -627,16 +643,18 @@
     const int m_out = j1 - j0;
     MmRangeIn in;
     in.s = s; in.L = L; in.nl = std::min(rot_in.level_in(L), L) + 1; in.rows = b1 - b0; in.cols = j1 - j0; in.fp64_planes = ModSplit(ctx->q, L).fp64_planes;
+    in.digit_planes = ModSplit(ctx->q, L).digit_planes;
+    in.digits_ok = rot_digits_possible(mac_use_dma(ctx), ctx->cfg.mac_i8, ctx->cfg.mac_i8_big, mac_use_dma(ctx) ? mac_dma_packed_mask(ctx, L) : 0u, ctx->cfg.rot_digits, ModSplit(ctx->q, L), s);
     in.acc_budget = ctx->cfg.acc_budget; in.no_overlap = ctx->cfg.no_overlap; in.dma = mac_use_dma(ctx); in.rot = rot_in.src;
     const MmRangePlan plan = mm_range_plan(in);
     RotOperand rot = rot_in;
     if (plan.whole_cache) {
-        double *buf = nullptr;
-        SFG_TRY(sfg_scratch(ctx, "mm.rotf", plan.cache_bytes, (void **)&buf));
+        void *buf = nullptr;
+        SFG_TRY(sfg_scratch(ctx, "mm.rotf", plan.cache_bytes, &buf));
         std::vector<std::vector<uint8_t>> tabs;
         for (int bi = b0; bi < b1; bi++) tabs.push_back(baby_table(sh, bi));
-        SFG_TRY(rotcache_build_rows_tab(ctx, rot_in.A, s, rot_in.in_level, L, sh.nbr, b0, b1, &tabs, buf));
-        rot = RotOperand::f64_cache(buf, rot_in.in_level);
+        SFG_TRY(rotcache_build_rows_form(ctx, rot_in.A, s, rot_in.in_level, L, sh.nbr, b0, b1, &tabs, buf, plan.rot_digits));
+        rot = plan.rot_digits ? RotOperand::digit_cache((const uint8_t *)buf, rot_in.in_level) : RotOperand::f64_cache((const double *)buf, rot_in.in_level);
     }
     const int jg = plan.jg; const size_t accw = (size_t)s * 2 * L * SFG_N;
     hipStream_t main_stream = ctx->stream;
@@ -716,11 +734,13 @@
     SFG_HIP(ctx, hipMemsetAsync(cache + (size_t)nrows * d * s * jw, 0, (size_t)3 * s * jw * 8, ctx->stream));
     return 0;
 }
-int rotcache_build_rows_tab(sfg_ctx *ctx, const u64 *A, int s, int in_level, int max_level, int nbr, int b0, int b1, const std::vector<std::vector<uint8_t>> *tabs, double *cache) {
+static int rotcache_build_rows_form(sfg_ctx *ctx, const u64 *A, int s, int in_level, int max_level, int nbr, int b0, int b1, const std::vector<std::vector<uint8_t>> *tabs, void *cache_, bool digits) {
     ctx->i8_gen++;
     SFG_HIP(ctx, hipSetDevice(ctx->device));
     const int N = SFG_N, d = SFG_D, L = max_level;
     size_t rowf = 0; SFG_TRY(rotcache_rowf(ctx, L, rowf));
+    rowf = digits ? (size_t)ModSplit(ctx->q, L).digit_planes * N : rowf * 8;
+    char *cache = (char *)cache_;
     const int lev = in_level > max_level ? max_level : in_level, nl = lev + 1;
     if (nl < L || in_level >= ctx->nq) SFG_FAIL(ctx, "rotcache: input level %d unusable with max_level = %d", in_level, max_level);
     if (s < 1 || b0 < 0 || b1 > nbr || b0 > b1) SFG_FAIL(ctx, "rotcache: block-row range out of bounds");
@@ -730,9 +750,12 @@
     SFG_TRY(sfg_scratch(ctx, "mm.rotc", 8, (void **)&rotc));
     const std::vector<uint8_t> all(d, 1);
     for (int bi = b0; bi < b1; bi++)
-        SFG_TRY(build_rot_row_tab(ctx, A, s, in_level + 1, nl, lev, L, nbr, bi, tabs ? (*tabs)[bi - b0] : all, a_row, rotc, true, cache + (size_t)(bi - b0) * per_row));
-    SFG_HIP(ctx, hipMemsetAsync(cache + (size_t)(b1 - b0) * per_row, 0, (size_t)3 * s * 2 * rowf * 8, ctx->stream));
-    return 0;
+        SFG_TRY(build_rot_row_tab(ctx, A, s, in_level + 1, nl, lev, L, nbr, bi, tabs ? (*tabs)[bi - b0] : all, a_row, rotc, true, cache + (size_t)(bi - b0) * per_row, digits));
+    SFG_HIP(ctx, hipMemsetAsync(cache + (size_t)(b1 - b0) * per_row, 0, (size_t)3 * s * 2 * rowf, ctx->stream));
+    return 0;
+}
+int rotcache_build_rows_tab(sfg_ctx *ctx, const u64 *A, int s, int in_level, int max_level, int nbr, int b0, int b1, const std::vector<std::vector<uint8_t>> *tabs, double *cache) {
+    return rotcache_build_rows_form(ctx, A, s, in_level, max_level, nbr, b0, b1, tabs, cache, false);
 }
 extern "C" int sfg_rotcache_build_rows_dev(sfg_ctx *ctx, const uint64_t *A, int s, int in_level, int max_level, int nbr, int b0, int b1, double *cache) {
     ApiScope api_scope(ctx);
diff --git a/sfgwas_amd/csrc/mm_plan.hpp b/sfgwas_amd/csrc/mm_plan.hpp
--- a/sfgwas_amd/csrc/mm_plan.hpp
+++ b/sfgwas_amd/csrc/mm_plan.hpp
@@ -31,10 +31,14 @@
 inline size_t mac_i8_tile_bytes(int Kp, int nl, int ND) { return (size_t)nl * (SFG_N / 2) * 6 * (((size_t)Kp + 63) / 64) * ND * 1024; }
 inline size_t mac_i8_rot_tile_bytes(int K, int nl, int ND) { return (size_t)nl * SFG_N * (((size_t)K + 63) / 64) * 2 * ND * 1024; }
 
-enum class RotSrc { own, f64_cache, i8_tiles };
+enum class RotSrc { own, f64_cache, i8_tiles, digit_cache };
+inline bool rot_digits_possible(bool dma, bool mac_i8, bool mac_i8_big, unsigned packed_mask, bool rot_digits_cfg, const ModSplit &m, int s) {
+    return rot_digits_cfg && dma && mac_i8 && packed_mask != 0 && !m.too_big && (mac_i8_big || m.all_small()) && m.digit_planes > 0 && 2 * s <= 30;
+}
 struct MmPlanIn {
     int mm_group = 8; bool mm_group_auto = true, mac_i8 = true, mac_i8_big = true, pt_compact = true, pt_kmajor = true; int pt_ride = 192; bool no_overlap = true;
     bool dma = true;
+    bool rot_digits = false;
     unsigned packed_mask = 0;
     ModSplit mods;
     int s = 0, L = 0, nblockrows = 0, ncolb = 0;
@@ -47,6 +51,8 @@
     int G = 0, ngroups = 0;
     bool keep_all = false;
     bool use_i8 = false, use_i8_big = false;
+    bool rot_digits = false;
+    size_t rot_row_bytes = 0;
     bool compact = false, kmajor = false; int pt_layout = 0, pt_planes = 0;
     size_t prow = 0, plw = 0, panel_words = 0;
     size_t grp_slices = 0;
@@ -57,17 +63,19 @@
 
 inline MmPlan plan_at(const MmPlanIn &in, int G) {
     const int N = SFG_N, d = SFG_D, nb = in.nblockrows;
-    const bool pre8 = in.rot == RotSrc::i8_tiles, own = in.rot == RotSrc::own;
+    const bool pre8 = in.rot == RotSrc::i8_tiles, own = in.rot == RotSrc::own, dcache = in.rot == RotSrc::digit_cache;
     MmPlan p;
     p.G = G; p.ngroups = (nb + G - 1) / G;
     p.prow = in.dma ? (size_t)N / 2 : (size_t)N;
-    if (in.dma && in.mac_i8 && in.packed_mask && in.rot == RotSrc::f64_cache && p.ngroups <= 16 && !in.mem_failed) {
+    if (in.dma && in.mac_i8 && in.packed_mask && (in.rot == RotSrc::f64_cache || dcache) && p.ngroups <= 16 && !in.mem_failed) {
         const size_t all = mac_i8_stream_bytes(G * d, in.mods.nsmall, 5, 0), per = mac_i8_stream_bytes(G * d, in.mods.nsmall, 5, 1) - all;
         p.keep_all = in.mem_keep >= (size_t)p.ngroups * per + all + SFG_I8_KEEP_RESERVE;
     }
-    p.use_i8 = pre8 || (in.dma && in.mac_i8 && in.packed_mask && (p.ngroups <= 2 || in.ncolb >= 4 || p.keep_all));
+    p.use_i8 = pre8 || dcache || (in.dma && in.mac_i8 && in.packed_mask && (p.ngroups <= 2 || in.ncolb >= 4 || p.keep_all));
     p.use_i8_big = pre8 || (p.use_i8 && in.mac_i8_big);
     const bool all_i8 = p.use_i8 && (p.use_i8_big || in.mods.all_small());
+    p.rot_digits = dcache || (own && all_i8 && rot_digits_possible(in.dma, in.mac_i8, in.mac_i8_big, in.packed_mask, in.rot_digits, in.mods, in.s));
+    p.rot_row_bytes = p.rot_digits ? (size_t)in.mods.digit_planes * N : (size_t)in.mods.fp64_planes * N * 8;
     p.grp_slices = (size_t)G * d + 3;
     p.pipelined = in.dma && own && nb > G && !in.no_overlap;
     p.compact = in.pt_compact && in.dma && all_i8;
@@ -84,7 +92,7 @@
     const MmPlan p = plan_at(in, G2);
     const bool ride2 = in.mac_i8 && in.pt_ride > 0 && in.ncolb >= 2;
     size_t need = p.panel_words * 8 * (ride2 ? 2 : 1);
-    if (in.rot == RotSrc::own) need += p.grp_slices * in.s * 2 * (size_t)in.mods.fp64_planes * SFG_N * 8 * (p.pipelined ? 2 : 1);
+    if (in.rot == RotSrc::own) need += p.grp_slices * in.s * 2 * p.rot_row_bytes * (p.pipelined ? 2 : 1);
     if (in.mac_i8) {
         need += mac_i8_stream_bytes(G2 * SFG_D, in.mods.nsmall, 5, 1);
         if (in.mac_i8_big && in.mods.nbig) need += mac_i8_stream_bytes(G2 * SFG_D, 1, 6, 1);
@@ -108,24 +116,29 @@
     return plan_at(in, mm_group_size(in));
 }
 inline bool mm_plan_reads_memory(const MmPlanIn &in) {
-    return in.dma && ((in.rot != RotSrc::i8_tiles && in.mm_group_auto && in.nblockrows > in.mm_group) || (in.rot == RotSrc::f64_cache && in.mac_i8 && in.packed_mask));
+    return in.dma && ((in.rot != RotSrc::i8_tiles && in.mm_group_auto && in.nblockrows > in.mm_group) || ((in.rot == RotSrc::f64_cache || in.rot == RotSrc::digit_cache) && in.mac_i8 && in.packed_mask));
 }
 
 struct MmRangeIn {
     int s = 0, L = 0, nl = 0, rows = 0, cols = 0, fp64_planes = 0;
+    int digit_planes = 0; bool digits_ok = false;
     size_t acc_budget = 0; bool no_overlap = true, dma = true; RotSrc rot = RotSrc::own;
 };
 struct MmRangePlan {
     int jg = 1, npasses = 0;
     bool whole_cache = false, overlap = false;
+    bool rot_digits = false;
     size_t cache_bytes = 0, acc_bytes = 0;
 };
 inline MmRangePlan mm_range_plan(const MmRangeIn &in) {
-    const size_t N = SFG_N, d = SFG_D, per_col = d * in.s * 2 * in.L * N * 8, rowf = (size_t)in.fp64_planes * N;
+    const size_t N = SFG_N, d = SFG_D, per_col = d * in.s * 2 * in.L * N * 8;
+    const bool digits = in.digits_ok && in.rot == RotSrc::own && in.dma && in.digit_planes > 0;
+    const size_t row_bytes = digits ? (size_t)in.digit_planes * N : (size_t)in.fp64_planes * N * 8;
     MmRangePlan p;
     int jg0 = (int)(in.acc_budget / per_col); if (jg0 < 1) jg0 = 1;
-    p.cache_bytes = ((size_t)in.rows * d * in.s * 2 * rowf + 3 * (size_t)in.s * 2 * rowf) * 8;
+    p.cache_bytes = ((size_t)in.rows * d * in.s * 2 + 3 * (size_t)in.s * 2) * row_bytes;
     p.whole_cache = in.rot == RotSrc::own && in.dma && in.cols > jg0 && in.rows > 0 && in.nl >= in.L && p.cache_bytes <= SFG_MM_WHOLE_CACHE_CAP;
+    p.rot_digits = p.whole_cache && digits;
     p.overlap = (p.whole_cache || in.rot != RotSrc::own) && !in.no_overlap;
     p.jg = p.overlap ? (jg0 + 1) / 2 : jg0;
     p.npasses = in.cols > 0 ? (in.cols + p.jg - 1) / p.jg : 0;
diff --git a/sfgwas_amd/csrc/rotate.hip b/sfgwas_amd/csrc/rotate.hip
--- a/sfgwas_amd/csrc/rotate.hip
+++ b/sfgwas_amd/csrc/rotate.hip
@@ -3,6 +3,7 @@
 #include "ksw.hpp"
 #include "ksw_plan.hpp"
 #include <memory>
+#include <type_traits>
 
 constexpr int KSW_T = 3;
 
@@ -164,6 +165,26 @@
         o[2 * x] = lo; o[2 * x + 1] = hi;
     } else o[x] = (ff.centre && v > __builtin_floor(q * 0.5)) ? v - q : v;
 }
+struct DigForm { int on, L, centre; size_t rowb; int plane_of[SFG_MAXMOD], big[SFG_MAXMOD]; };
+__device__ __forceinline__ void rot_digits_of(bool big, int centre, double v, double q, unsigned &lo, unsigned &hi) {
+    const double wc = ((big || centre) && v > __builtin_floor(q * 0.5)) ? v - q : v;
+    const u64 b = (u64)__double_as_longlong(wc + (big ? 4503599627370496.0 + 141289400074368.0 : 4503599627370496.0 + 551911719040.0));
+    lo = (unsigned)b ^ 0x80808080u; hi = (unsigned)(b >> 32) ^ 0x8080u;
+}
+__device__ __forceinline__ unsigned quad_bytes(unsigned w, unsigned sel) {
+    const unsigned w0 = (unsigned)__builtin_amdgcn_mov_dpp((int)w, 0x00, 0xF, 0xF, true), w1 = (unsigned)__builtin_amdgcn_mov_dpp((int)w, 0x55, 0xF, 0xF, true);
+    const unsigned w2 = (unsigned)__builtin_amdgcn_mov_dpp((int)w, 0xAA, 0xF, 0xF, true), w3 = (unsigned)__builtin_amdgcn_mov_dpp((int)w, 0xFF, 0xF, 0xF, true);
+    return __builtin_amdgcn_perm(__builtin_amdgcn_perm(w3, w2, sel), __builtin_amdgcn_perm(w1, w0, sel), 0x05040100u);
+}
+__device__ __forceinline__ void store_rot_digits(uint8_t *row, const DigForm &df, int t, int x, double v, double q) {
+    const int N = SFG_N, d = x & 3, nd = df.big[t] ? 6 : 5;
+    unsigned lo, hi; rot_digits_of(df.big[t] != 0, df.centre, v, q, lo, hi);
+    const unsigned sel = (unsigned)d | ((unsigned)(4 + d) << 8);
+    const unsigned o = quad_bytes(lo, sel), p = quad_bytes(hi, sel);
+    uint8_t *pl = row + (size_t)df.plane_of[t] * N + (x & ~3);
+    *reinterpret_cast<unsigned *>(pl + (size_t)d * N) = o;
+    if (4 + d < nd) *reinterpret_cast<unsigned *>(pl + (size_t)(4 + d) * N) = p;
+}
 template <int T>
 __device__ __forceinline__ void ksw_inner_q(const u64 *ext, const u64 *ct_in, const u64 *key, const KswConst &kc, int nmod, int t, int src, const size_t (&bi)[T],
                                            double q, double qinv, double (&a)[T][2]) {
@@ -180,9 +201,9 @@
         }
     }
 }
-template <int T>
+template <int T, class Form>
 __global__ void __launch_bounds__(256) k_ksw_finish(const u64 *ext, const u64 *ct_in, const u64 *const *keys, const int *inidx, const u64 *ext2, const uint16_t *const *index,
-                                                   u64 *const *ct_out, const KswTile *tiles, const KswConst *kcp, const ModConst *modc, int nmod, const u64 *add1, F64Form ff) {
+                                                   u64 *const *ct_out, const KswTile *tiles, const KswConst *kcp, const ModConst *modc, int nmod, const u64 *add1, Form ff) {
     const KswConst &kc = *kcp;
     const int N = SFG_N, x = blockIdx.x * 256 + threadIdx.x, t = blockIdx.y;
     if (ff.on && t >= ff.L) return;
@@ -205,7 +226,8 @@
                 if (p == 0) r += u64_to_f64(ct_in[(bi[j] * 2 * (size_t)kc.nl + t) * N + src]);
                 else if (add1) r += u64_to_f64(add1[(bi[j] * (size_t)kc.nl + t) * N + src]);
                 const double v = canon(r, q, qinv);
-                if (ff.on) store_rot_f64(reinterpret_cast<double *>(ct_out[b]) + (size_t)p * ff.rowf, ff, t, x, v, q);
+                if constexpr (std::is_same<Form, DigForm>::value) store_rot_digits(reinterpret_cast<uint8_t *>(ct_out[b]) + (size_t)p * ff.rowb, ff, t, x, v, q);
+                else if (ff.on) store_rot_f64(reinterpret_cast<double *>(ct_out[b]) + (size_t)p * ff.rowf, ff, t, x, v, q);
                 else ct_out[b][((size_t)p * kc.nl + t) * N + x] = f64_to_u64(v);
             }
         }
@@ -252,7 +274,7 @@
     KswJobs(int nct, const RotKey &key, u64 *out, size_t stride) { for (int j = 0; j < nct; j++) add(j, key, out + (size_t)j * stride); }
     KswJobs() {}
 };
-struct KswBatch { const u64 *in; int nin, level; const u64 *add1 = nullptr; const F64Form *ff = nullptr; const KswSum *sum = nullptr; };
+struct KswBatch { const u64 *in; int nin, level; const u64 *add1 = nullptr; const F64Form *ff = nullptr; const KswSum *sum = nullptr; const DigForm *df = nullptr; };
 static_assert(sizeof(KswSeg) == KSW_SEG_BYTES && sizeof(void *) == KSW_PTR_BYTES, "ksw_plan.hpp lays the tables out for these sizes");
 
 static int launch_keyswitch_jobs(sfg_ctx *ctx, const KswBatch &bt, const KswJobs &jb) {
@@ -264,9 +286,11 @@
     const KswConst &kc = *kcp;
     const size_t ctw = (size_t)2 * nl * N;
     const int nr = (int)jb.job_in.size(), nout = sum ? sum->nout : 0;
-    if (sum && (ff.on || add1 || (int)sum->plain.size() != nout)) SFG_FAIL(ctx, "key switch: internal: malformed sum groups");
+    const DigForm *df = bt.df;
+    if (df && (bt.ff || add1 || df->L > nl)) SFG_FAIL(ctx, "key switch: internal: digit-plane rows are one output form of plain rotations");
+    if (sum && (ff.on || df || add1 || (int)sum->plain.size() != nout)) SFG_FAIL(ctx, "key switch: internal: malformed sum groups");
     if (!nr && !nout) return 0;
-    const int nq_out = ff.on ? ff.L : nl;
+    const int nq_out = df ? df->L : ff.on ? ff.L : nl;
     const bool pre1 = !ctx->cfg.ntt_fwd_full;
     const KswSizes sz = ksw_plan_sizes(nl, kc.np, kc.nt, kc.beta, nin, nr, nout, ctx->cfg.ksw_budget, (size_t)N);
     std::vector<KswGroup> groups;
@@ -336,7 +360,9 @@
             SFG_HIP(ctx, hipGetLastError());
             SFG_TRY(launch_ntt_fwd_staged(ctx, ext2, ext2T, (size_t)nb * 2 * nl, pq, pre1));
             if (sum) { SFG_TRY(finish_sum(jobs, (size_t)c.c0, nb, bin, keys_d, inidx_d, idx_d)); continue; }
-            hipLaunchKernelGGL(k_ksw_finish<KSW_T>, dim3(N / 256, nq_out, ntiles), dim3(256), 0, ctx->stream, extT, bin, keys_d, inidx_d, ext2T, idx_d, out_d, tiles_d, kcd,
+            if (df) hipLaunchKernelGGL((k_ksw_finish<KSW_T, DigForm>), dim3(N / 256, nq_out, ntiles), dim3(256), 0, ctx->stream, extT, bin, keys_d, inidx_d, ext2T, idx_d, out_d, tiles_d, kcd,
+                                       ctx->modc, ctx->nmod, (const u64 *)nullptr, *df);
+            else hipLaunchKernelGGL((k_ksw_finish<KSW_T, F64Form>), dim3(N / 256, nq_out, ntiles), dim3(256), 0, ctx->stream, extT, bin, keys_d, inidx_d, ext2T, idx_d, out_d, tiles_d, kcd,
                                ctx->modc, ctx->nmod, add1 ? add1 + (size_t)i0 * nl * N : nullptr, ff);
             SFG_HIP(ctx, hipGetLastError());
         }
@@ -411,6 +437,42 @@
     }
     return launch_keyswitch_jobs(ctx, bt, jb);
 }
+__global__ void __launch_bounds__(256) k_rot_to_digits(const u64 *in, uint8_t *out, int nl, DigForm df, const ModConst *modc) {
+    const int N = SFG_N, x = 4 * (blockIdx.x * 256 + threadIdx.x), l = blockIdx.y; const size_t row = blockIdx.z;
+    const double q = modc[l].q;
+    const ulonglong2 a = *reinterpret_cast<const ulonglong2 *>(in + (row * nl + l) * N + x), b = *reinterpret_cast<const ulonglong2 *>(in + (row * nl + l) * N + x + 2);
+    unsigned lo[4], hi[4];
+    rot_digits_of(df.big[l] != 0, df.centre, u64_to_f64(a.x), q, lo[0], hi[0]); rot_digits_of(df.big[l] != 0, df.centre, u64_to_f64(a.y), q, lo[1], hi[1]);
+    rot_digits_of(df.big[l] != 0, df.centre, u64_to_f64(b.x), q, lo[2], hi[2]); rot_digits_of(df.big[l] != 0, df.centre, u64_to_f64(b.y), q, lo[3], hi[3]);
+    unsigned o[4], p[4]; bytes_tr4(lo[0], lo[1], lo[2], lo[3], o); bytes_tr4(hi[0], hi[1], hi[2], hi[3], p);
+    uint8_t *pl = out + row * df.rowb + (size_t)df.plane_of[l] * N + x;
+#pragma unroll
+    for (int d = 0; d < 4; d++) *reinterpret_cast<unsigned *>(pl + (size_t)d * N) = o[d];
+    *reinterpret_cast<unsigned *>(pl + (size_t)4 * N) = p[0];
+    if (df.big[l]) *reinterpret_cast<unsigned *>(pl + (size_t)5 * N) = p[1];
+}
+int launch_rotate_right_indexed_digits(sfg_ctx *ctx, const u64 *in, int nin, uint8_t *out8, int nct, int level, const int *nrot_host, const int *in_index, int L) {
+    const int N = SFG_N, nl = level + 1;
+    ctx->i8_gen++;
+    if (level < 0 || level >= ctx->nq || L > nl || L < 1) SFG_FAIL(ctx, "rotate: level out of range");
+    const size_t ctw = (size_t)2 * nl * N;
+    const ModSplit m(ctx->q, L);
+    if (m.too_big) SFG_FAIL(ctx, "sfg_mac: modulus >= 2^47 unsupported by the fp64 limb schedule");
+    DigForm df; memset(&df, 0, sizeof df);
+    df.on = 1; df.L = L; df.centre = mac_dma_packed_mask(ctx, L) != 0; df.rowb = (size_t)m.digit_planes * N;
+    for (int l = 0, pl = 0; l < L; l++) { df.plane_of[l] = pl; df.big[l] = m.is_big[l]; pl += m.is_big[l] ? 6 : 5; }
+    KswBatch bt{in, nin, level}; bt.df = &df; KswJobs jb; RotJob r;
+    for (int j = 0; j < nct; j++) {
+        SFG_TRY(resolve_rotation(ctx, nrot_host, in_index, j, nin, r));
+        uint8_t *dst = out8 + (size_t)j * 2 * df.rowb;
+        if (r.key) { jb.add(r.src, *r.key, reinterpret_cast<u64 *>(dst)); continue; }
+        const int run = unrotated_run(nrot_host, in_index, j, nct, r.src, nin);
+        hipLaunchKernelGGL(k_rot_to_digits, dim3(N / 1024, L, 2 * run), dim3(256), 0, ctx->stream, in + (size_t)r.src * ctw, dst, nl, df, ctx->modc);
+        SFG_HIP(ctx, hipGetLastError());
+        j += run - 1;
+    }
+    return launch_keyswitch_jobs(ctx, bt, jb);
+}
 int launch_relinearize(sfg_ctx *ctx, const u64 *tmp, int nct, int level, const u64 *mid, u64 *out) {
     auto it = ctx->rotkeys().find(1);
     if (it == ctx->rotkeys().end()) SFG_FAIL(ctx, "relinearize: no relinearisation key loaded");
```

Result: no change. 6460 billion, median of 6 (+0.6%).
